# pyprob/pyprob

Hardware: AMD Instinct MI355X
Metric: ic_train_traces_per_sec (higher is better)
Workload: dtype f32; 1 GPU; GaussianUnknownMean IC training, offline traces resident in HBM, LSTM hidden=512, batch=1024 per GPU; traces_in_hbm=1000000, params=1643583, global_batch=1024, parallelism=dp1, optimizer=Adam lr=1e-3*sqrt(world), launch=one Python iteration per step (ICEngine.train_step), eager launches, prewarm_steps=5870, minibatches_resident=976, minibatch_walk=step i trains minibatch (i * 1) mod 976 of the resident dataset

## Files before the change

### include/pyprob_amd.h

```cpp
#ifndef PYPROB_AMD_H
#define PYPROB_AMD_H

#include <stddef.h>
#include <stdint.h>

#ifdef __cplusplus
extern "C" {
#endif

#define PP_ABI_VERSION 15
#define PP_MAX_OBS 8
#define PP_MAX_LSTM_DEPTH 4
#define PP_MAX_OBS_DEPTH 4

#define PP_EINVAL   (-1)
#define PP_ENOSPACE (-2)
#define PP_ENODEV   (-3)
#define PP_EHIP     (-4)

#define PP_HEAD_NORMAL_MIXTURE       0
#define PP_HEAD_TRUNCNORMAL_MIXTURE  1
#define PP_HEAD_CATEGORICAL          2
#define PP_HEAD_BERNOULLI            4
#define PP_HEAD_POISSON_TN_MIXTURE   3
// ... 53 lines not shown

size_t pp_cnn2d5c_workspace_bytes(const pp_net* net, int32_t o, int32_t n_images);
int pp_cnn2d5c_forward(const pp_net* net, int32_t o, const float* params, const float* x, int32_t n_images,
                       float* features_out, void* workspace, size_t workspace_bytes, void* stream);
int pp_cnn2d5c_backward(const pp_net* net, int32_t o, const float* params, const float* d_features, int32_t n_images,
                        float* grads, void* workspace, size_t workspace_bytes, int32_t flags, void* stream);

#define PP_ADDR_TABLE_COLS 8
#define PP_AT_KIND 0
#define PP_AT_SMP_IN 1
#define PP_AT_ADDR_EMB 2
#define PP_AT_DTYPE_EMB 3
#define PP_AT_SMP_W 4
#define PP_AT_SMP_B 5
#define PP_AT_N_OUT 6
#define PP_AT_RESERVED 7

typedef struct pp_batch {
    int32_t n_traces;
    int32_t n_rows;
    int32_t t_max;
    int32_t obs_width;
    const int32_t* n_active;
    const int32_t* row_off;
    const int32_t* grp_off;
    const float*   obs;
    const float*   value;
    const float*   prior;
    const int32_t* addr;
    const int32_t* prev_row;
    const int32_t* grp_rows;
    const int32_t* trace;
    const int32_t* row_off_dev;
    const int32_t* nxt_off;
    const int32_t* nxt_rows;
} pp_batch;

typedef struct pp_pack_info {
    int64_t n_traces, n_rows, t_max, device_words;
    int64_t obs, value, prior, addr, prev_row, grp_rows, trace, row_off_dev, nxt_rows;
    int64_t n_active, row_off, grp_off, nxt_off;
    int64_t order;
    int64_t src_row;
} pp_pack_info;

int64_t pp_pack_words(int32_t n_traces, int64_t n_rows, int32_t t_max, int32_t obs_width, int32_t n_addr);

int pp_pack_ragged(const int32_t* trace_len, const int32_t* addr_ids, const float* values, const float* prior,
                   int32_t prior_width, const float* obs, int32_t n_traces, int32_t obs_width, int32_t n_addr,
                   void* out, int64_t out_words, pp_pack_info* info);

typedef struct pp_shard_columns {
    const int32_t* trace_len;
    const int64_t* row_off;
    const float*   obs;
    const float*   value;
    const float*   prior;
    const int32_t* addr;
    const int32_t* addr_remap;
} pp_shard_columns;

int pp_pack_indexed(const pp_shard_columns* shards, int32_t n_shards, const int64_t* first, const int64_t* ids,
                    int32_t n_ids, int32_t obs_width, int32_t n_addr, void* out, int64_t out_words, pp_pack_info* info);


size_t pp_ic_workspace_bytes(const pp_net* net, int32_t n_traces, int32_t n_rows);

#define PP_LOSS_BACKWARD   1
#define PP_LOSS_ZERO_GRADS 2
#define PP_LOSS_KEEP_LP    4

int pp_ic_loss(const pp_net* net, const pp_batch* batch, const float* params , float* grads ,
               void* workspace , size_t workspace_bytes, float* loss_out ,
               int32_t* status_out , float* lp_out , int32_t flags, void* stream);

#define PP_ADAM_ZERO_GRADS 1
#define PP_ADAM_SCRATCH 1056
#define PP_ADAM_SEEN 1027
int pp_adam_step(float* params, float* grads, float* exp_avg, float* exp_avg_sq, int64_t n_params,
                 const int32_t* chunk_tensor, const float* active, int32_t* tensor_step, int32_t* scratch,
                 int32_t n_tensors, float lr, float beta1, float beta2, float eps, float weight_decay, float grad_scale,
                 int32_t flags, const int32_t* skip, void* stream);

int pp_sgd_step(float* params, float* grads, float* momentum_buf, int64_t n_params, const int32_t* chunk_tensor,
                const float* active, int32_t n_tensors, float lr, float momentum, int32_t nesterov, float weight_decay,
                float grad_scale, int32_t flags, const int32_t* skip, void* stream);

#define PP_LARC_SCRATCH_FLOATS(n_params, n_tensors) (2 * ((n_params) / 1024) + (n_tensors))
int pp_larc_scale(const float* params, float* grads, int64_t n_params, const int32_t* chunk_tensor, const float* active,
                  int32_t n_tensors, float lr, float weight_decay, float grad_scale, float trust_coefficient, float eps,
                  float epsilon, int32_t clip, float* scratch, const int32_t* skip, void* stream);

typedef struct pp_train_buffers {
    float* params; float* grads; float* exp_avg; float* exp_avg_sq;
    const int32_t* chunk_tensor; int32_t* tensor_step; int32_t* adam_scratch;
    void* workspace; size_t workspace_bytes;
    void* staging; void* device_batch; int64_t slot_words;
    float* loss_ring; int32_t* status_ring;
    int32_t n_tensors; int32_t n_slots;
    int32_t dp_world; int32_t dp_n_skip;
    int64_t dp_skip_off[4], dp_skip_cnt[4];
} pp_train_buffers;

typedef struct pp_tensor_roles {
    const int32_t* off;
    const int32_t* addr;
    const int32_t* role;
} pp_tensor_roles;

int64_t pp_train_slot_words(int32_t n_traces, int64_t n_rows, int32_t t_max, int32_t obs_width, int32_t n_addr,
                            int32_t n_tensors);

int pp_train_sync(void);
int pp_train_resident(const pp_net* net, const pp_train_buffers* tb, const pp_batch* const* batches,
                      const float* const* active, int32_t n_steps, const float* lr, float beta1, float beta2, float eps,
                      float weight_decay, int32_t grads_clean, void* stream);

int pp_train_steps(const pp_net* net, const pp_train_buffers* buffers, const pp_tensor_roles* roles,
                   const pp_shard_columns* shards, int32_t n_shards, const int64_t* first, int32_t obs_width,
                   const int64_t* ids, const int64_t* step_off, int32_t n_steps, const float* lr ,
                   float beta1, float beta2, float eps, float weight_decay, int32_t grads_clean,
                   int64_t* addr_iterations, void* stream);


size_t pp_is_workspace_bytes(const pp_net* net, int32_t n);

int pp_is_init(const pp_net* net, const float* params, const float* obs, float* e_out, void* workspace,
               size_t workspace_bytes, void* stream);

int pp_is_step(const pp_net* net, const float* params, int32_t addr_id, int32_t prev_addr_id, int32_t n,
               const float* e_obs_vec, const float* prev_value, const float* prior, int32_t prior_stride,
               float* h, float* c, int32_t state_rows, const float* value_in, float* value_out, float* logq_out,
               uint64_t seed, uint64_t offset, void* workspace, size_t workspace_bytes, void* stream);

int pp_is_step_rows(const pp_net* net, const float* params, int32_t addr_id, int32_t prev_addr_id, int32_t n,
                    const float* e_obs_vec, const float* prev_value, const float* prior, int32_t prior_stride,
                    float* h, float* c, int32_t state_rows, const int64_t* rows, const float* value_in, float* value_out,
                    float* logq_out, uint64_t seed, uint64_t offset, void* workspace, size_t workspace_bytes, void* stream);
int pp_is_step_fused_supported(const pp_net* net, int32_t addr_id, int32_t n);
int pp_is_statement_rows(const pp_net* net, const float* params, int32_t addr_id, int32_t prev_addr_id, int32_t n,
                         const float* e_obs_vec, const float* prev_value_full, const float* prior, int32_t prior_stride,
                         float* h, float* c, int32_t state_rows, const int64_t* rows, float* value_full, float* lw_full,
                         int32_t prior_kind, uint64_t seed, uint64_t offset, void* workspace, size_t workspace_bytes,
                         void* stream);

int pp_logweight_accumulate(int32_t kind, const float* p0, int32_t p0_stride, const float* p1, int32_t p1_stride,
                            const float* x, int32_t x_stride, float scale, float* lw , float* lp_out,
                            int32_t n, void* stream);

int pp_logweight_accumulate_rows(int32_t kind, const float* p0, int32_t p0_stride, const float* p1, int32_t p1_stride,
                                 const float* x, int32_t x_stride, float scale, float* lw ,
                                 const int64_t* rows, int32_t m, void* stream);

int pp_copy_rows(const float* src, int32_t src_stride, float* dst , const int64_t* rows, int32_t m, void* stream);

#define PP_PARTITION_SCRATCH(m) (((m) + 1023) / 1024 + 1)
int pp_partition_rows(const uint8_t* cond, const int64_t* rows, int32_t m, int64_t* rows_true, int64_t* rows_false,
                      int32_t* counts, int32_t* scratch, void* stream);
int pp_partition_rows_polled(const uint8_t* cond, const int64_t* rows, int32_t m, int64_t* rows_true, int64_t* rows_false,
                             int32_t* counts , int32_t seq, int32_t* scratch, void* stream);

typedef struct pp_lw_term {
    int32_t kind, p0_stride, p1_stride, x_stride;
    const float *p0, *p1, *x;
    float scale;
} pp_lw_term;
// ... 184 lines not shown
```

### pyprob_amd/autograd.py

```python
import torch

from . import lib as L
from .ops import ops


def presence(network, bring_home=False):
    eng = network._hip_engine
    index = {n: i for i, n in enumerate(eng.spec.tensors.keys())}
    present = [False] * len(index)
    for name, p in network._hip_named_parameters():
        if p.grad is None:
            continue
        present[index[name]] = True
        if bring_home:
            flat = eng.tensor(name, eng.grads)
            if p.grad.data_ptr() != flat.data_ptr():
                flat.copy_(p.grad)
    return tuple(present)


class HipLoss(torch.autograd.Function):

    @staticmethod
    def forward(ctx, network, packed, names, *params):
        eng = network._hip_engine
        flags = L.PP_LOSS_BACKWARD | (0 if network._hip_grads_clean else L.PP_LOSS_ZERO_GRADS)
        batch_dev, batch_host = packed.op_tensors(eng.device)
        eng._ensure_workspace(packed.n_traces, packed.n_rows)
        loss, status, _ = ops.ic_loss(eng.params, eng.grads, eng.workspace, batch_dev, batch_host, eng.net_handle, flags)
        network._hip_grads_clean = False
        network._hip_status = status
        ctx.network, ctx.names = network, names
        return loss.reshape(())

    @staticmethod
    def backward(ctx, grad_output):
        eng = ctx.network._hip_engine
        eng.grads.mul_(grad_output.reshape(()).to(eng.grads.device))
        return (None, None, None) + tuple(eng.tensor(n, eng.grads) for n in ctx.names)


class _HipOptimizer(torch.optim.Optimizer):

    def __init__(self, network, defaults, larc=False):
        self._network = network
        self._larc = bool(larc)
        super().__init__(list(network.parameters()), defaults)
        self._active_cache = {}
        self._stepped = set()

    def _begin(self):
        net = self._network
        eng = net._hip_engine
        present = presence(net, bring_home=True)
        act = self._active_cache.get(present)
        if act is None:
            act = self._active_cache[present] = torch.tensor(present, dtype=torch.float32).to(eng.device)
            self._stepped.update(i for i, f in enumerate(present) if f)
        eng.active.copy_(act)
        eng._active_key = None
        group = self.param_groups[0]
        wd, scale = float(group['weight_decay']), float(net._hip_grad_scale)
        if self._larc:
            need = L.larc_scratch_floats(eng.params.numel(), eng.active.numel())
            if getattr(self, '_larc_scratch', None) is None or self._larc_scratch.numel() < need:
                self._larc_scratch = torch.empty(need, dtype=torch.float32, device=eng.params.device)
            ops.larc_scale(eng.params, eng.grads, eng.chunk_tensor, eng.active, float(group['lr']), wd, scale, 0.002, 1e-8,
                           1.0 / 16000.0, True, self._larc_scratch, None)
            wd, scale = 0.0, 1.0
        return net, eng, group, wd, scale

    def _end(self, net):
        net._hip_grad_scale = 1.0
        net._hip_grads_clean = True

    def zero_grad(self, set_to_none=True):
        for p in self.param_groups[0]['params']:
            p.grad = None

    def _groups_state(self):
        groups = [dict((k, v) for k, v in self.param_groups[0].items() if k != 'params')]
        groups[0]['params'] = list(range(len(self.param_groups[0]['params'])))
        return groups

    def _load_groups(self, state_dict):
        for k, v in state_dict['param_groups'][0].items():
            if k != 'params':
                self.param_groups[0][k] = v


class HipSGD(_HipOptimizer):

    def __init__(self, network, lr, momentum=0.9, weight_decay=0.0, nesterov=True, larc=False):
        super().__init__(network, dict(lr=lr, momentum=momentum, dampening=0, weight_decay=weight_decay, nesterov=nesterov),
                         larc=larc)

    @torch.no_grad()
    def step(self, closure=None):
        net, eng, group, wd, scale = self._begin()
        ops.sgd_step(eng.params, eng.grads, eng.exp_avg, eng.chunk_tensor, eng.active, float(group['lr']),
                     float(group['momentum']), bool(group['nesterov']), wd, scale, L.PP_ADAM_ZERO_GRADS, None)
        self._end(net)

    def state_dict(self):
        net = self._network
        eng = net._hip_engine
        names = list(eng.spec.tensors.keys())
        state = {}
        if float(self.param_groups[0]['momentum']) != 0.0:
            for i, (name, p) in enumerate(net._hip_named_parameters()):
                if names.index(name) in self._stepped:
# ... 62 lines not shown
```

### pyprob_amd/csrc/cnn2d.hip

```cpp
#include "cnn2d.hpp"

#include <algorithm>

namespace pp {

bool cnn_geom(const pp_net* net, int o, CnnGeom& g) {
    if (!net || o < 0 || o >= net->n_obs || net->obs_kind[o] != PP_OBS_CNN2D5C) return false;
    g.C = net->obs_shape[o][0]; g.H = net->obs_shape[o][1]; g.W = net->obs_shape[o][2];
    if (g.C < 1 || g.C > 4 || g.H < 20 || g.W < 20) return false;
    const int ci[5] = {g.C, 64, 64, 128, 128}, co[5] = {64, 64, 128, 128, 128};
    int h = g.H, w = g.W;
    for (int l = 0; l < 5; ++l) {
        g.cin[l] = ci[l]; g.cout[l] = co[l]; g.hin[l] = h; g.win[l] = w;
        h -= 2; w -= 2;
        if (l == 1) { g.hp1 = h / 2; g.wp1 = w / 2; h = g.hp1; w = g.wp1; }
    }
    g.hp2 = h / 2; g.wp2 = w / 2;
    g.F = 128 * g.hp2 * g.wp2;
    return g.hp2 >= 1 && g.wp2 >= 1;
}

__global__ __launch_bounds__(256) void cnn_weight_images_kernel(const float* __restrict__ W, int Cin, int Cout,
                                                                float* __restrict__ wf, float* __restrict__ wd) {
    const int n = 9 * Cin * Cout;
// ... 416 lines not shown
    hipLaunchKernelGGL(wgrad_reduce_kernel, dim3(cdiv(wn + Cout, 256)), dim3(256), 0, st, w.part, dbp, S, Cin, Cout,
                       grads + net->obs_conv_w[o][l], grads + net->obs_conv_b[o][l]);
    PP_LAUNCH_CHECK("wgrad_reduce");
    prof_end(cls, 2.0 * (double)M * (double)wn, st);
    return 0;
}

int cnn_backward(const pp_net* net, int o, const float* dfeat, int64_t lddf, int B, float* grads, void* ws, size_t ws_bytes,
                 hipStream_t st) {
    CnnGeom g;
    CnnWs w;
    PP_TRY(check_cnn(net, o, g, B, ws, ws_bytes, w, "pp_cnn2d5c_backward"));
    PP_CHECK_ARG(dfeat && grads && lddf >= g.F, "pp_cnn2d5c_backward: null pointer or short rows");
    {
        const int H5 = g.hin[4] - 2, W5 = g.win[4] - 2;
        const int64_t n = (int64_t)B * H5 * W5 * 128;
        prof_begin(PP_PROF_CNN_BWD + 0, st);
        hipLaunchKernelGGL(maxpool_bwd_kernel, dim3(cdiv(n, 256)), dim3(256), 0, st, w.a[4], H5, W5, 128, dfeat, g.hp2, g.wp2, 1,
                           lddf, w.g0, n);
        PP_LAUNCH_CHECK("maxpool_bwd");
        prof_end(PP_PROF_CNN_BWD + 0, 0.0, st);
    }
    PP_TRY(conv_wgrad(net, o, g, 4, w.a[3], w.g0, B, w, grads, st));
    PP_TRY(conv_mfma(PP_PROF_CNN_BWD + 2, w.g0, g.hin[4] - 2, g.win[4] - 2, 128, 128, w.wd[4], nullptr, w.a[3], w.g1, 2, 0, B, st));
    PP_TRY(conv_wgrad(net, o, g, 3, w.a[2], w.g1, B, w, grads, st));
    PP_TRY(conv_mfma(PP_PROF_CNN_BWD + 4, w.g1, g.hin[3] - 2, g.win[3] - 2, 128, 128, w.wd[3], nullptr, w.a[2], w.g0, 2, 0, B, st));
    PP_TRY(conv_wgrad(net, o, g, 2, w.p1, w.g0, B, w, grads, st));
    PP_TRY(conv_mfma(PP_PROF_CNN_BWD + 6, w.g0, g.hin[2] - 2, g.win[2] - 2, 128, 64, w.wd[2], nullptr, nullptr, w.g1, 2, 0, B, st));
    {
        const int H2 = g.hin[1] - 2, W2 = g.win[1] - 2;
        const int64_t n = (int64_t)B * H2 * W2 * 64;
        prof_begin(PP_PROF_CNN_BWD + 7, st);
        hipLaunchKernelGGL(maxpool_bwd_kernel, dim3(cdiv(n, 256)), dim3(256), 0, st, w.a[1], H2, W2, 64, w.g1, g.hp1, g.wp1, 0,
                           (int64_t)0, w.g0, n);
        PP_LAUNCH_CHECK("maxpool_bwd");
        prof_end(PP_PROF_CNN_BWD + 7, 0.0, st);
    }
    PP_TRY(conv_wgrad(net, o, g, 1, w.a[0], w.g0, B, w, grads, st));
    PP_TRY(conv_mfma(PP_PROF_CNN_BWD + 9, w.g0, g.hin[1] - 2, g.win[1] - 2, 64, 64, w.wd[1], nullptr, w.a[0], w.g1, 2, 0, B, st));
    {
        const int64_t M = (int64_t)B * (g.H - 2) * (g.W - 2);
        int64_t chunk;
        const int64_t wn = 9 * (int64_t)g.C * 64;
        const int S = wgrad_splits(M, wn, &chunk);
        float* dbp = w.part + S * wn;
        const dim3 grid(S), block(256);
        prof_begin(PP_PROF_CNN_BWD + 10, st);
        switch (g.C) {
            case 1: hipLaunchKernelGGL(conv1_wgrad_kernel<1>, grid, block, 0, st, w.a0, w.g1, w.part, dbp, g.H, g.W, M, chunk); break;
            case 2: hipLaunchKernelGGL(conv1_wgrad_kernel<2>, grid, block, 0, st, w.a0, w.g1, w.part, dbp, g.H, g.W, M, chunk); break;
            case 3: hipLaunchKernelGGL(conv1_wgrad_kernel<3>, grid, block, 0, st, w.a0, w.g1, w.part, dbp, g.H, g.W, M, chunk); break;
            default: hipLaunchKernelGGL(conv1_wgrad_kernel<4>, grid, block, 0, st, w.a0, w.g1, w.part, dbp, g.H, g.W, M, chunk); break;
        }
        PP_LAUNCH_CHECK("conv1_wgrad");
        hipLaunchKernelGGL(wgrad_reduce_kernel, dim3(cdiv(wn + 64, 256)), dim3(256), 0, st, w.part, dbp, S, g.C, 64,
                           grads + net->obs_conv_w[o][0], grads + net->obs_conv_b[o][0]);
        PP_LAUNCH_CHECK("wgrad_reduce");
        prof_end(PP_PROF_CNN_BWD + 10, 2.0 * (double)M * (double)wn, st);
    }
    return 0;
}

}

extern "C" {

size_t pp_cnn2d5c_workspace_bytes(const pp_net* net, int32_t o, int32_t n_images) {
    return pp::cnn_workspace_bytes(net, o, n_images);
}

int pp_cnn2d5c_forward(const pp_net* net, int32_t o, const float* params, const float* x, int32_t n_images,
                       float* features_out, void* workspace, size_t workspace_bytes, void* stream) {
    pp::CnnGeom g;
    PP_CHECK_ARG(pp::cnn_geom(net, o, g), "pp_cnn2d5c_forward: observable %d is not a CNN2D5C embedding", o);
    return pp::cnn_forward(net, o, params, x, (int64_t)g.C * g.H * g.W, n_images, features_out, g.F, workspace, workspace_bytes,
                           true, pp::as_stream(stream));
}

int pp_cnn2d5c_backward(const pp_net* net, int32_t o, const float* params, const float* d_features, int32_t n_images,
                        float* grads, void* workspace, size_t workspace_bytes, int32_t flags, void* stream) {
    pp::CnnGeom g;
    PP_CHECK_ARG(pp::cnn_geom(net, o, g), "pp_cnn2d5c_backward: observable %d is not a CNN2D5C embedding", o);
    PP_CHECK_ARG(flags == 0, "pp_cnn2d5c_backward: flags must be 0");
    (void)params;
    return pp::cnn_backward(net, o, d_features, g.F, n_images, grads, workspace, workspace_bytes, pp::as_stream(stream));
}

}
```

### pyprob_amd/csrc/common.hpp

```cpp
#pragma once
#include <hip/hip_runtime.h>
#include <stdlib.h>
#include <stdint.h>
#include <stdio.h>

#include "../../include/pyprob_amd.h"

#define PP_LOSS_SLOTS_FLOATS (64 * 32 + 32)
#define PP_TAIL_TEAMS_MAX 16

namespace pp {

constexpr int kWave = 64;

typedef float f32x4 __attribute__((ext_vector_type(4)));
typedef float f32x16 __attribute__((ext_vector_type(16)));

void set_error(const char* fmt, ...);

#define PP_CHECK_ARG(cond, ...)          \
    do {                                 \
        if (!(cond)) {                   \
            pp::set_error(__VA_ARGS__);  \
            return PP_EINVAL;            \
        }                                \
    } while (0)

#define PP_LAUNCH_CHECK(name)                                                   \
    do {                                                                        \
        hipError_t e__ = hipGetLastError();                                     \
        if (e__ != hipSuccess) {                                                \
            pp::set_error("%s: launch failed: %s", name, hipGetErrorString(e__)); \
            return (int)e__;                                                    \
        }                                                                       \
    } while (0)

#define PP_TRY(expr)            \
    do {                        \
        int rc__ = (expr);      \
        if (rc__ != 0) return rc__; \
    } while (0)

struct GemmBlock {
    int m0, m1, n0, n1, k0, k1;
};
struct GemmHole {
    GemmBlock b[2];
};

static inline bool deterministic_mode() {
    static const int on = getenv("PP_DETERMINISTIC") ? atoi(getenv("PP_DETERMINISTIC")) : 0;
    return on != 0;
}

struct GemmExt {
    const float* rb; const int32_t* rb_addr; const int32_t* rb_prev;
    float* cell_c; float* cell_h; int cell_H, cell_rows;
    const float* cell_cprev;
    float* bw_G; const float* bw_C; int bw_H;
    int lean;
    int64_t split_stride; int force_splits;
};
struct AuxJobs;

void prof_begin(int which, hipStream_t st);
void prof_end(int which, double work, hipStream_t st);

int gemm_f32(const pp_gemm_args* a, hipStream_t st, const GemmHole* hole = nullptr, const GemmExt* ext = nullptr);
int gemm_f32_grouped(const pp_gemm_args* args, int count, hipStream_t st, const GemmHole* holes = nullptr,
                     const GemmExt* ext = nullptr, const AuxJobs* aux = nullptr);
int aux_jobs_launch(const AuxJobs& jobs, hipStream_t st);
bool lstm_input_fast_ok(const pp_gemm_args& g, const GemmExt& x);
int lstm_input_fast(const pp_gemm_args& g, const GemmExt& x, hipStream_t st);

static inline hipStream_t as_stream(void* s) { return reinterpret_cast<hipStream_t>(s); }
static inline int cdiv(int64_t a, int64_t b) { return (int)((a + b - 1) / b); }

template <int CTRL>
__device__ __forceinline__ float dpp_mov(float v) {
    return __int_as_float(__builtin_amdgcn_update_dpp(0, __float_as_int(v), CTRL, 0xF, 0xF, false));
}
__device__ __forceinline__ float lane_bcast(float v, int lane) {
    return __int_as_float(__builtin_amdgcn_readlane(__float_as_int(v), lane));
}
__device__ __forceinline__ float wave_sum(float v) {
    v += dpp_mov<0xB1>(v);
    v += dpp_mov<0x4E>(v);
    v += dpp_mov<0x124>(v);
    v += dpp_mov<0x128>(v);
    return (lane_bcast(v, 0) + lane_bcast(v, 16)) + (lane_bcast(v, 32) + lane_bcast(v, 48));
}
__device__ __forceinline__ float wave_max(float v) {
    v = fmaxf(v, dpp_mov<0xB1>(v));
    v = fmaxf(v, dpp_mov<0x4E>(v));
    v = fmaxf(v, dpp_mov<0x124>(v));
    v = fmaxf(v, dpp_mov<0x128>(v));
    return fmaxf(fmaxf(lane_bcast(v, 0), lane_bcast(v, 16)), fmaxf(lane_bcast(v, 32), lane_bcast(v, 48)));
}
__device__ __forceinline__ double wave_sum(double v) {
#pragma unroll
    for (int o = 32; o > 0; o >>= 1) v += __shfl_xor(v, o, 64);
// ... 58 lines not shown
```

### pyprob_amd/csrc/dp.hip

```cpp
#include "common.hpp"

#include <dlfcn.h>
#include <string.h>

#include <rccl/rccl.h>

namespace pp {

struct Rccl {
    void* lib = nullptr;
    ncclResult_t (*GetUniqueId)(ncclUniqueId*) = nullptr;
    ncclResult_t (*CommInitRank)(ncclComm_t*, int, ncclUniqueId, int) = nullptr;
    ncclResult_t (*CommDestroy)(ncclComm_t) = nullptr;
    ncclResult_t (*AllReduce)(const void*, void*, size_t, ncclDataType_t, ncclRedOp_t, ncclComm_t, hipStream_t) = nullptr;
    ncclResult_t (*GroupStart)() = nullptr;
    ncclResult_t (*GroupEnd)() = nullptr;
    const char* (*GetErrorString)(ncclResult_t) = nullptr;
    ncclComm_t comm = nullptr;
    int world = 0, rank = -1;
};
static Rccl g_rccl;

static int rccl_load(const char* path) {
    if (g_rccl.lib) return 0;
// ... 31 lines not shown
    } while (0)

#define PP_NCCL(call, what)                                                                    \
    do {                                                                                       \
        ncclResult_t r__ = (call);                                                             \
        if (r__ != ncclSuccess) {                                                              \
            set_error("pp_dp: %s failed: %s", what, g_rccl.GetErrorString(r__));               \
            return PP_EHIP;                                                                    \
        }                                                                                      \
    } while (0)

int dp_world() { return g_rccl.comm ? g_rccl.world : 0; }

int dp_allreduce_pieces(float* base, const int64_t* off, const int64_t* cnt, int n, hipStream_t st) {
    PP_CHECK_ARG(g_rccl.comm, "pp_dp: no communicator (pp_dp_init)");
    PP_CHECK_ARG(base && off && cnt && n >= 1, "pp_dp_allreduce: bad argument");
    if (n > 1) PP_NCCL(g_rccl.GroupStart(), "ncclGroupStart");
    for (int i = 0; i < n; ++i) {
        if (cnt[i] <= 0) continue;
        PP_NCCL(g_rccl.AllReduce(base + off[i], base + off[i], (size_t)cnt[i], ncclFloat32, ncclSum, g_rccl.comm, st), "ncclAllReduce");
    }
    if (n > 1) PP_NCCL(g_rccl.GroupEnd(), "ncclGroupEnd");
    return 0;
}

struct Overlap {
    int64_t off[2] = {0, 0}, cnt[2] = {0, 0};
    int n = 0;
    hipStream_t side = nullptr;
    hipEvent_t ready = nullptr, done = nullptr;
    hipEvent_t ev[5] = {nullptr, nullptr, nullptr, nullptr, nullptr};
    bool pending = false, stats = false, stats_valid = false;
};
static Overlap g_ov;

bool dp_overlap_hull(int64_t* lo, int64_t* hi) {
    if (!g_rccl.comm || g_ov.n <= 0) return false;
    *lo = g_ov.off[0];
    *hi = g_ov.off[g_ov.n - 1] + g_ov.cnt[g_ov.n - 1];
    return true;
}

static int overlap_objects() {
    if (g_ov.side) return 0;
    PP_HIP(hipStreamCreateWithFlags(&g_ov.side, hipStreamNonBlocking));
    PP_HIP(hipEventCreateWithFlags(&g_ov.ready, hipEventDisableTiming));
    PP_HIP(hipEventCreateWithFlags(&g_ov.done, hipEventDisableTiming));
    for (auto& e : g_ov.ev) PP_HIP(hipEventCreate(&e));
    return 0;
}

int dp_bucket0_issue(float* grads_full, hipStream_t st) {
    if (!g_rccl.comm || g_ov.n <= 0 || g_ov.pending) return 0;
    PP_TRY(overlap_objects());
    PP_HIP(hipEventRecord(g_ov.ready, st));
    PP_HIP(hipStreamWaitEvent(g_ov.side, g_ov.ready, 0));
    if (g_ov.stats) PP_HIP(hipEventRecord(g_ov.ev[0], g_ov.side));
    PP_TRY(dp_allreduce_pieces(grads_full, g_ov.off, g_ov.cnt, g_ov.n, g_ov.side));
    if (g_ov.stats) PP_HIP(hipEventRecord(g_ov.ev[1], g_ov.side));
    PP_HIP(hipEventRecord(g_ov.done, g_ov.side));
    g_ov.pending = true;
    return 0;
}

__global__ void dp_tail_pre_kernel(float* __restrict__ tail, const float* __restrict__ presence, int n_tensors,
                                   const int32_t* __restrict__ status) {
    for (int t = threadIdx.x; t < n_tensors; t += blockDim.x)
        if (presence) tail[t] = presence[t];
    if (threadIdx.x == 0) tail[n_tensors + 1] = status[0] != 0 ? 1.0f : 0.0f;
}
__global__ void dp_tail_post_kernel(const float* __restrict__ tail, int n_tensors, float inv_world, float* __restrict__ loss_out,
                                    int32_t* __restrict__ status_out) {
    if (threadIdx.x == 0) {
        if (loss_out) loss_out[0] = tail[n_tensors] * inv_world;
        if (status_out) status_out[0] = tail[n_tensors + 1] > 0.0f ? 1 : 0;
    }
}

int dp_reduce_grads(float* grads_full, int64_t n_params, int n_tensors, const float* presence, const int32_t* status,
                    const int64_t* skip_off, const int64_t* skip_cnt, int n_skip, float* loss_out, int32_t* status_out,
                    hipStream_t st) {
    PP_CHECK_ARG(g_rccl.comm && grads_full && status && n_params > 0 && n_tensors >= 0 && n_skip >= 0 && n_skip <= 6 && (!g_ov.pending || n_skip <= 4),
                 "pp_dp_reduce_grads: bad argument");
    float* tail = grads_full + n_params;
    hipLaunchKernelGGL(dp_tail_pre_kernel, dim3(1), dim3(256), 0, st, tail, presence, n_tensors, status);
    PP_LAUNCH_CHECK("pp_dp_reduce_grads (tail)");
    int64_t so[8], sc[8];
    int ns = 0;
    {
        int i = 0, j = 0;
        const int nj = g_ov.pending ? g_ov.n : 0;
        while (i < n_skip || j < nj) {
            const bool take_i = j >= nj || (i < n_skip && skip_off[i] <= g_ov.off[j]);
            so[ns] = take_i ? skip_off[i] : g_ov.off[j];
            sc[ns] = take_i ? skip_cnt[i] : g_ov.cnt[j];
            ++ns;
            if (take_i) ++i; else ++j;
        }
    }
    int64_t off[10], cnt[10];
    int n = 0;
    int64_t pos = 0;
    const int64_t total = n_params + n_tensors + 2;
    for (int i = 0; i < ns; ++i) {
        PP_CHECK_ARG(so[i] >= pos && so[i] + sc[i] <= n_params, "pp_dp_reduce_grads: bad skip range (or one that overlaps the overlap range)");
        if (so[i] > pos) { off[n] = pos; cnt[n] = so[i] - pos; ++n; }
        pos = so[i] + sc[i];
    }
    off[n] = pos; cnt[n] = total - pos; ++n;
    const bool stats = g_ov.pending && g_ov.stats;
    if (stats) PP_HIP(hipEventRecord(g_ov.ev[2], st));
    PP_TRY(dp_allreduce_pieces(grads_full, off, cnt, n, st));
    if (stats) PP_HIP(hipEventRecord(g_ov.ev[3], st));
    if (g_ov.pending) {
        PP_HIP(hipStreamWaitEvent(st, g_ov.done, 0));
        if (stats) {
            PP_HIP(hipEventRecord(g_ov.ev[4], st));
            g_ov.stats_valid = true;
        }
        g_ov.pending = false;
    }
    hipLaunchKernelGGL(dp_tail_post_kernel, dim3(1), dim3(64), 0, st, tail, n_tensors, 1.0f / (float)g_rccl.world, loss_out,
                       status_out);
    PP_LAUNCH_CHECK("pp_dp_reduce_grads (tail)");
    return 0;
}

}

extern "C" {

using pp::set_error;

int pp_dp_unique_id(const char* rccl_path, void* id_out) {
    PP_TRY(pp::rccl_load(rccl_path));
    PP_CHECK_ARG(id_out, "pp_dp_unique_id: null pointer");
    ncclUniqueId id;
    if (pp::g_rccl.GetUniqueId(&id) != ncclSuccess) {
        pp::set_error("pp_dp_unique_id: ncclGetUniqueId failed");
        return PP_EHIP;
    }
    memcpy(id_out, &id, sizeof(id));
    return 0;
}

int pp_dp_init(const char* rccl_path, const void* unique_id, int32_t rank, int32_t world) {
    PP_TRY(pp::rccl_load(rccl_path));
    PP_CHECK_ARG(unique_id && world >= 1 && rank >= 0 && rank < world, "pp_dp_init: bad argument");
    if (pp::g_rccl.comm) {
        pp::set_error("pp_dp_init: a communicator already exists (pp_dp_destroy first)");
        return PP_EINVAL;
    }
    ncclUniqueId id;
    memcpy(&id, unique_id, sizeof(id));
    ncclComm_t comm = nullptr;
    ncclResult_t r = pp::g_rccl.CommInitRank(&comm, world, id, rank);
    if (r != ncclSuccess) {
        pp::set_error("pp_dp_init: ncclCommInitRank failed: %s", pp::g_rccl.GetErrorString(r));
        return PP_EHIP;
    }
    pp::g_rccl.comm = comm;
    pp::g_rccl.world = world;
    pp::g_rccl.rank = rank;
    return 0;
}

int pp_dp_world(void) { return pp::dp_world(); }

int pp_dp_destroy(void) {
    if (pp::g_rccl.comm) {
        (void)pp::g_rccl.CommDestroy(pp::g_rccl.comm);
        pp::g_rccl.comm = nullptr;
        pp::g_rccl.world = 0;
        pp::g_rccl.rank = -1;
    }
    pp::g_ov.n = 0;
    pp::g_ov.pending = false;
    pp::g_ov.stats = pp::g_ov.stats_valid = false;
    return 0;
}

int pp_dp_overlap(const int64_t* off, const int64_t* cnt, int32_t n) {
    PP_CHECK_ARG(n >= 0 && n <= 2 && (n == 0 || (off && cnt)), "pp_dp_overlap: at most two ranges");
    if (pp::g_ov.pending) {
        pp::set_error("pp_dp_overlap: an overlapped all-reduce is in flight (call between steps)");
        return PP_EINVAL;
    }
    for (int i = 0; i < n; ++i) {
        PP_CHECK_ARG(off[i] >= 0 && cnt[i] > 0 && (i == 0 || off[i] >= off[i - 1] + cnt[i - 1]), "pp_dp_overlap: ranges must ascend");
        pp::g_ov.off[i] = off[i];
        pp::g_ov.cnt[i] = cnt[i];
    }
    pp::g_ov.n = n;
    return 0;
}

int pp_dp_overlap_stats(int32_t arm, float* us_out) {
    int filled = 0;
    if (us_out && pp::g_ov.stats_valid) {
        PP_HIP(hipEventSynchronize(pp::g_ov.ev[4]));
        PP_HIP(hipEventSynchronize(pp::g_ov.ev[1]));
        float a = 0, b = 0, c = 0;
        PP_HIP(hipEventElapsedTime(&a, pp::g_ov.ev[0], pp::g_ov.ev[1]));
        PP_HIP(hipEventElapsedTime(&b, pp::g_ov.ev[2], pp::g_ov.ev[3]));
        PP_HIP(hipEventElapsedTime(&c, pp::g_ov.ev[3], pp::g_ov.ev[4]));
        us_out[0] = a * 1e3f; us_out[1] = b * 1e3f; us_out[2] = c * 1e3f;
        filled = 1;
    }
    pp::g_ov.stats = arm != 0;
    if (!arm) pp::g_ov.stats_valid = false;
    return filled;
}

int pp_dp_allreduce(float* base, const int64_t* off, const int64_t* cnt, int32_t n, void* stream) {
    return pp::dp_allreduce_pieces(base, off, cnt, n, pp::as_stream(stream));
}

int pp_dp_reduce_grads(float* grads_full, int64_t n_params, int32_t n_tensors, const float* presence, const int32_t* status,
                       const int64_t* skip_off, const int64_t* skip_cnt, int32_t n_skip, float* loss_out,
                       int32_t* status_out, void* stream) {
    return pp::dp_reduce_grads(grads_full, n_params, n_tensors, presence, status, skip_off, skip_cnt, n_skip, loss_out, status_out,
                               pp::as_stream(stream));
}

}
```

### pyprob_amd/csrc/engine.hip

```cpp
#include "common.hpp"
#include "gather.hpp"
#include "aux_jobs.hpp"
#include "panel.hpp"
#include "panel16.hpp"
#include "wgrad_t1.hpp"
#include "cnn2d.hpp"

#include <stdlib.h>
#include <string.h>

#include <algorithm>
#include <vector>

namespace pp {

const char* last_error();
int colsum_multi(const ColsumJob* jobs, int count, hipStream_t st, const float* fin_acc = nullptr,
                 const int32_t* fin_flag = nullptr, int fin_traces = 0, float* fin_loss = nullptr,
                 int32_t* fin_status = nullptr);
int colsum_f32(const float* X, int64_t ldx, const int32_t* idx, int n_rows, int n_cols, float* out, float* out2,
               hipStream_t st);
int embedding_rows(const float* E, int64_t lde, const int32_t* trace, int n_rows, int e_obs, float* Hs, int64_t ldh,
                   float* zero_small, int n_small, hipStream_t st);
int sample_embed_bwd(const pp_net* net, const float* params, const float* value, const int32_t* addr,
                     const int32_t* prev_row, int row_begin, int n_rows, const float* dX, int64_t ldx, float* grads,
                     hipStream_t st);
bool dp_overlap_hull(int64_t* lo, int64_t* hi);
int dp_bucket0_issue(float* grads_full, hipStream_t st);
int lstm_tail_plan(const int32_t* n_active, int T, int H, int* t0_out, int* teams_out);
void lstm_tail_exchange_bytes(int H, size_t* fwd, size_t* bwd);
int lstm_tail_fwd(float* G, float* C, float* Hs, const float* Whh, const int32_t* row_off_dev, int t0, int T, int H, int teams,
                  void* xch_f, void* xch_b, int32_t* flag, hipStream_t st);
int lstm_tail_bwd(float* G, const float* C, float* dH, float* dC, const float* Whh, const int32_t* row_off_dev, int t0, int T,
                  int H, int teams, void* xch_f, void* xch_b, int32_t* flag, float* db, float* db2, const LossFinalize& fin,
                  hipStream_t st);
int obs_grad(const float* dX, int64_t ldx, const int32_t* row_off_dev, int t_max, int n_traces, int e_obs,
             const float* E, int64_t lde, float* dE, int64_t ldde, hipStream_t st);
int lstm_cell_fwd(float* G, const float* c_prev, float* c, float* h, int n, int H, hipStream_t st, int c_prev_shared = 0);
int lstm_cell_bwd(float* G, const float* c_prev, const float* c, const float* dh, float* dc_carry, int n, int n_next,
                  int H, float* db, float* db2, hipStream_t st, const float* fin_acc = nullptr,
                  const int32_t* fin_flag = nullptr, int fin_traces = 0, float* fin_loss = nullptr,
                  int32_t* fin_status = nullptr, const float* dh_parts = nullptr, int n_parts = 0, int64_t part_stride = 0);
int head_logprob(int kind, const float* y, int64_t ldy, const int32_t* rows, const float* value, const float* prior,
                 int n, int n_out, float grad_scale, float* lp_out, float* dy, float* loss_acc, int32_t* nonfinite,
                 hipStream_t st);
bool head_tail_supported(int kind, int hid, int n_out);
struct TailJob {
    const float* A1; const float* W2; const float* b2; const int32_t* rows; float* DY; float* dZ1; int n;
};
int head_tail_multi(int kind, const TailJob* jobs, int count, int64_t lda1, int hid, int n_out, const float* value,
                    const float* prior, float grad_scale, float* lp_out, int64_t lddy, int64_t lddz, float* loss_acc,
                    int32_t* nonfinite, hipStream_t st);
int loss_finalize(const float* acc, const int32_t* flag, int n_traces, float* loss_out, int32_t* status_out,
                  hipStream_t st);
int loss_from_rows(const float* lp, int n_rows, int n_traces, const int32_t* flag, float* loss_out, int32_t* status_out,
                   hipStream_t st);
int sample_embed_bwd_det(const pp_net* net, const float* params, const float* value, const int32_t* prev_row,
                         const int32_t* nxt_rows, const int32_t* nxt_off, const float* dX, int64_t ldx, float* grads,
                         hipStream_t st);
int adam_step(float* params, float* grads, float* m, float* v, int64_t n_params, const int32_t* chunk_tensor,
              const float* active, int32_t* tensor_step, int32_t* arrived, int n_tensors, float lr, float beta1, float beta2,
              float eps, float wd, float gscale, int flags, const int32_t* skip, hipStream_t st);

extern long long* g_timeline;

int obs_embed_dgrad_fused(const pp_net* net, const float* P, int n_traces, float* const* obs_h, const float* cat,
                          const float* f1, const float* dX, int64_t ldx, const int32_t* row_off_dev, int t_max,
                          const float* E, float* dE, float* dF1, float* dCat, float* dHo0, int64_t dh_stride,
                          hipStream_t st, int n_split = 1, int64_t split_stride = 0);

static inline int64_t round4(int64_t x) { return (x + 3) & ~int64_t(3); }

struct Prof {
    int which = -1;
    std::vector<hipEvent_t> ev0, ev1;
    std::vector<double> flops;
    int used = 0;
    int stride = 1, seen = 0;
    bool cur = false;
};
static Prof g_prof;

void prof_begin(int which, hipStream_t st) {
    if (g_prof.which != which) return;
    g_prof.cur = (g_prof.seen++ % g_prof.stride) == 0 && g_prof.used < (int)g_prof.ev0.size();
    if (g_prof.cur) (void)hipEventRecord(g_prof.ev0[g_prof.used], st);
}
void prof_end(int which, double flops, hipStream_t st) {
    if (g_prof.which == which && g_prof.cur) {
        (void)hipEventRecord(g_prof.ev1[g_prof.used], st);
        g_prof.flops[g_prof.used] = flops;
        g_prof.used++;
        g_prof.cur = false;
    }
}

struct Carver {
    char* base;
    size_t off = 0, cap;
    Carver(void* p, size_t c) : base(static_cast<char*>(p)), cap(c) {}
    template <typename T>
    T* take(int64_t count) {
        off = (off + 255) & ~size_t(255);
        T* p = base ? reinterpret_cast<T*>(base + off) : nullptr;
        off += (size_t)std::max<int64_t>(count, 1) * sizeof(T);
        return p;
    }
};

struct Workspace {
    float* obs_h[PP_MAX_OBS];
    float* obs_hl[PP_MAX_OBS][PP_MAX_OBS_DEPTH];
    float* dObsH2;
    float* cat;
    float* f1;
    float* E;
    float* X;
    float* G;
    float* C;
    float* Hs;
    float* Gl[PP_MAX_LSTM_DEPTH];
    float* Cl[PP_MAX_LSTM_DEPTH];
    float* Hl[PP_MAX_LSTM_DEPTH];
    float* dH2;
    float* A1;
    float* Y;
    float* DY;
    float* dZ1;
    float* dH;
    float* dC;
    float* dHp;
    float* dX;
    float* dE;
    float* dF1;
    float* dCat;
    float* dObsH;
    float* loss_acc;
    int32_t* flag;
    void* xch_f;
    void* xch_b;
    float* lp_rows;
    float* AB;
    float* gsum;
    float* WihT;
    float* W1T;
// ... 566 lines not shown
}

static void queue_head_bias_sums(const Step& s, GradQueue& q, const pp_addr& ad, int h0, int m) {
    const Workspace& w = s.w;
    q.cs.push_back(ColsumJob{w.DY + (int64_t)h0 * w.out4, w.out4, nullptr, m, ad.n_out, s.grads + ad.b2, nullptr});
    q.cs.push_back(ColsumJob{w.dZ1 + (int64_t)h0 * w.hid4, w.hid4, nullptr, m, ad.hid, s.grads + ad.b1, nullptr});
}

static int heads_forward(const Step& s, GradQueue& q) {
    const pp_net* net = s.net; const pp_batch* bt = s.bt; const Workspace& w = s.w; const StepPlan& p = s.p;
    const float* P = s.P; hipStream_t st = s.st;
    const int H = p.H;
    const float gscale = -1.0f / (float)p.B;
    {
        std::vector<pp_gemm_args> hq;
        for (int a = 0; a < net->n_addr; ++a) {
            const int g0 = bt->grp_off[a], n = bt->grp_off[a + 1] - g0;
            if (n <= 0) continue;
            const pp_addr& ad = net->addrs[a];
            pp_gemm_args g{};
            g.A = p.heads_in; g.lda = p.heads_ld; g.a_idx = bt->grp_rows + g0;
            g.B = P + ad.w1; g.ldb = H;
            g.C = w.A1 + (int64_t)g0 * w.hid4; g.ldc = w.hid4;
            g.M = n; g.N = ad.hid; g.K = H;
            g.bias = P + ad.b1; g.relu = 1;
            hq.push_back(g);
        }
        PP_TRY(gemm_f32_grouped(hq.data(), (int)hq.size(), st));
    }
    std::vector<char> done(net->n_addr, 0);
    for (int a = 0; a < net->n_addr; ++a) {
        const int g0 = bt->grp_off[a], n = bt->grp_off[a + 1] - g0;
        if (n <= 0 || done[a]) continue;
        const pp_addr& ad = net->addrs[a];
        if (head_tail_supported(ad.kind, ad.hid, ad.n_out)) {
            std::vector<TailJob> tj;
            for (int b = a; b < net->n_addr; ++b) {
                const pp_addr& bd = net->addrs[b];
                const int h0 = bt->grp_off[b], m = bt->grp_off[b + 1] - h0;
                if (m <= 0 || done[b] || bd.kind != ad.kind || bd.hid != ad.hid || bd.n_out != ad.n_out) continue;
                done[b] = 1;
                tj.push_back(TailJob{w.A1 + (int64_t)h0 * w.hid4, P + bd.w2, P + bd.b2, bt->grp_rows + h0,
                                     p.bwd ? w.DY + (int64_t)h0 * w.out4 : nullptr, w.dZ1 + (int64_t)h0 * w.hid4, m});
                if (p.bwd) queue_head_bias_sums(s, q, bd, h0, m);
            }
            PP_TRY(head_tail_multi(ad.kind, tj.data(), (int)tj.size(), w.hid4, ad.hid, ad.n_out, bt->value, bt->prior, gscale,
                                   p.lp_rows, w.out4, w.hid4, p.loss_slots, w.flag, st));
            continue;
        }
        done[a] = 1;
        float* A1 = w.A1 + (int64_t)g0 * w.hid4;
        float* Y = w.Y + (int64_t)g0 * w.out4;
        PP_TRY(linear_fwd(A1, w.hid4, nullptr, P + ad.w2, P + ad.b2, Y, w.out4, n, ad.hid, ad.n_out, false, nullptr, st));
        PP_TRY(head_logprob(ad.kind, Y, w.out4, bt->grp_rows + g0, bt->value, bt->prior, n, ad.n_out, gscale, p.lp_rows,
                            p.bwd ? w.DY + (int64_t)g0 * w.out4 : nullptr, p.loss_slots, w.flag, st));
    }
    return 0;
}

static void queue_head_wgrads(const Step& s, GradQueue& q, int a) {
    const pp_batch* bt = s.bt; const Workspace& w = s.w; const StepPlan& p = s.p;
    const pp_addr& ad = s.net->addrs[a];
    const int g0 = bt->grp_off[a], n = bt->grp_off[a + 1] - g0;
    queue_wgrad(q.wq, w.DY + (int64_t)g0 * w.out4, w.out4, w.A1 + (int64_t)g0 * w.hid4, w.hid4, nullptr, s.grads + ad.w2, n, ad.hid,
                ad.n_out);
    queue_wgrad(q.wq, w.dZ1 + (int64_t)g0 * w.hid4, w.hid4, p.heads_in, p.heads_ld, p.panel ? nullptr : bt->grp_rows + g0,
                s.grads + ad.w1, n, p.H, ad.hid);
}

static int heads_backward(const Step& s, GradQueue& q) {
    const pp_net* net = s.net; const pp_batch* bt = s.bt; const Workspace& w = s.w; const StepPlan& p = s.p;
    const float* P = s.P; float* grads = s.grads; hipStream_t st = s.st;
    const int H = p.H;
    std::vector<pp_gemm_args> dq;
    for (int a = 0; a < net->n_addr; ++a) {
        const int g0 = bt->grp_off[a], n = bt->grp_off[a + 1] - g0;
        if (n <= 0) continue;
        const pp_addr& ad = net->addrs[a];
        const float* A1 = w.A1 + (int64_t)g0 * w.hid4;
        const float* DY = w.DY + (int64_t)g0 * w.out4;
        float* dZ1 = w.dZ1 + (int64_t)g0 * w.hid4;
        queue_head_wgrads(s, q, a);
        if (!head_tail_supported(ad.kind, ad.hid, ad.n_out)) {
            PP_TRY(colsum_f32(DY, w.out4, nullptr, n, ad.n_out, grads + ad.b2, nullptr, st));
            PP_TRY(linear_dgrad(DY, w.out4, P + ad.w2, dZ1, w.hid4, nullptr, A1, w.hid4, n, ad.hid, ad.n_out, false, st,
                                p.det ? nullptr : grads + ad.b1));
            if (p.det) q.cs.push_back(ColsumJob{dZ1, w.hid4, nullptr, n, ad.hid, grads + ad.b1, nullptr});
        }
        pp_gemm_args g{};
        g.A = dZ1; g.lda = w.hid4;
        g.B = P + ad.w1; g.ldb = H; g.b_kmajor = 1;
        g.C = w.dH; g.ldc = H; g.c_idx = bt->grp_rows + g0;
        g.M = n; g.N = H; g.K = ad.hid;
        if (p.fused_bwd) g.colsum = w.gsum + (int64_t)a * 2 * 4 * H;
        dq.push_back(g);
    }
    if (p.fused_bwd) {
        GemmExt x{};
        x.bw_G = w.Gl[0]; x.bw_C = w.Cl[0]; x.bw_H = H; x.lean = p.lean_cell ? 1 : 0;
        return gemm_f32_grouped(dq.data(), (int)dq.size(), st, nullptr, &x);
    }
    return gemm_f32_grouped(dq.data(), (int)dq.size(), st);
}

static void queue_lstm_wgrads(const Step& s, GradQueue& q, int l) {
    const pp_net* net = s.net; const pp_batch* bt = s.bt; const Workspace& w = s.w; const StepPlan& p = s.p;
    const int B = p.B, R = p.R, H = p.H;
    const LstmLayer ly = lstm_layer(net, l);
    GemmHole wh{};
    if (l == 0 && p.compact) {
        wh.b[1] = GemmBlock{H, 2 * H, 0, p.nx, 0, B};
        wh.b[0] = GemmBlock{0, 4 * H, p.c1, p.nx, 0, B};
        queue_wgrad(q.wq, w.Gl[0], 4 * H, w.X, w.i4, nullptr, s.grads + net->w_ih, R, p.nx, 4 * H, &q.holes, wh);
        q.wq.back().ldc = p.I;
    } else {
        const float* in = l == 0 ? w.X : w.Hl[l - 1];
        const int64_t in_ld = l == 0 ? w.i4 : H;
        const int in_w = l == 0 ? p.I : H;
        wh.b[1] = GemmBlock{H, 2 * H, 0, in_w, 0, B};
        if (l == 0) wh.b[0] = GemmBlock{0, 4 * H, p.c1, p.c4, 0, B};
        queue_wgrad(q.wq, w.Gl[l], 4 * H, in, in_ld, nullptr, s.grads + ly.w_ih, R, in_w, 4 * H, &q.holes, wh);
    }
    if (p.T > 1) {
        const int r1 = bt->row_off[1];
        queue_wgrad(q.wq, w.Gl[l] + (int64_t)r1 * 4 * H, 4 * H, w.Hl[l], H, bt->prev_row + r1, s.grads + ly.w_hh, R - r1, H, 4 * H);
    }
}

static int lstm_backward_steps(const Step& s, int l, float* dH_cur) {
    const pp_batch* bt = s.bt; const Workspace& w = s.w; const StepPlan& p = s.p;
    const int B = p.B, T = p.T, H = p.H;
    const LstmLayer ly = lstm_layer(s.net, l);
    const float* Whh = s.P + ly.w_hh;
    float* db_ih = p.det ? nullptr : s.grads + ly.b_ih;
    float* db_hh = p.det ? nullptr : s.grads + ly.b_hh;
    LossFinalize fin = p.fin;
    if (l != p.L - 1) fin.acc = nullptr;
    int dh_parts = 0;
    for (int t = T - 1; t >= 0; --t) {
        if (p.tail_teams && t >= p.tail_t0) {
            PP_TRY(lstm_tail_bwd(w.Gl[l], w.Cl[l], dH_cur, w.dC, Whh, bt->row_off_dev, p.tail_t0, T, H, p.tail_teams, w.xch_f,
                                 w.xch_b, w.flag, db_ih, db_hh, fin, s.st));
            t = p.tail_t0;
            continue;
        }
        const int n = bt->n_active[t], r0 = bt->row_off[t];
        const int n_next = (t + 1 < T) ? bt->n_active[t + 1] : 0;
        float* Gt = w.Gl[l] + (int64_t)r0 * 4 * H;
        const float* c_prev = t > 0 ? w.Cl[l] + (int64_t)bt->row_off[t - 1] * H : nullptr;
        PP_TRY(lstm_cell_bwd(Gt, c_prev, w.Cl[l] + (int64_t)r0 * H, dH_cur + (int64_t)r0 * H, w.dC, n, n_next, H, db_ih, db_hh, s.st,
                             t == T - 1 ? fin.acc : nullptr, w.flag, B, fin.loss_out, fin.status_out, w.dHp, dh_parts,
                             (int64_t)B * H));
        dh_parts = 0;
        if (t == 0) break;
        const int tiles = cdiv(n, 64) * cdiv(H, 64), nslab = 4 * H / 32;
        const int splits = std::max(1, std::min({DH_SPLITS, cdiv(256, tiles), nslab / 2}));
        if (step_env().dh_partials && !p.det && splits > 1 && H % 4 == 0) {
            pp_gemm_args g{};
            g.A = Gt; g.lda = 4 * H;
            g.B = Whh; g.ldb = H; g.b_kmajor = 1;
            g.C = w.dHp; g.ldc = H;
            g.M = n; g.N = H; g.K = 4 * H;
            GemmExt x{};
            x.split_stride = (int64_t)B * H;
            x.force_splits = splits;
            PP_TRY(gemm_f32(&g, s.st, nullptr, &x));
            dh_parts = splits;
        } else {
            PP_TRY(linear_dgrad(Gt, 4 * H, Whh, dH_cur + (int64_t)bt->row_off[t - 1] * H, H, nullptr, nullptr, 0, n, H, 4 * H, true,
                                s.st));
        }
    }
    return 0;
}

static int lstm_backward(const Step& s, GradQueue& q) {
    const Workspace& w = s.w; const StepPlan& p = s.p;
    const int B = p.B, R = p.R, H = p.H;
    float* dH_cur = w.dH;
    float* dH_other = w.dH2;
    for (int l = p.L - 1; l >= 0; --l) {
        const LstmLayer ly = lstm_layer(s.net, l);
        if (!p.fused_bwd) PP_TRY(lstm_backward_steps(s, l, dH_cur));
        if (p.det)
            q.cs.push_back(ColsumJob{w.Gl[l], 4 * H, nullptr, R, 4 * H, s.grads + ly.b_ih, s.grads + ly.b_hh});
        queue_lstm_wgrads(s, q, l);
        if (l > 0) {
            GemmHole dh{};
            dh.b[0] = GemmBlock{0, B, 0, H, H, 2 * H};
            PP_TRY(linear_dgrad(w.Gl[l], 4 * H, s.P + ly.w_ih, dH_other, H, nullptr, nullptr, 0, R, H, 4 * H, false, s.st, nullptr,
                                &dh));
            std::swap(dH_cur, dH_other);
        }
    }
    return 0;
}

static int input_backward(const Step& s, GradQueue& q) {
    const pp_net* net = s.net; const pp_batch* bt = s.bt; const Workspace& w = s.w; const StepPlan& p = s.p;
    const float* P = s.P; float* grads = s.grads; hipStream_t st = s.st;
    const int B = p.B, R = p.R, T = p.T, H = p.H;
    if (p.compact) {
        const GemmHole dx_unused{{{0, B, p.c1, p.nx, 0, 4 * H}, {0, B, 0, p.nx, H, 2 * H}}};
        pp_gemm_args g{};
        g.A = w.G; g.lda = 4 * H;
        g.B = P + net->w_ih; g.ldb = p.I; g.b_kmajor = 1;
        g.C = w.dX; g.ldc = w.i4;
        g.M = R; g.N = p.nx; g.K = 4 * H;
        if (p.dx_partials) {
            GemmExt x{};
            x.split_stride = (int64_t)R * w.i4;
            x.force_splits = p.dx_splits;
            PP_TRY(gemm_f32(&g, st, &dx_unused, &x));
        } else {
            g.accumulate = 1;
            g.split_k = 1;
            PP_TRY(gemm_f32(&g, st, &dx_unused));
        }
        if (!p.fused_bwd)
            for (int a = 0; a < net->n_addr; ++a) {
                const int g0 = bt->grp_off[a], n = bt->grp_off[a + 1] - g0;
                if (n > 0) q.cs.push_back(ColsumJob{w.G, 4 * H, bt->grp_rows + g0, n, 4 * H, w.gsum + (int64_t)a * 2 * 4 * H, nullptr});
                const int q0 = bt->nxt_off[a], m = bt->nxt_off[a + 1] - q0;
                if (m > 0)
                    q.cs.push_back(ColsumJob{w.G, 4 * H, bt->nxt_rows + q0, m, 4 * H, w.gsum + ((int64_t)a * 2 + 1) * 4 * H, nullptr});
            }
    } else {
        const GemmHole dx_unused{{{0, B, p.c1, p.c4, 0, 4 * H}, {0, B, 0, p.I, H, 2 * H}}};
        PP_TRY(linear_dgrad(w.G, 4 * H, P + net->w_ih, w.dX, w.i4, nullptr, nullptr, 0, R, p.I, 4 * H, true, st, nullptr,
                            &dx_unused));
        for (int a = 0; a < net->n_addr; ++a) {
            const pp_addr& ad = net->addrs[a];
            const int g0 = bt->grp_off[a], n = bt->grp_off[a + 1] - g0;
            if (n > 0) {
                q.cs.push_back(ColsumJob{w.dX + p.c4, w.i4, bt->grp_rows + g0, n, net->dtype_dim, grads + ad.dtype_emb, nullptr});
                q.cs.push_back(ColsumJob{w.dX + p.c5, w.i4, bt->grp_rows + g0, n, net->addr_dim, grads + ad.addr_emb, nullptr});
            }
            const int q0 = bt->nxt_off[a], m = bt->nxt_off[a + 1] - q0;
            if (m > 0) {
                q.cs.push_back(ColsumJob{w.dX + p.c2, w.i4, bt->nxt_rows + q0, m, net->dtype_dim, grads + ad.dtype_emb, nullptr});
                q.cs.push_back(ColsumJob{w.dX + p.c3, w.i4, bt->nxt_rows + q0, m, net->addr_dim, grads + ad.addr_emb, nullptr});
            }
        }
    }
    if (T > 1 && p.det)
        PP_TRY(sample_embed_bwd_det(net, P, bt->value, bt->prev_row, bt->nxt_rows, bt->nxt_off, w.dX, w.i4, grads, st));
    else if (T > 1)
        PP_TRY(sample_embed_bwd(net, P, bt->value, bt->addr, bt->prev_row, bt->row_off[1], R, w.dX, w.i4, grads, st));
    return 0;
}

static int flush_wgrads(const Step& s, GradQueue& q, const AuxJobs* aux = nullptr) {
    std::vector<pp_gemm_args>& wq = q.wq;
    std::vector<GemmHole>& wholes = q.holes;
    wholes.resize(wq.size(), GemmHole{});
    int64_t lo = 0, hi = 0;
    if (dp_overlap_hull(&lo, &hi) && wq.size() > 1) {
        std::vector<pp_gemm_args> qa, qb;
        std::vector<GemmHole> ha, hb;
        for (size_t i = 0; i < wq.size(); ++i) {
            const bool in = wq[i].C >= s.grads + lo && wq[i].C < s.grads + hi;
            (in ? qa : qb).push_back(wq[i]);
            (in ? ha : hb).push_back(wholes[i]);
        }
        if (!qa.empty() && !qb.empty()) {
            PP_TRY(launch_wgrads(qa, s.st, &ha, true, aux, true));
            PP_TRY(dp_bucket0_issue(s.grads, s.st));
            PP_TRY(launch_wgrads(qb, s.st, &hb, false, nullptr, true));
            wq.clear();
            wholes.clear();
            return 0;
        }
    }
    PP_TRY(launch_wgrads(wq, s.st, &wholes, true, aux, true));
    wq.clear();
    wholes.clear();
    return 0;
}

static bool colsums_ride(const std::vector<ColsumJob>& cs, AuxJobs& aux) {
    int n_live = 0;
    for (const auto& j : cs) n_live += (j.n_rows > 0 && j.n_cols > 0) ? 1 : 0;
    if (n_live > AUX_MAX_COLSUM) return false;
    for (const auto& j : cs)
        if (j.n_rows > 0 && j.n_cols > 0) aux.cs[aux.n_colsum++] = j;
    return true;
}

static int reduce_and_flush(const Step& s, GradQueue& q) {
    const pp_net* net = s.net; const StepPlan& p = s.p;
    const bool ride = step_env().aux_colsum;
    AuxJobs aux{};
    if (!p.compact) {
        if (p.ff && !p.det && ride && !q.wq.empty() && colsums_ride(q.cs, aux)) {
            aux.fin = p.fin;
            aux_layout(aux, false);
            return flush_wgrads(s, q, &aux);
        }
        if (p.ff)
            PP_TRY(colsum_multi(q.cs.data(), (int)q.cs.size(), s.st, p.fin_acc, s.w.flag, p.B, p.fin.loss_out, p.fin.status_out));
        else
            PP_TRY(colsum_multi(q.cs.data(), (int)q.cs.size(), s.st));
        return flush_wgrads(s, q);
    }
    if (!(p.fused_bwd && ride && colsums_ride(q.cs, aux))) PP_TRY(colsum_multi(q.cs.data(), (int)q.cs.size(), s.st));
    aux_derived(s, aux);
    if (p.fused_bwd) {
        aux.db_ih = s.grads + net->b_ih; aux.db_hh = s.grads + net->b_hh;
        aux.fin = p.fin;
    }
    aux_layout(aux, true);
    return flush_wgrads(s, q, &aux);
}

static const float* obs_grad_rows(const Step& s, int64_t* ld) {
    *ld = s.p.ff ? s.p.H : s.w.i4;
    return s.p.ff ? s.w.dH : s.w.dX;
}

static int obs_dgrad_fused(const Step& s) {
    const Workspace& w = s.w; const StepPlan& p = s.p;
    int64_t ldxs;
    const float* dXs = obs_grad_rows(s, &ldxs);
    return obs_embed_dgrad_fused(s.net, s.P, p.B, w.obs_h, w.cat, w.f1, dXs, ldxs, s.bt->row_off_dev, p.T, w.E, w.dE, w.dF1, w.dCat,
                                 w.dObsH, (int64_t)p.B * w.maxohid4, s.st, p.dx_splits, (int64_t)p.R * w.i4);
}
static void queue_obs_grads_fused(const Step& s, GradQueue& q) {
    const pp_net* net = s.net; const pp_batch* bt = s.bt; const Workspace& w = s.w;
    float* grads = s.grads;
    const int B = s.p.B, e = net->e_obs;
    const int64_t dhs = (int64_t)B * w.maxohid4;
    queue_wgrad(q.wq, w.dE, w.e4, w.f1, w.e4, nullptr, grads + net->fin_w1, B, e, e);
    queue_wgrad(q.wq, w.dF1, w.e4, w.cat, w.e4, nullptr, grads + net->fin_w0, B, e, e);
    q.cs.push_back(ColsumJob{w.dE, w.e4, nullptr, B, e, grads + net->fin_b1, nullptr});
    q.cs.push_back(ColsumJob{w.dF1, w.e4, nullptr, B, e, grads + net->fin_b0, nullptr});
    int ci = 0, co = 0;
    for (int o = 0; o < net->n_obs; ++o) {
        const int in = net->obs_in[o], hid = net->obs_hid[o], out = net->obs_out[o];
        float* dHo = w.dObsH + (int64_t)o * dhs;
        queue_wgrad(q.wq, w.dCat + co, w.e4, w.obs_h[o], w.ohid4[o], nullptr, grads + net->obs_w1[o], B, hid, out);
        for (int k = 0; k < in; ++k)
            q.cs.push_back(ColsumJob{dHo, w.ohid4[o], nullptr, B, hid, grads + net->obs_w0[o] + k, nullptr, bt->obs + ci + k,
                                     bt->obs_width, in});
        q.cs.push_back(ColsumJob{w.dCat + co, w.e4, nullptr, B, out, grads + net->obs_b1[o], nullptr});
        q.cs.push_back(ColsumJob{dHo, w.ohid4[o], nullptr, B, hid, grads + net->obs_b0[o], nullptr});
        ci += in;
        co += out;
    }
}

static int obs_backward_generic(const Step& s, GradQueue& q) {
    const pp_net* net = s.net; const pp_batch* bt = s.bt; const Workspace& w = s.w; const StepPlan& p = s.p;
    const float* P = s.P; float* grads = s.grads; hipStream_t st = s.st;
    const int B = p.B, e = net->e_obs;
    int64_t ldxs;
    const float* dXs = obs_grad_rows(s, &ldxs);
    PP_TRY(obs_grad(dXs, ldxs, bt->row_off_dev, p.T, B, e, w.E, w.e4, w.dE, w.e4, st));
    PP_TRY(reduce_and_flush(s, q));
    PP_TRY(linear_wgrad(w.dE, w.e4, w.f1, w.e4, nullptr, grads + net->fin_w1, grads + net->fin_b1, nullptr, B, e, e, st));
    PP_TRY(linear_dgrad(w.dE, w.e4, P + net->fin_w1, w.dF1, w.e4, nullptr, w.f1, w.e4, B, e, e, false, st,
                        p.det ? nullptr : grads + net->fin_b0));
    if (p.det) PP_TRY(colsum_f32(w.dF1, w.e4, nullptr, B, e, grads + net->fin_b0, nullptr, st));
    PP_TRY(linear_wgrad(w.dF1, w.e4, w.cat, w.e4, nullptr, grads + net->fin_w0, nullptr, nullptr, B, e, e, st));
    PP_TRY(linear_dgrad(w.dF1, w.e4, P + net->fin_w0, w.dCat, w.e4, nullptr, w.cat, w.e4, B, e, e, false, st));
    int ci = 0, co = 0;
    for (int o = 0; o < net->n_obs; ++o) {
        const bool cnn = net->obs_kind[o] == PP_OBS_CNN2D5C;
        const float* dz = w.dCat + co;
        int64_t lddz = w.e4;
        float* scratch[2] = {w.dObsH, w.dObsH2};
        for (int l = obs_layers(net, o) - 1; l >= 0; --l) {
            const ObsLin ly = obs_lin(net, o, l);
            const float* x = l == 0 ? (cnn ? w.cnn_feat[o] : bt->obs + ci) : w.obs_hl[o][l - 1];
            const int64_t ldx = l == 0 ? (cnn ? w.f4[o] : bt->obs_width) : w.ohid4[o];
            PP_TRY(linear_wgrad(dz, lddz, x, ldx, nullptr, grads + ly.w, grads + ly.b, nullptr, B, ly.in, ly.out, st));
            if (l > 0) {
                float* dprev = scratch[l & 1];
                PP_TRY(linear_dgrad(dz, lddz, P + ly.w, dprev, w.ohid4[o], nullptr, x, ldx, B, ly.in, ly.out, false, st));
                dz = dprev;
                lddz = w.ohid4[o];
            } else if (cnn) {
                PP_TRY(linear_dgrad(dz, lddz, P + ly.w, w.cnn_dfeat[o], w.f4[o], nullptr, nullptr, 0, B, ly.in, ly.out, false, st));
                PP_TRY(cnn_backward(net, o, w.cnn_dfeat[o], w.f4[o], B, grads, w.cnn_ws[o], w.cnn_ws_bytes[o], st));
            }
        }
        ci += net->obs_in[o];
        co += net->obs_out[o];
    }
    return 0;
}

int ic_loss(const pp_net* net, const pp_batch* bt, const float* P, float* grads, void* ws,
            size_t ws_bytes, float* loss_out, int32_t* status_out, float* lp_out, int flags, hipStream_t st) {
    PP_TRY(check_net(net));
    PP_CHECK_ARG(bt && P && ws && loss_out, "pp_ic_loss: null pointer");
    PP_CHECK_ARG(bt->n_traces > 0 && bt->n_rows >= bt->n_traces && bt->t_max >= 1, "pp_ic_loss: empty batch");
    PP_CHECK_ARG(bt->n_active && bt->row_off && bt->grp_off && bt->obs && bt->value && bt->prior && bt->addr &&
                     bt->prev_row && bt->grp_rows && bt->trace && bt->row_off_dev && bt->nxt_off && bt->nxt_rows,
                 "pp_ic_loss: incomplete pp_batch");
    {
        int obs_in = 0;
        for (int o = 0; o < net->n_obs; ++o) obs_in += net->obs_in[o];
        PP_CHECK_ARG(bt->obs_width == obs_in, "pp_ic_loss: batch obs_width %d != the network's observable width %d",
                     bt->obs_width, obs_in);
    }
    const bool bwd = flags & PP_LOSS_BACKWARD;
    PP_CHECK_ARG(!bwd || grads, "pp_ic_loss: PP_LOSS_BACKWARD needs a gradient buffer");
    Workspace w;
    carve(net, bt->n_traces, bt->n_rows, ws, ws_bytes, w);
    if (w.bytes > ws_bytes) {
        set_error("pp_ic_loss: workspace too small (%zu < %zu bytes)", ws_bytes, w.bytes);
        return PP_ENOSPACE;
    }
    if (bwd && (flags & PP_LOSS_ZERO_GRADS)) (void)hipMemsetAsync(grads, 0, (size_t)net->n_params * sizeof(float), st);
    const StepPlan p = plan_step(net, bt, flags, lp_out, loss_out, status_out, w);
    const Step s{net, bt, P, grads, w, p, st, lp_out, flags};
    GradQueue q;
    PP_TRY(first_launch(s));
    if (p.panel) {
        PP_TRY(panel_launch(s));
        const pp_addr& ad = net->addrs[p.only_addr];
        queue_head_bias_sums(s, q, ad, 0, p.R);
        queue_head_wgrads(s, q, p.only_addr);
        queue_lstm_wgrads(s, q, 0);
        if (!p.obs_tail) PP_TRY(obs_dgrad_fused(s));
        queue_obs_grads_fused(s, q);
        return reduce_and_flush(s, q);
    }
    PP_TRY(lstm_forward(s));
    PP_TRY(heads_forward(s, q));
    if (p.det) PP_TRY(loss_from_rows(p.lp_rows, p.R, p.B, w.flag, loss_out, status_out, st));
    if (!bwd) {
        if (!p.det) PP_TRY(loss_finalize(w.loss_acc, w.flag, p.B, loss_out, status_out, st));
        return 0;
    }
    PP_TRY(heads_backward(s, q));
    PP_TRY(lstm_backward(s, q));
    if (!p.ff) PP_TRY(input_backward(s, q));
    if (!p.fused_obs) return obs_backward_generic(s, q);
    PP_TRY(obs_dgrad_fused(s));
    queue_obs_grads_fused(s, q);
    return reduce_and_flush(s, q);
}

}

extern "C" {

int pp_abi_version(void) { return PP_ABI_VERSION; }
const char* pp_last_error(void) { return pp::last_error(); }

int pp_device_count(void) {
    int n = 0;
    if (hipGetDeviceCount(&n) != hipSuccess) return 0;
    int ok = 0;
    for (int i = 0; i < n; ++i) {
        hipDeviceProp_t prop;
        if (hipGetDeviceProperties(&prop, i) == hipSuccess && strncmp(prop.gcnArchName, "gfx950", 6) == 0) ok++;
    }
    return ok;
}

size_t pp_ic_workspace_bytes(const pp_net* net, int32_t n_traces, int32_t n_rows) {
    if (!net || pp::check_net(net) != 0) return 0;
    pp::Workspace w;
    pp::carve(net, n_traces, n_rows, nullptr, 0, w);
    return w.bytes;
}

int pp_ic_loss(const pp_net* net, const pp_batch* batch, const float* params, float* grads, void* workspace,
               size_t workspace_bytes, float* loss_out, int32_t* status_out, float* lp_out, int32_t flags, void* stream) {
    return pp::ic_loss(net, batch, params, grads, workspace, workspace_bytes, loss_out, status_out, lp_out, flags,
                       pp::as_stream(stream));
}

int pp_adam_step(float* params, float* grads, float* exp_avg, float* exp_avg_sq, int64_t n_params,
                 const int32_t* chunk_tensor, const float* active, int32_t* tensor_step, int32_t* arrived, int32_t n_tensors,
                 float lr, float beta1, float beta2, float eps, float weight_decay, float grad_scale, int32_t flags,
                 const int32_t* skip, void* stream) {
    pp::prof_begin(3, pp::as_stream(stream));
    const int rc = pp::adam_step(params, grads, exp_avg, exp_avg_sq, n_params, chunk_tensor, active, tensor_step, arrived,
                                 n_tensors, lr, beta1, beta2, eps, weight_decay, grad_scale, flags, skip, pp::as_stream(stream));
    pp::prof_end(3, ((flags & PP_ADAM_ZERO_GRADS) ? 32.0 : 28.0) * (double)n_params, pp::as_stream(stream));
    return rc;
}

int pp_colsum_f32(const float* X, int64_t ldx, const int32_t* row_idx, int32_t n_rows, int32_t n_cols, float* out,
                  float* out2, void* stream) {
    return pp::colsum_f32(X, ldx, row_idx, n_rows, n_cols, out, out2, pp::as_stream(stream));
}

int pp_lstm_input_gather(const pp_net* net, const float* params, const float* E, const int32_t* trace_of_row,
                         const float* value, const int32_t* addr, const int32_t* prev_row, int32_t n_rows, float* X,
                         int64_t ldx, void* stream) {
    if (!net) return PP_EINVAL;
    return pp::lstm_input_gather(net, params, E, pp::round4(net->e_obs), trace_of_row, value, addr, prev_row, -1, -1, n_rows,
                                 X, ldx, pp::as_stream(stream));
}

int pp_lstm_cell_fwd(float* G, const float* c_prev, float* c, float* h, int32_t n, int32_t H, void* stream) {
    return pp::lstm_cell_fwd(G, c_prev, c, h, n, H, pp::as_stream(stream));
}

int pp_lstm_cell_bwd(float* G, const float* c_prev, const float* c, const float* dh, float* dc_carry, int32_t n,
                     int32_t n_next, int32_t H, void* stream) {
    return pp::lstm_cell_bwd(G, c_prev, c, dh, dc_carry, n, n_next, H, nullptr, nullptr, pp::as_stream(stream));
}

int pp_head_logprob(int32_t kind, const float* y, int64_t ldy, const int32_t* rows, const float* value, const float* prior,
                    int32_t n, int32_t n_out, float grad_scale, float* lp_out, float* dy, float* loss_acc,
                    int32_t* nonfinite, void* stream) {
    return pp::head_logprob(kind, y, ldy, rows, value, prior, n, n_out, grad_scale, lp_out, dy, loss_acc, nonfinite,
                            pp::as_stream(stream));
}

__global__ void clock_probe_kernel(int iters, long long* out, float* sink) {
    float x = (float)threadIdx.x;
    const long long c0 = clock64();
    const long long w0 = wall_clock64();
    for (int i = 0; i < iters; ++i) x = x * 1.0000001f + 0.5f;
    const long long c1 = clock64();
    const long long w1 = wall_clock64();
    if (threadIdx.x == 0) {
        out[0] = c1 - c0;
        out[1] = w1 - w0;
    }
    if (x == 123.456f) sink[0] = x;
}

int pp_debug_clock_probe(int32_t iters, long long* out , float* sink , void* stream) {
    hipLaunchKernelGGL(clock_probe_kernel, dim3(1), dim3(64), 0, pp::as_stream(stream), iters, out, sink);
    PP_LAUNCH_CHECK("pp_debug_clock_probe");
    return 0;
}

int pp_debug_timeline(long long* buf ) {
    pp::g_timeline = buf;
    return 0;
}

int pp_prof_arm(int32_t which, int32_t max_samples) {
    for (auto e : pp::g_prof.ev0) (void)hipEventDestroy(e);
    for (auto e : pp::g_prof.ev1) (void)hipEventDestroy(e);
    pp::g_prof.ev0.clear();
    pp::g_prof.ev1.clear();
    pp::g_prof.flops.clear();
    pp::g_prof.used = 0;
    pp::g_prof.seen = 0;
    pp::g_prof.cur = false;
    pp::g_prof.which = -1;
    if (max_samples <= 0) return 0;
    pp::g_prof.ev0.resize(max_samples);
    pp::g_prof.ev1.resize(max_samples);
    pp::g_prof.flops.assign(max_samples, 0.0);
    for (int i = 0; i < max_samples; ++i) {
        if (hipEventCreate(&pp::g_prof.ev0[i]) != hipSuccess || hipEventCreate(&pp::g_prof.ev1[i]) != hipSuccess) {
            pp::set_error("pp_prof_arm: hipEventCreate failed");
            return PP_ENODEV;
        }
    }
    pp::g_prof.which = which;
    return 0;
}

int pp_prof_stride(int32_t stride) {
    pp::g_prof.stride = stride > 0 ? stride : 1;
    return 0;
}

int pp_prof_collect(float* ms_out, int32_t cap, int32_t* n_out, double* flops_out) {
    int n = std::min<int>(pp::g_prof.used, cap);
// ... 14 lines not shown
```

### pyprob_amd/csrc/gemm_f32.hip

```cpp
#include "common.hpp"
#include "aux_jobs.hpp"

#include <algorithm>

namespace pp {

extern long long* g_timeline;
#define GEMM_STAMP(k) do { __builtin_amdgcn_sched_barrier(0); if (p.dbg && threadIdx.x == 0 && bx == 1 && by == 1 && bz == 0) p.dbg[10 + (k)] = clock64(); __builtin_amdgcn_sched_barrier(0); } while (0)

constexpr int BK = 32;
constexpr int KPAD = 4;

struct GemmParams {
    const float* A; int64_t lda; const int32_t* a_idx;
    const float* B; int64_t ldb; const int32_t* b_idx;
    float* C; int64_t ldc; const int32_t* c_idx;
    int M, N, K;
    const float* bias; const float* bias2;
    const float* mask; int64_t ldmask;
    float* colsum;
    int relu, accumulate;
    int vec;
    int vec_c;
    int dbg_plain;
// ... 1573 lines not shown
                        a->K, (long long)a->lda, (long long)a->ldb, (int)((uintptr_t)a->A & 15), (int)((uintptr_t)a->B & 15));
            as = as && async_ok(a);
            tiles += (int64_t)cdiv(a->M, 64) * cdiv(a->N, 64);
            static const int effw = 1;
            work += effw ? effective_work(a, holes ? &holes[k] : nullptr)
                         : (int64_t)cdiv(a->M, 64) * cdiv(a->N, 64) * cdiv(a->K, BK);
            work32 += (int64_t)cdiv(a->M, DT) * cdiv(a->N, DT) * cdiv(a->K, BK);
            ++c;
        }
        const bool direct = (ext && ext->bw_G) ? true : use_direct(tiles, work);
        const int target = as ? target_async : target_staged;
        static const int spb_max = 24;
        const int spb = direct ? (int)std::max<int64_t>(8, (work32 + target_direct - 1) / target_direct)
                               : (int)std::min<int64_t>(spb_max, std::max<int64_t>(2, (work + target - 1) / target));
        const int tile = direct ? DT : 64;
        int64_t active_blocks = 0;
        int xcd_cursor = 0;
        int j = i;
        for (; j < count && g.count < GROUP_MAX; ++j) {
            const pp_gemm_args* a = &args[j];
            PP_CHECK_ARG(a->A && a->B && a->C && a->M >= 0 && a->N >= 0 && a->K >= 0, "pp_gemm_f32_grouped: bad problem");
            if (a->a_kmajor != akm || a->b_kmajor != bkm) break;
            if (a->M == 0 || a->N == 0) continue;
            const int q = g.count++;
            fill_params(a, g.p[q]);
            set_hole(g.p[q], holes ? &holes[j] : nullptr);
            g.p[q].vec = vec_ok(a) ? 1 : 0;
            int splits = direct ? (split_allowed(a) ? std::max(1, std::min(cdiv(cdiv(a->K, BK), spb), 32)) : 1)
                                : pick_splits_by_work(a, spb);
            static const int small_div = 1;
            if (!direct && as && small_div > 1 && split_allowed(a) && (int64_t)cdiv(a->M, 64) * cdiv(a->N, 64) <= 2)
                splits = std::max(splits, pick_splits_by_work(a, std::max(2, spb / small_div)));
            if (as && !direct && split_allowed(a) && !async_split_ok(a, splits))
                splits = std::min(cdiv(cdiv(a->K, BK), AS_KSLABS), 32);
            if (splits > 1 && !a->accumulate) PP_TRY(zero_for_split(a, st));
            as = as && async_split_ok(a, splits);
            g.gx[q] = cdiv(a->N, tile); g.gy[q] = cdiv(a->M, tile); g.gz[q] = splits;
            {
                int act = g.gx[q] * g.gy[q];
                if (tile == 64) (void)effective_work(a, holes ? &holes[j] : nullptr, &act);
                active_blocks += (int64_t)act * splits;
            }
            g.pmode[q] = pick_pmode(a->M, a->N, g.gx[q], g.gy[q]);
            static const int rotate = 1;
            g.rot[q] = (g.pmode[q] == 0 && rotate) ? (xcd_cursor & 7) : 0;
            if (g.pmode[q] == 0) xcd_cursor += g.gx[q] * g.gy[q];
            g.first[q + 1] = g.first[q] + group_blocks(g.gx[q], g.gy[q], splits, g.pmode[q]);
        }
        if (g_wgtrace && ((g_wgtrace_mode == 1 && akm && bkm) || (g_wgtrace_mode == 2 && !akm && bkm)) &&
            g.first[g.count] + (aux_pending ? aux->n_blocks : 0) <= g_wgtrace_cap)
            g.trace = g_wgtrace;
        bool rode = false;
        if (g.count > 0 && aux_pending && aux_fused_ok && akm && bkm && (direct || as)) {
            const int rc = direct ? launch_direct_grouped_aux(g, *aux, st)
                                  : launch_async_grouped_aux(g, *aux, eight_waves(active_blocks), st);
            if (rc == 0) {
                rode = true;
                aux_pending = false;
            } else {
                (void)hipGetLastError();
                aux_fused_ok = false;
            }
        }
        if (rode) { i = j; continue; }
        if (g.count > 0 && direct) PP_TRY(launch_direct_grouped(g, akm, bkm, st));
        else if (g.count > 0 && as) PP_TRY(launch_async_grouped(g, akm, bkm, st, active_blocks));
        else
        if (g.count > 0) PP_TRY(launch_grouped<4>(g, akm, bkm, st));
        i = j;
    }
    if (aux_pending) PP_TRY(aux_jobs_launch(*aux, st));
    return 0;
}

}

extern "C" int pp_debug_wgtrace(long long* buf, int32_t cap, int32_t mode) {
    pp::g_wgtrace = buf;
    pp::g_wgtrace_cap = cap;
    pp::g_wgtrace_mode = mode;
    return 0;
}

extern "C" int pp_gemm_f32(const pp_gemm_args* args, void* stream) { return pp::gemm_f32(args, pp::as_stream(stream), nullptr, nullptr); }
extern "C" int pp_gemm_f32_grouped(const pp_gemm_args* args, int32_t count, void* stream) {
    return pp::gemm_f32_grouped(args, count, pp::as_stream(stream), nullptr, nullptr, nullptr);
}
```

### pyprob_amd/csrc/is_kernels.hip

```cpp
#include "common.hpp"
#include "gather.hpp"
#include "is_draw.hpp"
#include "is_step_fused.hpp"
#include "obs_embed.hpp"
#include "cnn2d.hpp"

#include <math.h>
#include <string.h>

#include <algorithm>

namespace pp {

int lstm_cell_fwd(float* G, const float* c_prev, float* c, float* h, int n, int H, hipStream_t st, int c_prev_shared = 0);
bool obs_fused_supported(const pp_net* net);

static inline int64_t round4(int64_t x) { return (x + 3) & ~int64_t(3); }

template <int KIND>
__global__ __launch_bounds__(256) void is_mixture_shared_kernel(const float* __restrict__ y, const float* __restrict__ prior,
                                                                int n, int K, const float* __restrict__ value_in,
                                                                float* __restrict__ value_out,
                                                                float* __restrict__ logq_out, uint64_t seed,
                                                                uint64_t offset) {
// ... 1415 lines not shown
    PP_LAUNCH_CHECK("pp_is_fused");
    return 0;
}

int pp_logweight_accumulate(int32_t kind, const float* p0, int32_t p0_stride, const float* p1, int32_t p1_stride,
                            const float* x, int32_t x_stride, float scale, float* lw, float* lp_out, int32_t n,
                            void* stream) {
    if (!(p0 && x) || !pp::lw_kind_ok(kind, p1, p1_stride) || kind == 2) {
        pp::set_error("pp_logweight_accumulate: bad argument");
        return PP_EINVAL;
    }
    if (n <= 0) return 0;
    hipLaunchKernelGGL(pp::logweight_kernel, dim3(pp::cdiv(n, 256)), dim3(256), 0, pp::as_stream(stream), kind, p0,
                       p0_stride, p1, p1_stride, x, x_stride, scale, lw, lp_out, n);
    PP_LAUNCH_CHECK("pp_logweight_accumulate");
    return 0;
}

int pp_logweight_accumulate_rows(int32_t kind, const float* p0, int32_t p0_stride, const float* p1, int32_t p1_stride,
                                 const float* x, int32_t x_stride, float scale, float* lw, const int64_t* rows, int32_t m,
                                 void* stream) {
    if (!(p0 && x && lw && rows) || !pp::lw_kind_ok(kind, p1, p1_stride) || kind == 2) {
        pp::set_error("pp_logweight_accumulate_rows: bad argument");
        return PP_EINVAL;
    }
    if (m <= 0) return 0;
    hipLaunchKernelGGL(pp::logweight_rows_kernel, dim3(pp::cdiv(m, 256)), dim3(256), 0, pp::as_stream(stream), kind, p0, p0_stride,
                       p1, p1_stride, x, x_stride, scale, lw, rows, m);
    PP_LAUNCH_CHECK("pp_logweight_accumulate_rows");
    return 0;
}

int pp_copy_rows(const float* src, int32_t src_stride, float* dst, const int64_t* rows, int32_t m, void* stream) {
    if (!(src && dst && rows) || (src_stride != 0 && src_stride != 1)) {
        pp::set_error("pp_copy_rows: bad argument");
        return PP_EINVAL;
    }
    if (m <= 0) return 0;
    hipLaunchKernelGGL(pp::rows_copy_kernel, dim3(pp::cdiv(m, 256)), dim3(256), 0, pp::as_stream(stream), src, src_stride, dst, rows, m);
    PP_LAUNCH_CHECK("pp_copy_rows");
    return 0;
}

static int partition_rows(const uint8_t* cond, const int64_t* rows, int32_t m, int64_t* rows_true, int64_t* rows_false,
                          int32_t* counts, int32_t* scratch, int seq, void* stream) {
    if (!(cond && rows_true && rows_false && counts && scratch) || m < 0) {
        pp::set_error("pp_partition_rows: bad argument (scratch of PP_PARTITION_SCRATCH(m) int32 is required)");
        return PP_EINVAL;
    }
    hipStream_t st = pp::as_stream(stream);
    if (m == 0) {
        if (seq != 0) {
            pp::set_error("pp_partition_rows_polled: m = 0 needs no launch (the caller knows the counts)");
            return PP_EINVAL;
        }
        (void)hipMemsetAsync(counts, 0, 2 * sizeof(int32_t), st);
        return 0;
    }
    const int blocks = pp::cdiv(m, pp::PART_TILE);
    hipLaunchKernelGGL(pp::partition_count_kernel, dim3(blocks), dim3(256), 0, st, cond, rows, m, scratch);
    hipLaunchKernelGGL(pp::partition_scatter_kernel, dim3(blocks), dim3(256), 0, st, cond, rows, m, scratch, rows_true, rows_false,
                       counts, seq);
    PP_LAUNCH_CHECK("pp_partition_rows");
    return 0;
}

int pp_partition_rows(const uint8_t* cond, const int64_t* rows, int32_t m, int64_t* rows_true, int64_t* rows_false,
                      int32_t* counts, int32_t* scratch, void* stream) {
    return partition_rows(cond, rows, m, rows_true, rows_false, counts, scratch, 0, stream);
}

int pp_partition_rows_polled(const uint8_t* cond, const int64_t* rows, int32_t m, int64_t* rows_true, int64_t* rows_false,
                             int32_t* counts, int32_t seq, int32_t* scratch, void* stream) {
    if (seq == 0) {
        pp::set_error("pp_partition_rows_polled: seq must be non-zero");
        return PP_EINVAL;
    }
    return partition_rows(cond, rows, m, rows_true, rows_false, counts, scratch, seq, stream);
}

int pp_axpy(float scale, const float* term, float* lw, int32_t n, void* stream) {
    if (!(term && lw)) return PP_EINVAL;
    if (n <= 0) return 0;
    hipLaunchKernelGGL(pp::axpy_kernel, dim3(pp::cdiv(n, 256)), dim3(256), 0, pp::as_stream(stream), scale, term, lw, n);
    PP_LAUNCH_CHECK("pp_axpy");
    return 0;
}

int pp_is_stats(const float* lw, const float* x, int32_t n, double* out, double* scratch, void* stream) {
    if (!(lw && out && scratch) || n <= 0) {
        pp::set_error("pp_is_stats: bad argument (scratch of PP_IS_STATS_SCRATCH doubles is required)");
        return PP_EINVAL;
    }
    const int tile = 256 * pp::STAT_PER_THREAD;
    const int blocks = std::min(pp::STAT_BLOCKS, pp::cdiv(n, tile));
    hipLaunchKernelGGL(pp::is_stats_partial_kernel, dim3(blocks), dim3(256), 0, pp::as_stream(stream), lw, x, n, scratch);
    hipLaunchKernelGGL(pp::is_stats_combine_kernel, dim3(1), dim3(256), 0, pp::as_stream(stream), scratch, blocks, out);
    PP_LAUNCH_CHECK("pp_is_stats");
    return 0;
}

int pp_logweight_terms(const pp_lw_term* terms, int32_t count, float* lw, int32_t n, int32_t overwrite, void* stream) {
    if (!(terms && lw) || count < 1 || count > 4) {
        pp::set_error("pp_logweight_terms: 1..4 terms");
        return PP_EINVAL;
    }
    if (n <= 0) return 0;
    pp::LwTerms t;
    t.count = count;
    for (int q = 0; q < count; ++q) {
        const pp_lw_term& s = terms[q];
        if (!s.x || (s.kind != 2 && !(s.p0 && pp::lw_kind_ok(s.kind, s.p1, s.p1_stride)))) {
            pp::set_error("pp_logweight_terms: bad term %d", q);
            return PP_EINVAL;
        }
        t.t[q] = pp::LwTerm{s.kind, s.p0_stride, s.p1_stride, s.x_stride, s.p0, s.p1, s.x, s.scale};
    }
    hipLaunchKernelGGL(pp::logweight_multi_kernel, dim3(pp::cdiv(n, 256)), dim3(256), 0, pp::as_stream(stream), t, lw, n,
                       overwrite);
    PP_LAUNCH_CHECK("pp_logweight_terms");
    return 0;
}

}
```

### pyprob_amd/csrc/kernels.hip

```cpp
#include "common.hpp"
#include "gather.hpp"
#include "head_math.hpp"
#include "aux_jobs.hpp"

#include <math.h>
#include <stdarg.h>
#include <stdlib.h>

#include <algorithm>
#include <vector>

namespace pp {

static thread_local char g_err[512] = "";
void set_error(const char* fmt, ...) {
    va_list ap;
    va_start(ap, fmt);
    vsnprintf(g_err, sizeof(g_err), fmt, ap);
    va_end(ap);
}
const char* last_error() { return g_err; }

constexpr int COLSUM_ROWS = 64;
constexpr int COLSUM_MAX_JOBS = 48;

int loss_finalize(const float* acc, const int32_t* flag, int n_traces, float* loss_out, int32_t* status_out, hipStream_t st);

struct ColsumGroups {
    ColsumJob j[COLSUM_MAX_JOBS];
    int first[COLSUM_MAX_JOBS + 1];
};

__global__ __launch_bounds__(256) void colsum_det_kernel(const ColsumGroups g) {
    __shared__ float part[4][64];
    const int tid = threadIdx.x, cl = tid & 63, rl = tid >> 6;
    const int col = blockIdx.x * 64 + cl;
    const int j0 = g.first[blockIdx.y], j1 = g.first[blockIdx.y + 1];
    float total = 0.0f;
    for (int q = j0; q < j1; ++q) {
        const ColsumJob& jb = g.j[q];
        float acc = 0.0f;
        if (col < jb.n_cols) {
            for (int i = rl; i < jb.n_rows; i += 4) {
                const int64_t r = jb.idx ? (int64_t)jb.idx[i] : (int64_t)i;
                float v = jb.X[r * jb.ldx + col];
                if (jb.wgt) v *= jb.wgt[(int64_t)i * jb.ldw];
                acc += v;
            }
        }
        part[rl][cl] = acc;
        __syncthreads();
        if (rl == 0) total += (part[0][cl] + part[1][cl]) + (part[2][cl] + part[3][cl]);
        __syncthreads();
    }
    const ColsumJob& j = g.j[j0];
    if (rl == 0 && col < j.n_cols) {
        float* dst = j.out + (int64_t)col * (j.out_stride ? j.out_stride : 1);
        *dst += total;
        if (j.out2) j.out2[col] += total;
    }
}

static int colsum_multi_det(const ColsumJob* jobs, int count, hipStream_t st) {
    std::vector<char> done(count, 0);
    int left = 0;
    for (int i = 0; i < count; ++i) {
        if (jobs[i].n_rows <= 0 || jobs[i].n_cols <= 0) done[i] = 1; else ++left;
    }
    while (left > 0) {
        ColsumGroups pack;
        int n = 0, groups = 0, max_cols = 0;
        pack.first[0] = 0;
        for (int i = 0; i < count && n < COLSUM_MAX_JOBS; ++i) {
            if (done[i]) continue;
            bool clash = false;
            for (int q = 0; q < n; ++q) clash = clash || pack.j[q].out == jobs[i].out;
            if (clash) continue;
            const int g0 = n;
            for (int k = i; k < count && n < COLSUM_MAX_JOBS; ++k) {
                if (done[k] || jobs[k].out != jobs[i].out) continue;
                PP_CHECK_ARG(jobs[k].X && jobs[k].n_cols == jobs[i].n_cols && jobs[k].out2 == jobs[i].out2 &&
                                 jobs[k].out_stride == jobs[i].out_stride, "pp_colsum_f32: inconsistent jobs for one destination");
                pack.j[n++] = jobs[k];
                done[k] = 1;
                --left;
            }
            if (n > g0) {
                pack.first[++groups] = n;
                max_cols = std::max(max_cols, jobs[i].n_cols);
            }
        }
        if (groups == 0) break;
// ... 855 lines not shown
        TailJobs pack;
        int nj = 0, max_n = 0;
        for (; i < count && nj < TAIL_MAX_JOBS; ++i) {
            if (jobs[i].n <= 0) continue;
            PP_CHECK_ARG(jobs[i].A1 && jobs[i].W2 && jobs[i].b2 && (!jobs[i].DY || jobs[i].dZ1), "head_tail: bad job");
            pack.j[nj++] = jobs[i];
            max_n = std::max(max_n, jobs[i].n);
        }
        if (nj == 0) continue;
        const int rpw = std::max((max_n + 4 * 256 - 1) / (4 * 256), 1);
        dim3 grid(cdiv(max_n, 4 * rpw), nj);
        if (kind == PP_HEAD_NORMAL_MIXTURE)
            PP_TRY(head_tail_launch<0>(ne, grid, lds, st, pack, lda1, hid, n_out / 3, value, prior, rpw, grad_scale, lp_out, lddy,
                                       lddz, loss_acc, nonfinite));
        else if (kind == PP_HEAD_TRUNCNORMAL_MIXTURE)
            PP_TRY(head_tail_launch<1>(ne, grid, lds, st, pack, lda1, hid, n_out / 3, value, prior, rpw, grad_scale, lp_out, lddy,
                                       lddz, loss_acc, nonfinite));
        else
            PP_TRY(head_tail_launch<2>(ne, grid, lds, st, pack, lda1, hid, n_out / 3, value, prior, rpw, grad_scale, lp_out, lddy,
                                       lddz, loss_acc, nonfinite));
        PP_LAUNCH_CHECK("head_tail");
    }
    return 0;
}

__global__ void loss_finalize_kernel(const float* __restrict__ acc, const int32_t* __restrict__ flag, float inv_b,
                                     float* __restrict__ loss_out, int32_t* __restrict__ status_out) {
    float tot = 0.0f;
    for (int k = 0; k < 64; ++k) tot += acc[32 * k];
    const float l = tot * inv_b;
    loss_out[0] = l;
    if (status_out) status_out[0] = (flag[0] != 0 || !isfinite(l)) ? 1 : 0;
}

__global__ __launch_bounds__(256) void loss_rows_kernel(const float* __restrict__ lp, int n_rows, float inv_b,
                                                        const int32_t* __restrict__ flag, float* __restrict__ loss_out,
                                                        int32_t* __restrict__ status_out) {
    __shared__ double part[256];
    __shared__ int bad[256];
    double acc = 0.0;
    int b = 0;
    for (int r = threadIdx.x; r < n_rows; r += 256) {
        float l = lp[r];
        if (l == -INFINITY) l = kLogEps;
        if (!isfinite(l)) b = 1;
        acc -= (double)l;
    }
    part[threadIdx.x] = acc;
    bad[threadIdx.x] = b;
    __syncthreads();
    for (int s = 128; s > 0; s >>= 1) {
        if (threadIdx.x < s) {
            part[threadIdx.x] += part[threadIdx.x + s];
            bad[threadIdx.x] |= bad[threadIdx.x + s];
        }
        __syncthreads();
    }
    if (threadIdx.x == 0) {
        const float l = (float)(part[0] * (double)inv_b);
        loss_out[0] = l;
        if (status_out) status_out[0] = (bad[0] || (flag && flag[0] != 0) || !isfinite(l)) ? 1 : 0;
    }
}

int loss_from_rows(const float* lp, int n_rows, int n_traces, const int32_t* flag, float* loss_out, int32_t* status_out,
                   hipStream_t st) {
    hipLaunchKernelGGL(loss_rows_kernel, dim3(1), dim3(256), 0, st, lp, n_rows, 1.0f / (float)n_traces, flag, loss_out,
                       status_out);
    PP_LAUNCH_CHECK("loss_from_rows");
    return 0;
}

int loss_finalize(const float* acc, const int32_t* flag, int n_traces, float* loss_out, int32_t* status_out,
                  hipStream_t st) {
    hipLaunchKernelGGL(loss_finalize_kernel, dim3(1), dim3(1), 0, st, acc, flag, 1.0f / (float)n_traces, loss_out,
                       status_out);
    PP_LAUNCH_CHECK("loss_finalize");
    return 0;
}

constexpr int ADAM_TOP = 1024, ADAM_FIRST = 1025, ADAM_CHUNKS = 1026;
constexpr int ADAM_SEEN = 1027;

__global__ __launch_bounds__(256) void adam_kernel(float* __restrict__ P, float* __restrict__ Gr, float* __restrict__ M,
                                                   float* __restrict__ V, const int32_t* __restrict__ chunk_tensor,
                                                   int n_chunks, const float* __restrict__ active,
                                                   int32_t* __restrict__ tensor_step, int32_t* __restrict__ scratch, float lr,
                                                   float beta1, float beta2, float eps, float wd, float gscale,
                                                   int zero_grads, const int32_t* __restrict__ skip, int wt) {
    __shared__ float s_corr[2];
    const uint32_t buf_bytes = (uint32_t)n_chunks * 4096u, wo = ((uint32_t)blockIdx.x * 1024u + threadIdx.x * 4u) * 4u;
    const f32x4 zero4 = f32x4{0.f, 0.f, 0.f, 0.f};
    const int b = blockIdx.x;
    const bool skipped = skip && skip[0] != 0;
    const int t = chunk_tensor[b];
    if (t < 0 || !(active[t] > 0.0f)) return;
    if (skipped) {
        if (zero_grads) {
            if (wt) store16_wt(Gr, buf_bytes, wo, zero4);
            else *reinterpret_cast<f32x4*>(Gr + (int64_t)b * 1024 + threadIdx.x * 4) = zero4;
        }
        return;
    }
    int32_t* const sc = scratch + (int64_t)t * PP_ADAM_SCRATCH;
    const int64_t o = (int64_t)b * 1024 + threadIdx.x * 4;
    const f32x4 g0 = *reinterpret_cast<const f32x4*>(Gr + o);
    __shared__ int s_seen;
    if (threadIdx.x == 0) s_seen = __atomic_load_n(sc + ADAM_SEEN, __ATOMIC_RELAXED);
    __syncthreads();
    const bool seen = s_seen != 0;
    bool idle = false;
    if (!seen && wd == 0.0f) {
        const bool zero = g0[0] == 0.0f && g0[1] == 0.0f && g0[2] == 0.0f && g0[3] == 0.0f;
        idle = __syncthreads_and(zero ? 1 : 0) != 0;
        if (!idle && threadIdx.x == 0) __atomic_store_n(sc + ADAM_SEEN, 1, __ATOMIC_RELAXED);
    } else if (!seen && threadIdx.x == 0) {
        __atomic_store_n(sc + ADAM_SEEN, 1, __ATOMIC_RELAXED);
    }
    f32x4 p = f32x4{0.f, 0.f, 0.f, 0.f}, m = p, v = p;
    if (!idle) {
        p = *reinterpret_cast<f32x4*>(P + o);
        m = *reinterpret_cast<f32x4*>(M + o);
        v = *reinterpret_cast<f32x4*>(V + o);
    }
    int step_old = 0, first = 0, chunks = 0;
    if (threadIdx.x == 0) {
        first = __atomic_load_n(sc + ADAM_FIRST, __ATOMIC_RELAXED) - 1;
        chunks = __atomic_load_n(sc + ADAM_CHUNKS, __ATOMIC_RELAXED);
        if (first < 0) {
            int lo = 0, hi = b;
            while (lo < hi) {
                const int mid = (lo + hi) >> 1;
                if (chunk_tensor[mid] < t) lo = mid + 1; else hi = mid;
            }
            int lo2 = b, hi2 = n_chunks;
            while (lo2 < hi2) {
                const int mid = (lo2 + hi2) >> 1;
                if (chunk_tensor[mid] <= t) lo2 = mid + 1; else hi2 = mid;
            }
            first = lo;
            chunks = lo2 - lo;
        }
        step_old = __atomic_load_n(tensor_step + t, __ATOMIC_RELAXED);
        const int step = step_old + 1;
        double p1 = 1.0, p2 = 1.0, q1 = (double)beta1, q2 = (double)beta2;
        for (int e = step; e > 0; e >>= 1) {
            if (e & 1) { p1 *= q1; p2 *= q2; }
            q1 *= q1;
            q2 *= q2;
        }
        const double bc1 = 1.0 - p1, bc2 = 1.0 - p2;
        s_corr[0] = (float)((double)lr / bc1);
        s_corr[1] = (float)(1.0 / sqrt(bc2));
    }
    __syncthreads();
    const float step_size = s_corr[0], inv_sqrt_bc2 = s_corr[1];
    const int k = (b - first) & 31;
    const int quota = (chunks - k + 31) >> 5;
    int ticket = -1;
    if (threadIdx.x == 0) ticket = atomicAdd(sc + 32 * k, 1);
    if (!idle) {
#pragma unroll
        for (int e = 0; e < 4; ++e) {
            float g = g0[e] * gscale;
            if (wd != 0.0f) g += wd * p[e];
            m[e] = beta1 * m[e] + (1.0f - beta1) * g;
            v[e] = beta2 * v[e] + (1.0f - beta2) * g * g;
            const float denom = sqrtf(v[e]) * inv_sqrt_bc2 + eps;
            p[e] -= step_size * (m[e] / denom);
        }
        if (wt) {
            store16_wt(P, buf_bytes, wo, p);
            store16_wt(M, buf_bytes, wo, m);
            store16_wt(V, buf_bytes, wo, v);
            if (zero_grads) store16_wt(Gr, buf_bytes, wo, zero4);
        } else {
            *reinterpret_cast<f32x4*>(P + o) = p;
            *reinterpret_cast<f32x4*>(M + o) = m;
            *reinterpret_cast<f32x4*>(V + o) = v;
            if (zero_grads) *reinterpret_cast<f32x4*>(Gr + o) = zero4;
        }
    }
    if (threadIdx.x == 0 && ticket == quota - 1) {
        __atomic_store_n(sc + 32 * k, 0, __ATOMIC_RELAXED);
        if (atomicAdd(sc + ADAM_TOP, 1) == min(chunks, 32) - 1) {
            __atomic_store_n(sc + ADAM_TOP, 0, __ATOMIC_RELAXED);
            __atomic_store_n(sc + ADAM_FIRST, first + 1, __ATOMIC_RELAXED);
            __atomic_store_n(sc + ADAM_CHUNKS, chunks, __ATOMIC_RELAXED);
            __atomic_store_n(tensor_step + t, step_old + 1, __ATOMIC_RELAXED);
        }
    }
}

int adam_step(float* params, float* grads, float* m, float* v, int64_t n_params, const int32_t* chunk_tensor,
              const float* active, int32_t* tensor_step, int32_t* scratch, int n_tensors, float lr, float beta1, float beta2,
              float eps, float wd, float gscale, int flags, const int32_t* skip, hipStream_t st) {
    PP_CHECK_ARG(params && grads && m && v && chunk_tensor && active && tensor_step && scratch, "pp_adam_step: null pointer");
    PP_CHECK_ARG(n_params % 1024 == 0, "pp_adam_step: n_params must be a multiple of 1024 (padded tensors)");
    if (n_tensors <= 0 || n_params == 0) return 0;
    const int n_chunks = (int)(n_params / 1024);
    const int wt = store_wt_mode() && n_params < ((int64_t)1 << 30) ? 1 : 0;
    hipLaunchKernelGGL(adam_kernel, dim3((unsigned)n_chunks), dim3(256), 0, st, params, grads, m, v, chunk_tensor, n_chunks,
                       active, tensor_step, scratch, lr, beta1, beta2, eps, wd, gscale, (flags & PP_ADAM_ZERO_GRADS) ? 1 : 0, skip, wt);
    PP_LAUNCH_CHECK("pp_adam_step");
    return 0;
}

}
```

### pyprob_amd/csrc/optim.hip

```cpp
#include "common.hpp"

namespace pp {

__global__ __launch_bounds__(256) void sgd_kernel(float* __restrict__ P, float* __restrict__ Gr, float* __restrict__ Mb,
                                                  const int32_t* __restrict__ chunk_tensor, const float* __restrict__ active,
                                                  float lr, float momentum, int nesterov, float wd, float gscale,
                                                  int zero_grads, const int32_t* __restrict__ skip) {
    const int b = blockIdx.x;
    const int t = chunk_tensor[b];
    if (t < 0 || !(active[t] > 0.0f)) return;
    const int64_t o = (int64_t)b * 1024 + threadIdx.x * 4;
    const f32x4 zero = f32x4{0.f, 0.f, 0.f, 0.f};
    if (skip && skip[0] != 0) {
        if (zero_grads) *reinterpret_cast<f32x4*>(Gr + o) = zero;
        return;
    }
    const f32x4 g0 = *reinterpret_cast<const f32x4*>(Gr + o);
    f32x4 p = *reinterpret_cast<const f32x4*>(P + o);
    f32x4 m = zero;
    const bool with_momentum = momentum != 0.0f;
    if (with_momentum) m = *reinterpret_cast<const f32x4*>(Mb + o);
#pragma unroll
    for (int e = 0; e < 4; ++e) {
        float g = g0[e] * gscale;
// ... 64 lines not shown
            const int mid = (lo + hi) >> 1;
            if (chunk_tensor[mid] < t) lo = mid + 1; else hi = mid;
        }
        int lo2 = lo, hi2 = n_chunks;
        while (lo2 < hi2) {
            const int mid = (lo2 + hi2) >> 1;
            if (chunk_tensor[mid] <= t) lo2 = mid + 1; else hi2 = mid;
        }
        s_run[0] = lo;
        s_run[1] = lo2;
    }
    __syncthreads();
    double sp = 0.0, sg = 0.0;
    for (int c = s_run[0] + (int)threadIdx.x; c < s_run[1]; c += 256) {
        sp += (double)partial[2 * (int64_t)c];
        sg += (double)partial[2 * (int64_t)c + 1];
    }
    sp = wave_sum(sp);
    sg = wave_sum(sg);
    const int w = threadIdx.x >> 6;
    if ((threadIdx.x & 63) == 0) {
        s_red[w] = sp;
        s_red[4 + w] = sg;
    }
    __syncthreads();
    if (threadIdx.x == 0) {
        const double pn = sqrt((s_red[0] + s_red[1]) + (s_red[2] + s_red[3]));
        const double gn = sqrt((s_red[4] + s_red[5]) + (s_red[6] + s_red[7])) * (double)gscale;
        double local = (double)epsilon;
        if (pn != 0.0 && gn != 0.0) local = (double)trust * pn / (gn + pn * (double)wd + (double)eps);
        const double adaptive = clip ? fmin(local / (double)lr, 1.0) : local;
        ratio[t] = (float)adaptive;
    }
}

__global__ __launch_bounds__(256) void larc_apply_kernel(const float* __restrict__ P, float* __restrict__ Gr,
                                                         const int32_t* __restrict__ chunk_tensor,
                                                         const float* __restrict__ active, const float* __restrict__ ratio,
                                                         float wd, float gscale, const int32_t* __restrict__ skip) {
    const int b = blockIdx.x;
    const int t = chunk_tensor[b];
    if (t < 0 || !(active[t] > 0.0f) || (skip && skip[0] != 0)) return;
    const int64_t o = (int64_t)b * 1024 + threadIdx.x * 4;
    f32x4 g = *reinterpret_cast<const f32x4*>(Gr + o);
    const float r = ratio[t];
    if (wd != 0.0f) {
        const f32x4 p = *reinterpret_cast<const f32x4*>(P + o);
#pragma unroll
        for (int e = 0; e < 4; ++e) g[e] = (g[e] * gscale + wd * p[e]) * r;
    } else {
#pragma unroll
        for (int e = 0; e < 4; ++e) g[e] = (g[e] * gscale) * r;
    }
    *reinterpret_cast<f32x4*>(Gr + o) = g;
}

int larc_scale(const float* params, float* grads, int64_t n_params, const int32_t* chunk_tensor, const float* active,
               int n_tensors, float lr, float wd, float gscale, float trust, float eps, float epsilon, int clip, float* scratch,
               const int32_t* skip, hipStream_t st) {
    PP_CHECK_ARG(params && grads && chunk_tensor && active && scratch, "pp_larc_scale: null pointer");
    PP_CHECK_ARG(n_params % 1024 == 0, "pp_larc_scale: n_params must be a multiple of 1024 (padded tensors)");
    PP_CHECK_ARG(lr > 0.0f || !clip, "pp_larc_scale: the clipping variant divides by the learning rate");
    if (n_tensors <= 0 || n_params == 0) return 0;
    const int n_chunks = (int)(n_params / 1024);
    float* partial = scratch;
    float* ratio = scratch + 2 * (int64_t)n_chunks;
    hipLaunchKernelGGL(larc_partial_kernel, dim3((unsigned)n_chunks), dim3(256), 0, st, params, grads, chunk_tensor, active, partial,
                       skip);
    hipLaunchKernelGGL(larc_ratio_kernel, dim3((unsigned)n_tensors), dim3(256), 0, st, chunk_tensor, n_chunks, active, partial, ratio,
                       lr, wd, gscale, trust, eps, epsilon, clip ? 1 : 0, skip);
    hipLaunchKernelGGL(larc_apply_kernel, dim3((unsigned)n_chunks), dim3(256), 0, st, params, grads, chunk_tensor, active, ratio, wd,
                       gscale, skip);
    PP_LAUNCH_CHECK("pp_larc_scale");
    return 0;
}

}

extern "C" {

int pp_sgd_step(float* params, float* grads, float* momentum_buf, int64_t n_params, const int32_t* chunk_tensor,
                const float* active, int32_t n_tensors, float lr, float momentum, int32_t nesterov, float weight_decay,
                float grad_scale, int32_t flags, const int32_t* skip, void* stream) {
    pp::prof_begin(3, pp::as_stream(stream));
    const int rc = pp::sgd_step(params, grads, momentum_buf, n_params, chunk_tensor, active, n_tensors, lr, momentum, nesterov,
                                weight_decay, grad_scale, flags, skip, pp::as_stream(stream));
    const double words = (momentum != 0.0f ? 5.0 : 3.0) + ((flags & PP_ADAM_ZERO_GRADS) ? 1.0 : 0.0);
    pp::prof_end(3, 4.0 * words * (double)n_params, pp::as_stream(stream));
    return rc;
}

int pp_larc_scale(const float* params, float* grads, int64_t n_params, const int32_t* chunk_tensor, const float* active,
                  int32_t n_tensors, float lr, float weight_decay, float grad_scale, float trust_coefficient, float eps,
                  float epsilon, int32_t clip, float* scratch, const int32_t* skip, void* stream) {
    return pp::larc_scale(params, grads, n_params, chunk_tensor, active, n_tensors, lr, weight_decay, grad_scale,
                          trust_coefficient, eps, epsilon, clip, scratch, skip, pp::as_stream(stream));
}

}
```

### pyprob_amd/csrc/train_loop.hip

```cpp
#include "common.hpp"

#include <algorithm>
#include <vector>

namespace pp {
void set_error(const char* fmt, ...);
int ic_loss(const pp_net* net, const pp_batch* bt, const float* P, float* grads, void* ws, size_t ws_bytes, float* loss_out,
            int32_t* status_out, float* lp_out, int flags, hipStream_t st);
int adam_step(float* params, float* grads, float* m, float* v, int64_t n_params, const int32_t* chunk_tensor,
              const float* active, int32_t* tensor_step, int32_t* arrived, int n_tensors, float lr, float beta1, float beta2,
              float eps, float wd, float gscale, int flags, const int32_t* skip, hipStream_t st);
int dp_world();
int dp_reduce_grads(float* grads_full, int64_t n_params, int n_tensors, const float* presence, const int32_t* status,
                    const int64_t* skip_off, const int64_t* skip_cnt, int n_skip, float* loss_out, int32_t* status_out,
                    hipStream_t st);
}

static hipEvent_t g_half_event[2];
static bool g_have_event[2] = {false, false};

extern "C" {

int64_t pp_train_slot_words(int32_t n_traces, int64_t n_rows, int32_t t_max, int32_t obs_width, int32_t n_addr,
                            int32_t n_tensors) {
    return ((pp_pack_words(n_traces, n_rows, t_max, obs_width, n_addr) + n_tensors + 63) / 64) * 64;
}

int pp_train_steps(const pp_net* net, const pp_train_buffers* tb, const pp_tensor_roles* roles,
                   const pp_shard_columns* shards, int32_t n_shards, const int64_t* first, int32_t obs_width,
                   const int64_t* ids, const int64_t* step_off, int32_t n_steps, const float* lr, float beta1, float beta2,
                   float eps, float weight_decay, int32_t grads_clean, int64_t* addr_iterations, void* stream) {
    if (!(net && tb && roles && shards && first && ids && step_off && lr) || n_steps < 0) {
        pp::set_error("pp_train_steps: null pointer");
        return PP_EINVAL;
    }
    if (!(tb->params && tb->grads && tb->exp_avg && tb->exp_avg_sq && tb->chunk_tensor && tb->tensor_step && tb->adam_scratch &&
          tb->workspace && tb->staging && tb->device_batch && tb->loss_ring && tb->status_ring) ||
        tb->n_slots < 1 || tb->n_slots > 64 || tb->slot_words <= 0 || tb->n_tensors <= 0) {
        pp::set_error("pp_train_steps: incomplete pp_train_buffers");
        return PP_EINVAL;
    }
    hipStream_t st = pp::as_stream(stream);
    const int n_addr = net->n_addr, n_tensors = tb->n_tensors;
    const bool dp = tb->dp_world >= 1;
    if (dp && (pp::dp_world() != tb->dp_world || tb->dp_n_skip < 0 || tb->dp_n_skip > 4)) {
        pp::set_error("pp_train_steps: dp_world %d but the communicator has %d ranks (pp_dp_init)", tb->dp_world, pp::dp_world());
        return PP_EINVAL;
    }
    float* const dp_tail = tb->grads + net->n_params;
    const int G = std::max(1, tb->n_slots / 2);
    hipEvent_t* ev = g_half_event;
    bool* have_ev = g_have_event;
    struct Packed { pp_pack_info info; int64_t words; };
    std::vector<Packed> pk(G);
    int rc = 0;
    for (int i = 0, gi = 0; i < n_steps && rc == 0; ++gi) {
        const int half = tb->n_slots >= 2 ? (gi & 1) : 0;
        const int gs = std::min({G, 1 << std::min(gi, 16), n_steps - i});
        if (!have_ev[half]) {
            if (hipEventCreateWithFlags(&ev[half], hipEventDisableTiming) != hipSuccess) {
                pp::set_error("pp_train_steps: hipEventCreate failed");
                rc = PP_EHIP;
                break;
            }
            have_ev[half] = true;
        } else {
            (void)hipEventSynchronize(ev[half]);
        }
        float* host0 = static_cast<float*>(tb->staging) + (int64_t)half * G * tb->slot_words;
        float* dev0 = static_cast<float*>(tb->device_batch) + (int64_t)half * G * tb->slot_words;
        for (int k = 0; k < gs && rc == 0; ++k) {
            float* host = host0 + (int64_t)k * tb->slot_words;
            const int32_t* hosti = reinterpret_cast<const int32_t*>(host);
            const int64_t n = step_off[i + k + 1] - step_off[i + k];
            if (n <= 0 || n > INT32_MAX) {
                pp::set_error("pp_train_steps: step %d has %lld traces", i + k, (long long)n);
                rc = PP_EINVAL;
                break;
            }
            pp_pack_info& info = pk[k].info;
            rc = pp_pack_indexed(shards, n_shards, first, ids + step_off[i + k], (int32_t)n, obs_width, n_addr, host,
                                 tb->slot_words - n_tensors, &info);
            if (rc != 0) break;
            pk[k].words = info.src_row + info.n_rows;
            const int32_t* goff = hosti + info.grp_off;
            const int32_t* noff = hosti + info.nxt_off;
            float* act = host + pk[k].words;
            for (int t = 0; t < n_tensors; ++t) {
                const int role = roles->role[t];
                bool on = role & 4;
                for (int q = roles->off[t]; q < roles->off[t + 1] && !on; ++q) {
                    const int a = roles->addr[q];
                    on = ((role & 1) && goff[a + 1] > goff[a]) || ((role & 2) && noff[a + 1] > noff[a]);
                }
                act[t] = on ? 1.0f : 0.0f;
            }
            if (addr_iterations)
                for (int a = 0; a < n_addr; ++a) addr_iterations[a] += goff[a + 1] > goff[a];
        }
        if (rc != 0) break;
        const size_t bytes = ((size_t)(gs - 1) * tb->slot_words + pk[gs - 1].words + n_tensors) * 4;
        if (hipMemcpyAsync(dev0, host0, bytes, hipMemcpyHostToDevice, st) != hipSuccess ||
            hipEventRecord(ev[half], st) != hipSuccess) {
            pp::set_error("pp_train_steps: upload failed: %s", hipGetErrorString(hipGetLastError()));
            rc = PP_EHIP;
            break;
        }
        for (int k = 0; k < gs && rc == 0; ++k, ++i) {
            const pp_pack_info& info = pk[k].info;
            const int32_t* hosti = reinterpret_cast<const int32_t*>(host0 + (int64_t)k * tb->slot_words);
            float* dev = dev0 + (int64_t)k * tb->slot_words;
            const int32_t* devi = reinterpret_cast<const int32_t*>(dev);
            pp_batch bt{};
            bt.n_traces = (int32_t)info.n_traces; bt.n_rows = (int32_t)info.n_rows; bt.t_max = (int32_t)info.t_max;
            bt.obs_width = obs_width;
            bt.n_active = hosti + info.n_active; bt.row_off = hosti + info.row_off;
            bt.grp_off = hosti + info.grp_off; bt.nxt_off = hosti + info.nxt_off;
            bt.obs = dev + info.obs; bt.value = dev + info.value; bt.prior = dev + info.prior;
            bt.addr = devi + info.addr; bt.prev_row = devi + info.prev_row; bt.grp_rows = devi + info.grp_rows;
            bt.trace = devi + info.trace; bt.row_off_dev = devi + info.row_off_dev; bt.nxt_rows = devi + info.nxt_rows;
            const int flags = PP_LOSS_BACKWARD | ((i == 0 && !grads_clean) ? PP_LOSS_ZERO_GRADS : 0);
            rc = pp::ic_loss(net, &bt, tb->params, tb->grads, tb->workspace, tb->workspace_bytes,
                             dp ? dp_tail + n_tensors : tb->loss_ring + i, tb->status_ring + i, nullptr, flags, st);
            if (rc != 0) break;
            if (dp) {
                rc = pp::dp_reduce_grads(tb->grads, net->n_params, n_tensors, dev + pk[k].words, tb->status_ring + i,
                                         tb->dp_skip_off, tb->dp_skip_cnt, tb->dp_n_skip, tb->loss_ring + i, tb->status_ring + i,
                                         st);
                if (rc != 0) break;
            }
            rc = pp::adam_step(tb->params, tb->grads, tb->exp_avg, tb->exp_avg_sq, net->n_params, tb->chunk_tensor,
                               dp ? dp_tail : dev + pk[k].words, tb->tensor_step, tb->adam_scratch, n_tensors, lr[i], beta1, beta2,
                               eps, weight_decay, dp ? 1.0f / (float)tb->dp_world : 1.0f, PP_ADAM_ZERO_GRADS,
                               tb->status_ring + i, st);
        }
    }
    return rc;
}

int pp_train_resident(const pp_net* net, const pp_train_buffers* tb, const pp_batch* const* batches, const float* const* active,
                      int32_t n_steps, const float* lr, float beta1, float beta2, float eps, float weight_decay,
                      int32_t grads_clean, void* stream) {
    if (!(net && tb && batches && active && lr) || n_steps < 0) {
        pp::set_error("pp_train_resident: null pointer");
        return PP_EINVAL;
    }
    if (!(tb->params && tb->grads && tb->exp_avg && tb->exp_avg_sq && tb->chunk_tensor && tb->tensor_step && tb->adam_scratch &&
          tb->workspace && tb->loss_ring && tb->status_ring) || tb->n_tensors <= 0) {
        pp::set_error("pp_train_resident: incomplete pp_train_buffers");
        return PP_EINVAL;
    }
    hipStream_t st = pp::as_stream(stream);
    const int n_tensors = tb->n_tensors;
    const bool dp = tb->dp_world >= 1;
    if (dp && (pp::dp_world() != tb->dp_world || tb->dp_n_skip < 0 || tb->dp_n_skip > 4)) {
        pp::set_error("pp_train_resident: dp_world %d but the communicator has %d ranks (pp_dp_init)", tb->dp_world, pp::dp_world());
        return PP_EINVAL;
    }
    float* const dp_tail = tb->grads + net->n_params;
    for (int i = 0; i < n_steps; ++i) {
        if (!batches[i] || !active[i]) {
            pp::set_error("pp_train_resident: step %d has no batch / presence map", i);
            return PP_EINVAL;
        }
        const int flags = PP_LOSS_BACKWARD | ((i == 0 && !grads_clean) ? PP_LOSS_ZERO_GRADS : 0);
        int rc = pp::ic_loss(net, batches[i], tb->params, tb->grads, tb->workspace, tb->workspace_bytes,
                             dp ? dp_tail + n_tensors : tb->loss_ring + i, tb->status_ring + i, nullptr, flags, st);
        if (rc != 0) return rc;
        if (dp) {
            rc = pp::dp_reduce_grads(tb->grads, net->n_params, n_tensors, active[i], tb->status_ring + i, tb->dp_skip_off,
                                     tb->dp_skip_cnt, tb->dp_n_skip, tb->loss_ring + i, tb->status_ring + i, st);
            if (rc != 0) return rc;
        }
        rc = pp::adam_step(tb->params, tb->grads, tb->exp_avg, tb->exp_avg_sq, net->n_params, tb->chunk_tensor,
                           dp ? dp_tail : active[i], tb->tensor_step, tb->adam_scratch, n_tensors, lr[i], beta1, beta2, eps,
                           weight_decay, dp ? 1.0f / (float)tb->dp_world : 1.0f, PP_ADAM_ZERO_GRADS, tb->status_ring + i, st);
        if (rc != 0) return rc;
    }
    return 0;
}

int pp_train_sync(void) {
    for (int h = 0; h < 2; ++h)
        if (g_have_event[h] && hipEventSynchronize(g_half_event[h]) != hipSuccess) {
            pp::set_error("pp_train_sync: %s", hipGetErrorString(hipGetLastError()));
            return PP_EHIP;
        }
    return 0;
}

}
```

### pyprob_amd/engine.py

```python
import ctypes as C

import numpy as np
import torch

from . import lib as L
from .spec import NetSpec


import os
_ADAM_CLEARS = os.environ.get('PP_ADAM_ZERO', '1') != '0'
import itertools
_engine_tokens = itertools.count(1)


class ICEngine:
    def __init__(self, spec: NetSpec, device='cuda:0', seed=None):
        self.lib = L.load()
        self.token = next(_engine_tokens)
        if not torch.cuda.is_available():
            raise L.HipLibraryError('pyprob_amd needs a ROCm device (torch.cuda.is_available() is False); there is '
                                    'no CPU fallback.')
        self.spec = spec
        self.device = torch.device(device)
        self.rng = np.random.default_rng(seed)
        self.params = torch.zeros(0, dtype=torch.float32, device=self.device)
        self.workspace = None
        self.ws_bytes = 0
        self.ws_shape = (0, 0)
        self.status_buf = torch.zeros(4, dtype=torch.int32, device=self.device)
        self.world_size = 1
        self.force_allreduce = False
        self.optimizer = dict(kind='adam', larc=False, momentum=0.9)
        self._resize(initialise=list(spec.tensors.keys()))

    def _resize(self, initialise):
        spec = self.spec
        n = spec.n_params
        new = torch.zeros(n + 1024, dtype=torch.float32, device=self.device)[:n]
        old_n = self.params.numel()
        if old_n:
            new[:old_n].copy_(self.params)
        host = {}
        for name in initialise:
            host[name] = spec.init_tensor(name, self.rng)
        self.params = new
        for name, arr in host.items():
            self.set_tensor(name, arr)
        self.grads_full = torch.zeros(n + spec.n_tensors + 2, dtype=torch.float32, device=self.device)
        self.grads = self.grads_full[:n]
        self.active = self.grads_full[n:n + spec.n_tensors]
        self.loss_buf = self.grads_full[n + spec.n_tensors:n + spec.n_tensors + 1]
        self.status_tail = self.grads_full[n + spec.n_tensors + 1:]
        self.dp_skip = []
        self.dp_overlap = getattr(self, 'dp_overlap', [])
        self.native_dp = getattr(self, 'native_dp', False)
        self.exp_avg = torch.zeros(n, dtype=torch.float32, device=self.device)
        self.exp_avg_sq = torch.zeros(n, dtype=torch.float32, device=self.device)
        self.tensor_step = torch.zeros(spec.n_tensors, dtype=torch.int32, device=self.device)
        self.arrived = torch.zeros(L.PP_ADAM_SCRATCH * spec.n_tensors, dtype=torch.int32, device=self.device)
        self._grads_clean = False
        self.chunk_tensor = torch.from_numpy(spec.chunk_tensor_map()).to(self.device)
        self.addr_table = torch.from_numpy(spec.address_table()).to(self.device)
        self.net = spec.c_struct(self.addr_table.data_ptr())
        from . import ops
        ops.unregister_net(getattr(self, 'net_handle', None))
        self.net_handle = ops.register_net(self.net, spec)
        self._active_cache = {}
        self._active_key = None
        self.ws_shape = (0, 0)

    def add_addresses(self, items):
        created = []
        for address, dist_name, ncat in items:
            created += self.spec.add_address(address, dist_name, ncat)
        if created:
            self._resize(initialise=created)
        return bool(created)

    def _ensure_workspace(self, n_traces, n_rows):
        if n_traces <= self.ws_shape[0] and n_rows <= self.ws_shape[1]:
            return
        bt, br = max(n_traces, self.ws_shape[0]), max(n_rows, self.ws_shape[1])
        need = self.lib.pp_ic_workspace_bytes(C.byref(self.net), bt, br)
        if need == 0:
            raise RuntimeError('pp_ic_workspace_bytes failed: %s' % self.lib.pp_last_error().decode())
        self.workspace = torch.zeros(need, dtype=torch.uint8, device=self.device)
        self.ws_bytes = need
        self.ws_shape = (bt, br)

    def tensor(self, name, buf=None):
        off, shape = self.spec.tensors[name]
        buf = self.params if buf is None else buf
        return buf[off:off + int(np.prod(shape))].view(shape)

    def set_tensor(self, name, array):
        t = torch.as_tensor(np.asarray(array, np.float32)).to(self.device)
        self.tensor(name).copy_(t.view(self.spec.tensors[name][1]))

    def state_dict(self):
        return {name: self.tensor(name).detach().cpu().clone() for name in self.spec.tensors}

    def load_state_dict(self, sd):
        for name in self.spec.tensors:
            self.set_tensor(name, sd[name].detach().cpu().numpy() if hasattr(sd[name], 'detach') else sd[name])

    def grad_dict(self):
        return {name: self.tensor(name, self.grads).detach().cpu().numpy().copy() for name in self.spec.tensors}

    def loss(self, batch, backward=False, keep_lp=False, zero_grads=True, loss_out=None, status_out=None):
        if batch.c is None:
            batch.to(self.device)
        self._ensure_workspace(batch.n_traces, batch.n_rows)
        flags = 0
        if backward:
            flags |= L.PP_LOSS_BACKWARD
            if zero_grads and not self._grads_clean:
                flags |= L.PP_LOSS_ZERO_GRADS
            self._grads_clean = False
        lp = None
        if keep_lp:
            flags |= L.PP_LOSS_KEEP_LP
            lp = torch.empty(batch.n_rows, dtype=torch.float32, device=self.device)
        if getattr(self, '_use_ops', False):
            from .ops import ops
            bdev, bhost = batch.op_tensors(self.device)
            l_, s_, lp_ = ops.ic_loss(self.params, self.grads, self.workspace, bdev, bhost, self.net_handle, flags)
            (self.loss_buf if loss_out is None else loss_out)[:1].copy_(l_)
            (self.status_buf if status_out is None else status_out)[:1].copy_(s_)
            if keep_lp:
                lp.copy_(lp_)
        else:
            rc = self.lib.pp_ic_loss(C.byref(self.net), C.byref(batch.c), self.params.data_ptr(),
                                     self.grads.data_ptr() if backward else None, self.workspace.data_ptr(), self.ws_bytes,
                                     (self.loss_buf if loss_out is None else loss_out).data_ptr(),
                                     (self.status_buf if status_out is None else status_out).data_ptr(), L.ptr(lp), flags,
                                     L.stream_ptr())
            L.check(rc, 'pp_ic_loss')
        if backward:
            self._set_active(batch)
        return (self.loss_buf[:1], lp) if keep_lp else self.loss_buf[:1]

    def _set_active(self, batch):
        key = batch.presence_key
        if key == self._active_key and self.world_size == 1 and not self.force_allreduce:
            return
        act = self._active_cache.get(key)
        if act is None:
            act = torch.from_numpy(self.spec.active_mask(batch.cur_counts, batch.prev_counts)).to(self.device)
            self._active_cache[key] = act
        if self.world_size == 1 and not self.force_allreduce:
            self._presence = act
        else:
            self.active.copy_(act)
            self._presence = self.active
        self._active_key = key

    def presence(self):
        return self._presence if self._active_key is not None else self.active

    def adam_step(self, lr, beta1=0.9, beta2=0.999, eps=1e-8, weight_decay=0.0, zero_grads=False, skip=None, grad_scale=None):
        gs = 1.0 / self.world_size if grad_scale is None else grad_scale
        if getattr(self, '_use_ops', False):
            from .ops import ops
            ops.adam_step(self.params, self.grads, self.exp_avg, self.exp_avg_sq, self.chunk_tensor, self.presence(),
                          self.tensor_step, self.arrived, lr, beta1, beta2, eps, weight_decay, gs,
                          L.PP_ADAM_ZERO_GRADS if zero_grads else 0, skip)
        else:
            rc = self.lib.pp_adam_step(self.params.data_ptr(), self.grads.data_ptr(), self.exp_avg.data_ptr(),
                                       self.exp_avg_sq.data_ptr(), self.spec.n_params, self.chunk_tensor.data_ptr(),
                                       self.presence().data_ptr(), self.tensor_step.data_ptr(), self.arrived.data_ptr(),
                                       self.spec.n_tensors, lr, beta1, beta2, eps, weight_decay, gs,
                                       L.PP_ADAM_ZERO_GRADS if zero_grads else 0, L.ptr(skip), L.stream_ptr())
            L.check(rc, 'pp_adam_step')
        self._grads_clean = bool(zero_grads)

    def set_optimizer(self, kind='adam', larc=False, momentum=0.9):
        kind = str(kind).lower()
        if kind not in ('adam', 'sgd'):
            raise ValueError('unknown optimizer {!r} (adam | sgd)'.format(kind))
        self.optimizer = dict(kind=kind, larc=bool(larc), momentum=float(momentum))
        self.reset_optimizer()

    def sgd_step(self, lr, momentum=0.9, nesterov=True, weight_decay=0.0, zero_grads=False, skip=None, grad_scale=None):
        gs = 1.0 / self.world_size if grad_scale is None else grad_scale
        flags = L.PP_ADAM_ZERO_GRADS if zero_grads else 0
        if getattr(self, '_use_ops', False):
            from .ops import ops
            ops.sgd_step(self.params, self.grads, self.exp_avg, self.chunk_tensor, self.presence(), float(lr), float(momentum),
                         bool(nesterov), float(weight_decay), float(gs), flags, skip)
        else:
            rc = self.lib.pp_sgd_step(self.params.data_ptr(), self.grads.data_ptr(), self.exp_avg.data_ptr(), self.spec.n_params,
                                      self.chunk_tensor.data_ptr(), self.presence().data_ptr(), self.spec.n_tensors, lr, momentum,
                                      int(bool(nesterov)), weight_decay, gs, flags, L.ptr(skip), L.stream_ptr())
            L.check(rc, 'pp_sgd_step')
        self._grads_clean = bool(zero_grads)

    def larc_scale(self, lr, weight_decay=0.0, skip=None, trust_coefficient=0.002, clip=True, eps=1e-8, epsilon=1.0 / 16000.0):
        need = L.larc_scratch_floats(self.spec.n_params, self.spec.n_tensors)
        if getattr(self, '_larc_scratch', None) is None or self._larc_scratch.numel() < need:
            self._larc_scratch = torch.empty(need, dtype=torch.float32, device=self.device)
        if getattr(self, '_use_ops', False):
            from .ops import ops
            ops.larc_scale(self.params, self.grads, self.chunk_tensor, self.presence(), float(lr), float(weight_decay),
                           1.0 / self.world_size, float(trust_coefficient), float(eps), float(epsilon), bool(clip),
                           self._larc_scratch, skip)
        else:
            rc = self.lib.pp_larc_scale(self.params.data_ptr(), self.grads.data_ptr(), self.spec.n_params,
                                        self.chunk_tensor.data_ptr(), self.presence().data_ptr(), self.spec.n_tensors, lr, weight_decay,
                                        1.0 / self.world_size, trust_coefficient, eps, epsilon, int(bool(clip)),
                                        self._larc_scratch.data_ptr(), L.ptr(skip), L.stream_ptr())
            L.check(rc, 'pp_larc_scale')

    def optimizer_step(self, lr, weight_decay=0.0, zero_grads=False, skip=None):
        opt = self.optimizer
        scale = None
        if opt['larc']:
            self.larc_scale(lr, weight_decay, skip=skip)
            weight_decay, scale = 0.0, 1.0
        if opt['kind'] == 'sgd':
            self.sgd_step(lr, opt['momentum'], True, weight_decay, zero_grads, skip, grad_scale=scale)
        elif scale is None:
            self.adam_step(lr, weight_decay=weight_decay, zero_grads=zero_grads, skip=skip)
        else:
            self.adam_step(lr, weight_decay=0.0, zero_grads=zero_grads, skip=skip, grad_scale=1.0)

    def _adam_only(self, what):
        if self.optimizer['kind'] != 'adam' or self.optimizer['larc']:
            raise RuntimeError('{} runs Optimizer.ADAM; other optimizers step through train_step'.format(what))

    def train_step(self, batch, lr, weight_decay=0.0):
        loss = self.loss(batch, backward=True)
        if self.world_size > 1 or self.force_allreduce:
            self.allreduce_grads()
            self.optimizer_step(lr, weight_decay=weight_decay, zero_grads=_ADAM_CLEARS, skip=self.reduced_status())
        else:
            self.optimizer_step(lr, weight_decay=weight_decay, zero_grads=_ADAM_CLEARS, skip=self.status_buf)
        return loss

    def train_run(self, dataset, id_lists, lrs, weight_decay=0.0, beta1=0.9, beta2=0.999, eps=1e-8):
        self._adam_only('train_run (pp_train_steps)')
        dp = self.world_size != 1 or self.force_allreduce
        if dp and not (self.native_dp and self.lib.pp_dp_world() == self.world_size):
            raise RuntimeError('train_run under data parallelism needs the native RCCL communicator '
                               '(pyprob_amd.parallel.init_native_comm); without it the steps go through train_step')
        n_steps = len(id_lists)
        spec = self.spec
        shards, n_shards, first = dataset.native_columns(spec)
        sizes = np.fromiter((len(x) for x in id_lists), np.int64, n_steps)
        step_off = np.concatenate([[0], np.cumsum(sizes)]).astype(np.int64)
        ids = np.ascontiguousarray(np.concatenate([np.asarray(x, np.int64).reshape(-1) for x in id_lists]))
        if ids.size == 0 or np.any(sizes <= 0):
            raise ValueError('empty batch')
        if np.any(ids < 0) or np.any(ids >= len(dataset.trace_len)):
            raise IndexError('trace index out of range')
        lens = dataset.trace_len[ids].astype(np.int64)
        b_max, t_max = int(sizes.max()), int(lens.max())
        r_max = int(np.add.reduceat(lens, step_off[:-1]).max())
        self._ensure_workspace(b_max, r_max)
        key = (id(spec), spec.n_tensors)
        if getattr(self, '_roles_key', None) != key:
            off, addr, role = spec.tensor_roles()
            self._roles_arrays = (off, addr, role)
            self._roles = L.pp_tensor_roles(off.ctypes.data, addr.ctypes.data, role.ctypes.data)
            self._roles_key = key
        n_slots = 16
        slot_words = int(self.lib.pp_train_slot_words(b_max, r_max, t_max, dataset.obs_width, len(spec.addresses),
                                                      spec.n_tensors))
        if getattr(self, '_slot_words', 0) < slot_words:
            L.check(self.lib.pp_train_sync(), 'pp_train_sync')
            torch.cuda.synchronize(self.device)
            self._staging = torch.empty(n_slots * slot_words, dtype=torch.float32).pin_memory()
            self._device_batch = torch.empty(n_slots * slot_words, dtype=torch.float32, device=self.device)
            self._slot_words = slot_words
        if getattr(self, '_ring_n', 0) < n_steps:
            self._ring_n = max(n_steps, 64)
            self._loss_ring = torch.zeros(self._ring_n, dtype=torch.float32, device=self.device)
            self._status_ring = torch.zeros(self._ring_n, dtype=torch.int32, device=self.device)
        tb = L.pp_train_buffers(self.params.data_ptr(), self.grads.data_ptr(), self.exp_avg.data_ptr(),
                                self.exp_avg_sq.data_ptr(), self.chunk_tensor.data_ptr(), self.tensor_step.data_ptr(),
                                self.arrived.data_ptr(), self.workspace.data_ptr(), self.ws_bytes,
                                self._staging.data_ptr(), self._device_batch.data_ptr(), self._slot_words,
                                self._loss_ring.data_ptr(), self._status_ring.data_ptr(), spec.n_tensors, n_slots)
        if dp:
            tb.dp_world, tb.dp_n_skip = self.world_size, len(self.dp_skip)
            for k, (off, cnt) in enumerate(self.dp_skip):
                tb.dp_skip_off[k], tb.dp_skip_cnt[k] = off, cnt
        lr = np.ascontiguousarray(lrs, np.float32).reshape(-1)
        if len(lr) != n_steps:
            raise ValueError('one learning rate per step')
        iters = np.zeros(max(len(spec.addresses), 1), np.int64)
        rc = self.lib.pp_train_steps(C.byref(self.net), C.byref(tb), C.byref(self._roles), shards, n_shards,
                                     first.ctypes.data, dataset.obs_width, ids.ctypes.data, step_off.ctypes.data, n_steps,
                                     lr.ctypes.data, beta1, beta2, eps, weight_decay, 1 if self._grads_clean else 0,
                                     iters.ctypes.data, L.stream_ptr())
        if rc != 0:
            msg = self.lib.pp_last_error().decode()
            self._grads_clean = False
            if 'address' in msg:
                raise KeyError('Address unknown by inference network ({})'.format(msg))
            raise RuntimeError('pp_train_steps failed (rc=%d): %s' % (rc, msg))
        self._grads_clean = True
        self._active_key = None
        for a, k in enumerate(iters[:len(spec.addresses)]):
            spec.addresses[a].total_train_iterations += int(k)
        return self._loss_ring[:n_steps], self._status_ring[:n_steps]

    def train_resident(self, batches, lrs, weight_decay=0.0, beta1=0.9, beta2=0.999, eps=1e-8):
        n_steps = len(batches)
        self._adam_only('train_resident (pp_train_resident)')
        dp = self.world_size != 1 or self.force_allreduce
        if dp and not (self.native_dp and self.lib.pp_dp_world() == self.world_size):
            raise RuntimeError('train_resident under data parallelism needs the native RCCL communicator')
        b_max = max(b.n_traces for b in batches)
        r_max = max(b.n_rows for b in batches)
        self._ensure_workspace(b_max, r_max)
        if getattr(self, '_ring_n', 0) < n_steps:
            self._ring_n = max(n_steps, 64)
            self._loss_ring = torch.zeros(self._ring_n, dtype=torch.float32, device=self.device)
            self._status_ring = torch.zeros(self._ring_n, dtype=torch.int32, device=self.device)
# ... 9 lines not shown
            acts.append(act)
        bptr = (C.c_void_p * n_steps)(*[C.addressof(b.c) for b in batches])
        aptr = (C.c_void_p * n_steps)(*[a.data_ptr() for a in acts])
        lr = np.ascontiguousarray(lrs, np.float32).reshape(-1)
        if len(lr) != n_steps:
            raise ValueError('one learning rate per step')
        tb = L.pp_train_buffers(self.params.data_ptr(), self.grads.data_ptr(), self.exp_avg.data_ptr(),
                                self.exp_avg_sq.data_ptr(), self.chunk_tensor.data_ptr(), self.tensor_step.data_ptr(),
                                self.arrived.data_ptr(), self.workspace.data_ptr(), self.ws_bytes, None, None, 0,
                                self._loss_ring.data_ptr(), self._status_ring.data_ptr(), self.spec.n_tensors, 0)
        if dp:
            tb.dp_world, tb.dp_n_skip = self.world_size, len(self.dp_skip)
            for k, (off, cnt) in enumerate(self.dp_skip):
                tb.dp_skip_off[k], tb.dp_skip_cnt[k] = off, cnt
        rc = self.lib.pp_train_resident(C.byref(self.net), C.byref(tb), bptr, aptr, n_steps, lr.ctypes.data, beta1, beta2, eps,
                                        weight_decay, 1 if self._grads_clean else 0, L.stream_ptr())
        L.check(rc, 'pp_train_resident')
        self._grads_clean = True
        self._active_key = None
        return self._loss_ring[:n_steps], self._status_ring[:n_steps]

    def read_back(self, losses, statuses):
        n = losses.numel()
        pool = getattr(self, '_readback_pool', None)
        if pool is None:
            pool = self._readback_pool = []
        k = getattr(self, '_readback_next', 0)
        self._readback_next = k + 1
        if len(pool) < 4:
            pool.append(None)
        slot = k % len(pool)
        if pool[slot] is None or pool[slot][0].numel() < n:
            pool[slot] = (torch.empty(max(n, 64), dtype=torch.float32).pin_memory(),
                          torch.empty(max(n, 64), dtype=torch.int32).pin_memory(), torch.cuda.Event())
        h_loss, h_status, event = pool[slot]
        h_loss[:n].copy_(losses, non_blocking=True)
        h_status[:n].copy_(statuses, non_blocking=True)
        event.record()

        def wait():
            event.synchronize()
            return h_loss[:n].numpy().copy(), h_status[:n].numpy().copy()
        return wait

    def capture_train_step(self, batch, lr, weight_decay=0.0):
        self._ensure_workspace(batch.n_traces, batch.n_rows)
        self.loss(batch, backward=True)
        self.adam_step(lr, weight_decay=weight_decay)
        torch.cuda.synchronize()
        g1 = torch.cuda.CUDAGraph()
        if self.world_size == 1:
            with torch.cuda.graph(g1):
                self.loss(batch, backward=True)
                self.adam_step(lr, weight_decay=weight_decay)
            self._graphs = (g1, None)
        else:
            g2 = torch.cuda.CUDAGraph()
            with torch.cuda.graph(g1):
                self.loss(batch, backward=True)
            with torch.cuda.graph(g2):
                self.adam_step(lr, weight_decay=weight_decay)
            self._graphs = (g1, g2)
        return self._graphs

    def replay_train_step(self):
        g1, g2 = self._graphs
        g1.replay()
        if g2 is not None:
            self.allreduce_grads()
            g2.replay()
        return self.loss_buf[:1]

    def allreduce_grads(self):
        if self.native_dp and self.lib.pp_dp_world() == self.world_size and not self.grads_full.is_cpu:
            n = self.grads.numel()
            k = len(self.dp_skip)
            off = (C.c_int64 * max(k, 1))(*[o for o, _ in self.dp_skip])
            cnt = (C.c_int64 * max(k, 1))(*[c for _, c in self.dp_skip])
            L.check(self.lib.pp_dp_reduce_grads(self.grads_full.data_ptr(), n, self.spec.n_tensors, None,
                                                self.status_buf.data_ptr(), off, cnt, k, None, None, L.stream_ptr()),
                    'pp_dp_reduce_grads')
            return
        from .parallel import allreduce_flat_
        self.status_tail.copy_(self.status_buf[:1])
        if self.dp_overlap:
            import torch.distributed as dist
            from .parallel import allreduce_pieces_
            early = [dist.all_reduce(self.grads_full[o:o + c], async_op=True) for o, c in self.dp_overlap]
            pieces, pos = [], 0
            for off, cnt in sorted(list(self.dp_skip) + list(self.dp_overlap)):
                if off > pos:
                    pieces.append((pos, off))
                pos = off + cnt
            pieces.append((pos, self.grads_full.numel()))
            allreduce_pieces_([self.grads_full[a:b] for a, b in pieces if b > a])
            for work in early:
                work.wait()
            return
        if not self.dp_skip:
            allreduce_flat_(self.grads_full)
            return
        pieces, pos = [], 0
        for off, cnt in self.dp_skip:
            if off > pos:
                pieces.append((pos, off))
            pos = off + cnt
        pieces.append((pos, self.grads_full.numel()))
        from .parallel import allreduce_pieces_
        allreduce_pieces_([self.grads_full[a:b] for a, b in pieces])

    def reduced_status(self):
        return self.status_tail.view(torch.int32)

    def skip_recurrent_weights(self, enable=True):
        self.dp_skip = []
        if enable and not self.spec.feedforward:
            off, shape = self.spec.tensors['_layers_lstm.weight_hh_l0']
            n = int(np.prod(shape))
            self.dp_skip = [(off, ((n + 1023) // 1024) * 1024)]

    def enable_dp_overlap(self, enable=True):
        self.dp_overlap = []
        if enable and not self.spec.feedforward and os.environ.get('PP_DP_OVERLAP', '0') == '1':
            names = ['_layers_lstm.weight_ih_l0', '_layers_lstm.weight_hh_l0', '_layers_lstm.bias_ih_l0', '_layers_lstm.bias_hh_l0']
            pieces = []
            for n in names:
                off, shape = self.spec.tensors[n]
                cnt = ((int(np.prod(shape)) + 1023) // 1024) * 1024
                if any(o <= off and off + cnt <= o + c for o, c in self.dp_skip):
                    continue
                if pieces and pieces[-1][0] + pieces[-1][1] == off:
                    pieces[-1] = (pieces[-1][0], pieces[-1][1] + cnt)
                else:
                    pieces.append((off, cnt))
            self.dp_overlap = pieces[:2] if len(pieces) <= 2 else []
        if self.native_dp and not self.grads_full.is_cpu and self.lib.pp_dp_world() >= 1:
            k = len(self.dp_overlap)
            off = (C.c_int64 * max(k, 1))(*[o for o, _ in self.dp_overlap])
            cnt = (C.c_int64 * max(k, 1))(*[c for _, c in self.dp_overlap])
            L.check(self.lib.pp_dp_overlap(off, cnt, k), 'pp_dp_overlap')
        return list(self.dp_overlap)

    def agree_skip_recurrent(self, single_statement):
        flag = 1 if single_statement else 0
        if self.world_size > 1:
            import torch.distributed as dist
            if dist.is_available() and dist.is_initialized():
                dev = self.device if dist.get_backend() == 'nccl' else 'cpu'
                t = torch.tensor([flag], dtype=torch.int32, device=dev)
                dist.all_reduce(t, op=dist.ReduceOp.MIN)
                flag = int(t.item())
        self.skip_recurrent_weights(bool(flag))
        if self.world_size > 1 or self.force_allreduce:
            self.enable_dp_overlap(True)
        return bool(flag)

    def broadcast_params(self):
        import torch.distributed as dist
        dist.broadcast(self.params, 0)

    def reset_optimizer(self):
        self.exp_avg.zero_()
        self.exp_avg_sq.zero_()
        self.tensor_step.zero_()
        self.arrived.view(-1, L.PP_ADAM_SCRATCH)[:, L.PP_ADAM_SEEN] = 0

    def moments_written(self):
        self.arrived.view(-1, L.PP_ADAM_SCRATCH)[:, L.PP_ADAM_SEEN] = 1
```

### pyprob_amd/lib.py

```python
import ctypes as C
import os

HERE = os.path.dirname(os.path.abspath(__file__))
LIB_PATH = os.path.join(HERE, 'libpyprob_amd.so')

PP_ABI_VERSION = 15
PP_MAX_OBS = 8
PP_MAX_LSTM_DEPTH = 4
PP_MAX_OBS_DEPTH = 4
PP_MAX_MIXTURE_COMPONENTS = 16
PP_ADDR_TABLE_COLS = 8
PP_HEAD_NORMAL_MIXTURE, PP_HEAD_TRUNCNORMAL_MIXTURE, PP_HEAD_CATEGORICAL, PP_HEAD_POISSON_TN_MIXTURE = 0, 1, 2, 3
PP_HEAD_BERNOULLI = 4
PP_OBS_FEEDFORWARD, PP_OBS_CNN2D5C = 0, 1
PP_PROF_CNN_FWD, PP_PROF_CNN_BWD = 32, 48
PP_LOSS_BACKWARD, PP_LOSS_ZERO_GRADS, PP_LOSS_KEEP_LP = 1, 2, 4
PP_ADAM_ZERO_GRADS = 1
PP_ADAM_SCRATCH = 1056
PP_ADAM_SEEN = 1027


def larc_scratch_floats(n_params, n_tensors):
    return 2 * (int(n_params) // 1024) + int(n_tensors)

# ... 47 lines not shown


class pp_lw_term(C.Structure):
    _fields_ = [('kind', i32), ('p0_stride', i32), ('p1_stride', i32), ('x_stride', i32),
                ('p0', vp), ('p1', vp), ('x', vp), ('scale', C.c_float)]


PP_DIST_MAX_TERMS = 8
PP_DIST_MAX_ROUNDS = 64


class pp_dist(C.Structure):
    _fields_ = [('kind', i32), ('p_stride', i32 * 4), ('p', vp * 4)]


class pp_dist_term(C.Structure):
    _fields_ = [('d', pp_dist), ('x', vp), ('x_stride', i32), ('scale', C.c_float)]


PP_MIX_MAX_COMPONENTS = 16
PP_OBS_PER_GROUP_X = 16


class pp_mixture(C.Structure):
    _fields_ = [('count', i32), ('probs_stride', i32), ('probs', vp), ('comp', pp_dist * PP_MIX_MAX_COMPONENTS)]


class pp_obs_operand(C.Structure):
    _fields_ = [('p', vp), ('row_stride', i64), ('elem_stride', i32), ('_pad', i32)]


class pp_gemm_args(C.Structure):
    _fields_ = [('A', vp), ('lda', i64), ('a_idx', vp),
                ('B', vp), ('ldb', i64), ('b_idx', vp),
                ('C', vp), ('ldc', i64), ('c_idx', vp),
                ('M', i32), ('N', i32), ('K', i32), ('a_kmajor', i32), ('b_kmajor', i32),
                ('bias', vp), ('bias2', vp), ('mask', vp), ('ldmask', i64), ('relu', i32), ('accumulate', i32),
                ('colsum', vp), ('split_k', i32), ('_pad', i32)]


class pp_pack_info(C.Structure):
    _fields_ = [(n, i64) for n in ('n_traces', 'n_rows', 't_max', 'device_words', 'obs', 'value', 'prior', 'addr', 'prev_row',
                                   'grp_rows', 'trace', 'row_off_dev', 'nxt_rows', 'n_active', 'row_off', 'grp_off',
                                   'nxt_off', 'order', 'src_row')]


class pp_shard_columns(C.Structure):
    _fields_ = [(n, vp) for n in ('trace_len', 'row_off', 'obs', 'value', 'prior', 'addr', 'addr_remap')]


class pp_train_buffers(C.Structure):
    _fields_ = [('params', vp), ('grads', vp), ('exp_avg', vp), ('exp_avg_sq', vp),
                ('chunk_tensor', vp), ('tensor_step', vp), ('adam_scratch', vp),
                ('workspace', vp), ('workspace_bytes', C.c_size_t),
                ('staging', vp), ('device_batch', vp), ('slot_words', i64),
                ('loss_ring', vp), ('status_ring', vp), ('n_tensors', i32), ('n_slots', i32),
                ('dp_world', i32), ('dp_n_skip', i32), ('dp_skip_off', i64 * 4), ('dp_skip_cnt', i64 * 4)]


class pp_tensor_roles(C.Structure):
    _fields_ = [('off', vp), ('addr', vp), ('role', vp)]


PROTOTYPES = {
    'pp_train_slot_words': (i64, [i32, i64, i32, i32, i32, i32]),
    'pp_train_sync': (C.c_int, []),
    'pp_train_resident': (C.c_int, [C.POINTER(pp_net), C.POINTER(pp_train_buffers), vp, vp, i32, vp, C.c_float, C.c_float,
                                    C.c_float, C.c_float, i32, vp]),
    'pp_train_steps': (C.c_int, [C.POINTER(pp_net), C.POINTER(pp_train_buffers), C.POINTER(pp_tensor_roles), vp, i32, vp, i32,
                                 vp, vp, i32, vp, C.c_float, C.c_float, C.c_float, C.c_float, i32, vp, vp]),
    'pp_pack_indexed': (C.c_int, [vp, i32, vp, vp, i32, i32, i32, vp, i64, vp]),
    'pp_pack_words': (i64, [i32, i64, i32, i32, i32]),
    'pp_pack_ragged': (C.c_int, [vp, vp, vp, vp, i32, vp, i32, i32, i32, vp, i64, vp]),
    'pp_cnn2d5c_workspace_bytes': (C.c_size_t, [C.POINTER(pp_net), i32, i32]),
    'pp_cnn2d5c_forward': (C.c_int, [C.POINTER(pp_net), i32, vp, vp, i32, vp, vp, C.c_size_t, vp]),
    'pp_cnn2d5c_backward': (C.c_int, [C.POINTER(pp_net), i32, vp, vp, i32, vp, vp, C.c_size_t, i32, vp]),
    'pp_abi_version': (C.c_int, []),
    'pp_last_error': (C.c_char_p, []),
    'pp_device_count': (C.c_int, []),
    'pp_ic_workspace_bytes': (C.c_size_t, [C.POINTER(pp_net), i32, i32]),
    'pp_ic_loss': (C.c_int, [C.POINTER(pp_net), C.POINTER(pp_batch), vp, vp, vp, C.c_size_t, vp, vp, vp, i32, vp]),
    'pp_adam_step': (C.c_int, [vp, vp, vp, vp, i64, vp, vp, vp, vp, i32, C.c_float, C.c_float, C.c_float, C.c_float,
                               C.c_float, C.c_float, i32, vp, vp]),
    'pp_sgd_step': (C.c_int, [vp, vp, vp, i64, vp, vp, i32, C.c_float, C.c_float, i32, C.c_float, C.c_float, i32, vp, vp]),
    'pp_larc_scale': (C.c_int, [vp, vp, i64, vp, vp, i32, C.c_float, C.c_float, C.c_float, C.c_float, C.c_float, C.c_float,
                                i32, vp, vp, vp]),
    'pp_is_workspace_bytes': (C.c_size_t, [C.POINTER(pp_net), i32]),
    'pp_is_init': (C.c_int, [C.POINTER(pp_net), vp, vp, vp, vp, C.c_size_t, vp]),
    'pp_is_step': (C.c_int, [C.POINTER(pp_net), vp, i32, i32, i32, vp, vp, vp, i32, vp, vp, i32, vp, vp, vp, C.c_uint64,
                             C.c_uint64, vp, C.c_size_t, vp]),
    'pp_is_step_rows': (C.c_int, [C.POINTER(pp_net), vp, i32, i32, i32, vp, vp, vp, i32, vp, vp, i32, vp, vp, vp, vp, C.c_uint64,
                                  C.c_uint64, vp, C.c_size_t, vp]),
    'pp_is_step_fused_supported': (C.c_int, [C.POINTER(pp_net), i32, i32]),
    'pp_is_statement_rows': (C.c_int, [C.POINTER(pp_net), vp, i32, i32, i32, vp, vp, vp, i32, vp, vp, i32, vp, vp, vp, i32,
                                       C.c_uint64, C.c_uint64, vp, C.c_size_t, vp]),
    'pp_prior_draw': (C.c_int, [i32, vp, i32, vp, i32, i32, C.c_uint64, C.c_uint64, C.c_uint32, vp, vp]),
    'pp_obs_draw': (C.c_int, [i32, vp, C.c_int64, i32, vp, C.c_int64, i32, i32, i32, C.c_uint64, C.c_uint64, C.c_uint32, vp, vp]),
    'pp_is_first_statement_supported': (C.c_int, [C.POINTER(pp_net), i32]),
    'pp_is_first_statement': (C.c_int, [C.POINTER(pp_net), vp, vp, i32, vp, vp, vp, vp, C.c_size_t, vp]),
    'pp_is_step_net': (C.c_int, [C.POINTER(pp_net), vp, i32, i32, i32, vp, vp, vp, vp, i32, vp, C.c_size_t, vp]),
    'pp_is_fused': (C.c_int, [C.POINTER(pp_net), i32, i32, vp, C.POINTER(pp_lw_term), C.POINTER(C.c_int32), i32, vp, vp, i32,
                              C.c_uint64, C.c_uint64, vp, vp, vp, C.c_size_t, vp]),
    'pp_is_batch_workspace_bytes': (C.c_size_t, [C.POINTER(pp_net), i32]),
    'pp_is_batch_first': (C.c_int, [C.POINTER(pp_net), vp, vp, i32, i32, vp, i64, vp, vp, vp, C.c_size_t, vp]),
    'pp_is_fused_groups': (C.c_int, [C.POINTER(pp_net), i32, i32, i32, vp, i64, vp, C.POINTER(pp_lw_term), C.POINTER(C.c_int32), i32,
                                     vp, vp, i32, C.c_uint64, C.c_uint64, vp, vp, C.c_size_t, vp]),
    'pp_is_batch_bias': (C.c_int, [C.POINTER(pp_net), vp, i32, i32, i32, i32, i32, vp, vp, vp, C.c_size_t, vp]),
    'pp_is_statement_groups': (C.c_int, [C.POINTER(pp_net), vp, i32, i32, i32, i32, vp, vp, vp, vp, i32, vp, vp, vp, vp, i32,
                                         C.c_uint64, C.c_uint64, vp, i64, vp, C.c_size_t, vp]),
    'pp_is_cdf_workspace_bytes': (C.c_size_t, [i32, i32]),
    'pp_is_cdf_groups': (C.c_int, [vp, i32, i32, vp, vp, vp, C.c_size_t, vp]),
    'pp_is_resample_groups': (C.c_int, [vp, vp, i32, i32, i32, i32, i32, C.c_uint64, C.c_uint64, vp, vp, vp]),
    'pp_is_moments_workspace_bytes': (C.c_size_t, [i32, i32, i32]),
    'pp_is_moments_groups': (C.c_int, [vp, vp, i32, i32, i32, vp, vp, vp, C.c_size_t, vp]),
    'pp_is_hist_shift': (i32, [i32]),
    'pp_is_hist_workspace_bytes': (C.c_size_t, [i32, i32, i32, i32]),
    'pp_is_hist_groups': (C.c_int, [vp, vp, vp, i32, i32, vp, i32, i64, vp, i32, i64, vp, vp, vp, C.c_size_t, vp]),
    'pp_is_extent_workspace_bytes': (C.c_size_t, [i32, i32]),
    'pp_is_extent_groups': (C.c_int, [vp, vp, i32, i32, vp, vp, C.c_size_t, vp]),
    'pp_logweight_accumulate': (C.c_int, [i32, vp, i32, vp, i32, vp, i32, C.c_float, vp, vp, i32, vp]),
    'pp_logweight_accumulate_rows': (C.c_int, [i32, vp, i32, vp, i32, vp, i32, C.c_float, vp, vp, i32, vp]),
    'pp_copy_rows': (C.c_int, [vp, i32, vp, vp, i32, vp]),
    'pp_partition_rows': (C.c_int, [vp, vp, i32, vp, vp, vp, vp, vp]),
    'pp_partition_rows_polled': (C.c_int, [vp, vp, i32, vp, vp, vp, i32, vp, vp]),
    'pp_logweight_terms': (C.c_int, [C.POINTER(pp_lw_term), i32, vp, i32, i32, vp]),
    'pp_axpy': (C.c_int, [C.c_float, vp, vp, i32, vp]),
    'pp_is_stats': (C.c_int, [vp, vp, i32, vp, vp, vp]),
    'pp_dist_logweight': (C.c_int, [C.POINTER(pp_dist_term), i32, vp, vp, vp, i32, i32, vp]),
    'pp_dist_draw': (C.c_int, [C.POINTER(pp_dist), vp, i32, i32, C.c_uint64, C.c_uint64, C.c_uint32, vp, vp]),
    'pp_mix_logweight': (C.c_int, [C.POINTER(pp_mixture), vp, i32, C.c_float, vp, vp, vp, i32, i32, vp]),
    'pp_obs_logweight': (C.c_int, [i32, C.POINTER(pp_obs_operand), pp_obs_operand, i32, C.c_float, vp, vp, vp, i32, i32, vp]),
    'pp_obs_logweight_groups': (C.c_int, [i32, C.POINTER(pp_obs_operand), pp_obs_operand, i32, i32, C.c_float, vp, vp, i32, i32, vp]),
    'pp_mix_draw': (C.c_int, [C.POINTER(pp_mixture), vp, i32, i32, C.c_uint64, C.c_uint64, C.c_uint32, vp, vp]),
    'pp_gemm_f32': (C.c_int, [C.POINTER(pp_gemm_args), vp]),
    'pp_gemm_f32_grouped': (C.c_int, [C.POINTER(pp_gemm_args), i32, vp]),
    'pp_colsum_f32': (C.c_int, [vp, i64, vp, i32, i32, vp, vp, vp]),
    'pp_lstm_input_gather': (C.c_int, [C.POINTER(pp_net), vp, vp, vp, vp, vp, vp, i32, vp, i64, vp]),
    'pp_lstm_cell_fwd': (C.c_int, [vp, vp, vp, vp, i32, i32, vp]),
    'pp_lstm_cell_bwd': (C.c_int, [vp, vp, vp, vp, vp, i32, i32, i32, vp]),
    'pp_head_logprob': (C.c_int, [i32, vp, i64, vp, vp, vp, i32, i32, C.c_float, vp, vp, vp, vp, vp]),
    'pp_debug_clock_probe': (C.c_int, [i32, vp, vp, vp]),
    'pp_dp_unique_id': (C.c_int, [C.c_char_p, vp]),
    'pp_dp_init': (C.c_int, [C.c_char_p, vp, i32, i32]),
    'pp_dp_world': (C.c_int, []),
    'pp_dp_destroy': (C.c_int, []),
    'pp_dp_allreduce': (C.c_int, [vp, vp, vp, i32, vp]),
    'pp_dp_reduce_grads': (C.c_int, [vp, i64, i32, vp, vp, vp, vp, i32, vp, vp, vp]),
    'pp_dp_overlap': (C.c_int, [vp, vp, i32]),
    'pp_dp_overlap_stats': (C.c_int, [i32, vp]),
    'pp_debug_timeline': (C.c_int, [vp]),
    'pp_debug_wgtrace': (C.c_int, [vp, C.c_int32, C.c_int32]),
    'pp_debug_wgrad_plan': (C.c_int, [vp, vp, i32, vp, i32, vp]),
    'pp_debug_wgrad_run': (C.c_int, [vp, vp, i32, i32, vp, vp, i32]),
    'pp_prof_arm': (C.c_int, [i32, i32]),
    'pp_prof_stride': (C.c_int, [i32]),
    'pp_prof_collect': (C.c_int, [vp, i32, vp, vp]),
}

_lib = None


class HipLibraryError(RuntimeError):
    pass


def load():
# ... 43 lines not shown
```

Baseline: 16.99 million traces/s.

## Restrict Adam step to tensors whose gradients were actually written

Adds host-side tracking of which parameter tensors had gradients written since the last clean state, and builds a cached run/gap plan so the Adam kernel processes only the contiguous runs of touched tensors. Untouched tensors (zero grads, with no weight decay) can then be skipped instead of streamed through the full optimizer. Every gradient-writing entry point now marks the tensors it touches, which adds host bookkeeping per launch and risks wrong updates if a writer is missed. Because Adam momentum still moves parameters even when gradients are zero, the skipped tensors need separate handling, for example the gap bookkeeping.

Result: faster. 17.23 million traces/s, median of 6 (+1.4%).

```diff
diff --git a/include/pyprob_amd.h b/include/pyprob_amd.h
--- a/include/pyprob_amd.h
+++ b/include/pyprob_amd.h
@@ -159,6 +159,21 @@
                  int32_t n_tensors, float lr, float beta1, float beta2, float eps, float weight_decay, float grad_scale,
                  int32_t flags, const int32_t* skip, void* stream);
 
+int pp_adam_step_live(float* params, float* grads, float* exp_avg, float* exp_avg_sq, int64_t n_params,
+                      const int32_t* chunk_tensor, const float* active, int32_t* tensor_step, int32_t* scratch,
+                      int32_t n_tensors, float lr, float beta1, float beta2, float eps, float weight_decay, float grad_scale,
+                      int32_t flags, const int32_t* skip, void* stream);
+int pp_adam_live_bind(const float* grads , const float* exp_avg , const float* exp_avg_sq , int64_t n_params,
+                      const int32_t* tensor_first , int32_t n_tensors, int32_t clean);
+int pp_adam_live_unbind(const float* grads);
+int pp_adam_live_mark_touched(const void* buffer);
+int pp_adam_live_mark_range(const float* grads, int64_t offset, int64_t count);
+int pp_adam_live_info(const float* grads, int64_t* out , uint8_t* touched_out );
+int pp_adam_live_plan(const int32_t* tensor_first , int32_t n_tensors, const uint8_t* live ,
+                      int32_t* out );
+int pp_adam_live_table(const float* grads, const float* exp_avg, const float* exp_avg_sq, int64_t n_params, int32_t n_tensors,
+                       float weight_decay, int32_t* out );
+
 int pp_sgd_step(float* params, float* grads, float* momentum_buf, int64_t n_params, const int32_t* chunk_tensor,
                 const float* active, int32_t n_tensors, float lr, float momentum, int32_t nesterov, float weight_decay,
                 float grad_scale, int32_t flags, const int32_t* skip, void* stream);
diff --git a/pyprob_amd/autograd.py b/pyprob_amd/autograd.py
--- a/pyprob_amd/autograd.py
+++ b/pyprob_amd/autograd.py
@@ -27,6 +27,7 @@
         flags = L.PP_LOSS_BACKWARD | (0 if network._hip_grads_clean else L.PP_LOSS_ZERO_GRADS)
         batch_dev, batch_host = packed.op_tensors(eng.device)
         eng._ensure_workspace(packed.n_traces, packed.n_rows)
+        eng.mark_touched()
         loss, status, _ = ops.ic_loss(eng.params, eng.grads, eng.workspace, batch_dev, batch_host, eng.net_handle, flags)
         network._hip_grads_clean = False
         network._hip_status = status
diff --git a/pyprob_amd/csrc/adam_live.hpp b/pyprob_amd/csrc/adam_live.hpp
--- /dev/null
+++ b/pyprob_amd/csrc/adam_live.hpp
@@ -0,0 +1,94 @@
+#pragma once
+#include <cstdint>
+#include <vector>
+
+namespace pp {
+
+constexpr int ADAM_LIVE_MAX_RUNS = 4;
+
+struct AdamLiveTable {
+    int n_runs;
+    int live_blocks;
+    int run_blk[ADAM_LIVE_MAX_RUNS];
+    int run_chunk[ADAM_LIVE_MAX_RUNS];
+    int n_gaps;
+    int gap_t0[ADAM_LIVE_MAX_RUNS + 1], gap_t1[ADAM_LIVE_MAX_RUNS + 1];
+};
+
+inline bool adam_live_plan(const int32_t* first, int n_tensors, const uint8_t* live, AdamLiveTable& tab) {
+    tab = AdamLiveTable{};
+    int blk = 0;
+    for (int t = 0; t < n_tensors;) {
+        int e = t;
+        while (e < n_tensors && (live[e] != 0) == (live[t] != 0)) ++e;
+        if (live[t]) {
+            if (first[e] > first[t]) {
+                if (tab.n_runs == ADAM_LIVE_MAX_RUNS) return false;
+                tab.run_blk[tab.n_runs] = blk;
+                tab.run_chunk[tab.n_runs] = first[t];
+                ++tab.n_runs;
+                blk += first[e] - first[t];
+            }
+        } else {
+            if (tab.n_gaps == ADAM_LIVE_MAX_RUNS + 1) return false;
+            tab.gap_t0[tab.n_gaps] = t;
+            tab.gap_t1[tab.n_gaps] = e;
+            ++tab.n_gaps;
+        }
+        t = e;
+    }
+    tab.live_blocks = blk;
+    return true;
+}
+
+struct GradTrack {
+    const float* grads = nullptr;
+    const float* m = nullptr;
+    const float* v = nullptr;
+    int64_t n_params = 0;
+    int n_tensors = 0;
+    std::vector<int32_t> first;
+    std::vector<uint8_t> touched;
+    uint64_t version = 1;
+    uint64_t plan_version = 0;
+    int plan_key = -1;
+    bool plan_ok = false;
+    AdamLiveTable plan{};
+    uint64_t builds = 0;
+
+    int tensor_of_chunk(int64_t c) const {
+        int lo = 0, hi = n_tensors;
+        while (hi - lo > 1) {
+            const int mid = (lo + hi) >> 1;
+            if (first[mid] <= c) lo = mid; else hi = mid;
+        }
+        return lo;
+    }
+    void touch_tensor(int t) {
+        if (!touched[t]) {
+            touched[t] = 1;
+            ++version;
+        }
+    }
+    void touch_all() {
+        for (int t = 0; t < n_tensors; ++t) touch_tensor(t);
+    }
+    void touch_offset(int64_t off) {
+        if (off >= 0 && off < n_params && n_tensors > 0) touch_tensor(tensor_of_chunk(off >> 10));
+    }
+    bool table(bool wd_on, const AdamLiveTable** out) {
+        const int key = wd_on ? 1 : 0;
+        if (plan_version != version || plan_key != key) {
+            std::vector<uint8_t> live(touched);
+            if (wd_on) live.assign(live.size(), 1);
+            plan_ok = adam_live_plan(first.data(), n_tensors, live.data(), plan);
+            plan_version = version;
+            plan_key = key;
+            ++builds;
+        }
+        *out = &plan;
+        return plan_ok;
+    }
+};
+
+}
diff --git a/pyprob_amd/csrc/cnn2d.hip b/pyprob_amd/csrc/cnn2d.hip
--- a/pyprob_amd/csrc/cnn2d.hip
+++ b/pyprob_amd/csrc/cnn2d.hip
@@ -522,6 +522,7 @@
     pp::CnnGeom g;
     PP_CHECK_ARG(pp::cnn_geom(net, o, g), "pp_cnn2d5c_backward: observable %d is not a CNN2D5C embedding", o);
     PP_CHECK_ARG(flags == 0, "pp_cnn2d5c_backward: flags must be 0");
+    pp::grads_touch_all(grads);
     (void)params;
     return pp::cnn_backward(net, o, d_features, g.F, n_images, grads, workspace, workspace_bytes, pp::as_stream(stream));
 }
diff --git a/pyprob_amd/csrc/common.hpp b/pyprob_amd/csrc/common.hpp
--- a/pyprob_amd/csrc/common.hpp
+++ b/pyprob_amd/csrc/common.hpp
@@ -17,6 +17,10 @@
 typedef float f32x16 __attribute__((ext_vector_type(16)));
 
 void set_error(const char* fmt, ...);
+
+void grads_touch(const float* ptr);
+void grads_touch_range(const float* grads, int64_t off, int64_t cnt);
+void grads_touch_all(const void* ptr);
 
 #define PP_CHECK_ARG(cond, ...)          \
     do {                                 \
diff --git a/pyprob_amd/csrc/dp.hip b/pyprob_amd/csrc/dp.hip
--- a/pyprob_amd/csrc/dp.hip
+++ b/pyprob_amd/csrc/dp.hip
@@ -137,6 +137,14 @@
                     hipStream_t st) {
     PP_CHECK_ARG(g_rccl.comm && grads_full && status && n_params > 0 && n_tensors >= 0 && n_skip >= 0 && n_skip <= 6 && (!g_ov.pending || n_skip <= 4),
                  "pp_dp_reduce_grads: bad argument");
+    {
+        int64_t pos = 0;
+        for (int i = 0; i < n_skip; ++i) {
+            grads_touch_range(grads_full, pos, skip_off[i] - pos);
+            pos = skip_off[i] + skip_cnt[i];
+        }
+        grads_touch_range(grads_full, pos, n_params - pos);
+    }
     float* tail = grads_full + n_params;
     hipLaunchKernelGGL(dp_tail_pre_kernel, dim3(1), dim3(256), 0, st, tail, presence, n_tensors, status);
     PP_LAUNCH_CHECK("pp_dp_reduce_grads (tail)");
@@ -268,6 +276,7 @@
 }
 
 int pp_dp_allreduce(float* base, const int64_t* off, const int64_t* cnt, int32_t n, void* stream) {
+    for (int i = 0; base && off && cnt && i < n; ++i) pp::grads_touch_range(base, off[i], cnt[i]);
     return pp::dp_allreduce_pieces(base, off, cnt, n, pp::as_stream(stream));
 }
 
diff --git a/pyprob_amd/csrc/engine.hip b/pyprob_amd/csrc/engine.hip
--- a/pyprob_amd/csrc/engine.hip
+++ b/pyprob_amd/csrc/engine.hip
@@ -5,6 +5,7 @@
 #include "panel16.hpp"
 #include "wgrad_t1.hpp"
 #include "cnn2d.hpp"
+#include "adam_live.hpp"
 
 #include <stdlib.h>
 #include <string.h>
@@ -61,6 +62,15 @@
 int adam_step(float* params, float* grads, float* m, float* v, int64_t n_params, const int32_t* chunk_tensor,
               const float* active, int32_t* tensor_step, int32_t* arrived, int n_tensors, float lr, float beta1, float beta2,
               float eps, float wd, float gscale, int flags, const int32_t* skip, hipStream_t st);
+int adam_step_live(float* params, float* grads, float* m, float* v, int64_t n_params, const int32_t* chunk_tensor,
+                   const float* active, int32_t* tensor_step, int32_t* arrived, int n_tensors, float lr, float beta1, float beta2,
+                   float eps, float wd, float gscale, int flags, const int32_t* skip, hipStream_t st);
+int adam_live_bind(const float* grads, const float* m, const float* v, int64_t n_params, const int32_t* first, int n_tensors,
+                   bool clean);
+void adam_live_unbind(const float* grads);
+bool adam_live_table(const float* grads, const float* m, const float* v, int64_t n_params, int n_tensors, bool wd_on,
+                     AdamLiveTable& tab);
+int adam_live_info(const float* grads, int64_t* out, uint8_t* touched_out);
 
 extern long long* g_timeline;
 
@@ -793,6 +803,8 @@
         float* dZ1 = w.dZ1 + (int64_t)g0 * w.hid4;
         queue_head_wgrads(s, q, a);
         if (!head_tail_supported(ad.kind, ad.hid, ad.n_out)) {
+            grads_touch(grads + ad.b2);
+            grads_touch(grads + ad.b1);
             PP_TRY(colsum_f32(DY, w.out4, nullptr, n, ad.n_out, grads + ad.b2, nullptr, st));
             PP_TRY(linear_dgrad(DY, w.out4, P + ad.w2, dZ1, w.hid4, nullptr, A1, w.hid4, n, ad.hid, ad.n_out, false, st,
                                 p.det ? nullptr : grads + ad.b1));
@@ -845,6 +857,8 @@
     const float* Whh = s.P + ly.w_hh;
     float* db_ih = p.det ? nullptr : s.grads + ly.b_ih;
     float* db_hh = p.det ? nullptr : s.grads + ly.b_hh;
+    if (db_ih) grads_touch(db_ih);
+    if (db_hh) grads_touch(db_hh);
     LossFinalize fin = p.fin;
     if (l != p.L - 1) fin.acc = nullptr;
     int dh_parts = 0;
@@ -954,6 +968,7 @@
             }
         }
     }
+    if (T > 1) grads_touch_all(grads);
     if (T > 1 && p.det)
         PP_TRY(sample_embed_bwd_det(net, P, bt->value, bt->prev_row, bt->nxt_rows, bt->nxt_off, w.dX, w.i4, grads, st));
     else if (T > 1)
@@ -1002,6 +1017,22 @@
     const pp_net* net = s.net; const StepPlan& p = s.p;
     const bool ride = step_env().aux_colsum;
     AuxJobs aux{};
+    for (const auto& g : q.wq) grads_touch(g.C);
+    for (const auto& j : q.cs) {
+        grads_touch(j.out);
+        if (j.out2) grads_touch(j.out2);
+    }
+    if (p.compact) {
+        grads_touch(s.grads + net->w_ih);
+        for (int a = 0; a < net->n_addr; ++a) {
+            grads_touch(s.grads + net->addrs[a].addr_emb);
+            grads_touch(s.grads + net->addrs[a].dtype_emb);
+        }
+        if (p.fused_bwd) {
+            grads_touch(s.grads + net->b_ih);
+            grads_touch(s.grads + net->b_hh);
+        }
+    }
     if (!p.compact) {
         if (p.ff && !p.det && ride && !q.wq.empty() && colsums_ride(q.cs, aux)) {
             aux.fin = p.fin;
@@ -1066,6 +1097,7 @@
     const int B = p.B, e = net->e_obs;
     int64_t ldxs;
     const float* dXs = obs_grad_rows(s, &ldxs);
+    grads_touch_all(grads);
     PP_TRY(obs_grad(dXs, ldxs, bt->row_off_dev, p.T, B, e, w.E, w.e4, w.dE, w.e4, st));
     PP_TRY(reduce_and_flush(s, q));
     PP_TRY(linear_wgrad(w.dE, w.e4, w.f1, w.e4, nullptr, grads + net->fin_w1, grads + net->fin_b1, nullptr, B, e, e, st));
@@ -1189,6 +1221,7 @@
                  const int32_t* chunk_tensor, const float* active, int32_t* tensor_step, int32_t* arrived, int32_t n_tensors,
                  float lr, float beta1, float beta2, float eps, float weight_decay, float grad_scale, int32_t flags,
                  const int32_t* skip, void* stream) {
+    pp::grads_touch_all(grads);
     pp::prof_begin(3, pp::as_stream(stream));
     const int rc = pp::adam_step(params, grads, exp_avg, exp_avg_sq, n_params, chunk_tensor, active, tensor_step, arrived,
                                  n_tensors, lr, beta1, beta2, eps, weight_decay, grad_scale, flags, skip, pp::as_stream(stream));
@@ -1196,8 +1229,71 @@
     return rc;
 }
 
+int pp_adam_step_live(float* params, float* grads, float* exp_avg, float* exp_avg_sq, int64_t n_params,
+                      const int32_t* chunk_tensor, const float* active, int32_t* tensor_step, int32_t* arrived, int32_t n_tensors,
+                      float lr, float beta1, float beta2, float eps, float weight_decay, float grad_scale, int32_t flags,
+                      const int32_t* skip, void* stream) {
+    pp::prof_begin(3, pp::as_stream(stream));
+    const int rc = pp::adam_step_live(params, grads, exp_avg, exp_avg_sq, n_params, chunk_tensor, active, tensor_step, arrived,
+                                      n_tensors, lr, beta1, beta2, eps, weight_decay, grad_scale, flags, skip,
+                                      pp::as_stream(stream));
+    pp::prof_end(3, ((flags & PP_ADAM_ZERO_GRADS) ? 32.0 : 28.0) * (double)n_params, pp::as_stream(stream));
+    return rc;
+}
+
+int pp_adam_live_bind(const float* grads, const float* exp_avg, const float* exp_avg_sq, int64_t n_params,
+                      const int32_t* tensor_first, int32_t n_tensors, int32_t clean) {
+    return pp::adam_live_bind(grads, exp_avg, exp_avg_sq, n_params, tensor_first, n_tensors, clean != 0);
+}
+
+int pp_adam_live_unbind(const float* grads) {
+    pp::adam_live_unbind(grads);
+    return 0;
+}
+
+int pp_adam_live_mark_touched(const void* buffer) {
+    pp::grads_touch_all(buffer);
+    return 0;
+}
+
+int pp_adam_live_mark_range(const float* grads, int64_t offset, int64_t count) {
+    pp::grads_touch_range(grads, offset, count);
+    return 0;
+}
+
+int pp_adam_live_info(const float* grads, int64_t* out, uint8_t* touched_out) {
+    if (!out) return PP_EINVAL;
+    return pp::adam_live_info(grads, out, touched_out);
+}
+
+static void adam_table_words(const pp::AdamLiveTable& tab, int32_t* out) {
+    int k = 0;
+    out[k++] = tab.n_runs; out[k++] = tab.live_blocks; out[k++] = tab.n_gaps;
+    for (int r = 0; r < pp::ADAM_LIVE_MAX_RUNS; ++r) { out[k++] = tab.run_blk[r]; out[k++] = tab.run_chunk[r]; }
+    for (int g = 0; g <= pp::ADAM_LIVE_MAX_RUNS; ++g) { out[k++] = tab.gap_t0[g]; out[k++] = tab.gap_t1[g]; }
+}
+
+int pp_adam_live_plan(const int32_t* tensor_first, int32_t n_tensors, const uint8_t* live, int32_t* out) {
+    if (!(tensor_first && live && out) || n_tensors <= 0) return PP_EINVAL;
+    pp::AdamLiveTable tab;
+    if (!pp::adam_live_plan(tensor_first, n_tensors, live, tab)) return 1;
+    adam_table_words(tab, out);
+    return 0;
+}
+
+int pp_adam_live_table(const float* grads, const float* exp_avg, const float* exp_avg_sq, int64_t n_params, int32_t n_tensors,
+                       float weight_decay, int32_t* out) {
+    if (!out) return PP_EINVAL;
+    pp::AdamLiveTable tab;
+    if (!pp::adam_live_table(grads, exp_avg, exp_avg_sq, n_params, n_tensors, weight_decay != 0.0f, tab)) return 1;
+    adam_table_words(tab, out);
+    return 0;
+}
+
 int pp_colsum_f32(const float* X, int64_t ldx, const int32_t* row_idx, int32_t n_rows, int32_t n_cols, float* out,
                   float* out2, void* stream) {
+    pp::grads_touch_all(out);
+    pp::grads_touch_all(out2);
     return pp::colsum_f32(X, ldx, row_idx, n_rows, n_cols, out, out2, pp::as_stream(stream));
 }
 
diff --git a/pyprob_amd/csrc/gemm_f32.hip b/pyprob_amd/csrc/gemm_f32.hip
--- a/pyprob_amd/csrc/gemm_f32.hip
+++ b/pyprob_amd/csrc/gemm_f32.hip
@@ -1679,7 +1679,11 @@
     return 0;
 }
 
-extern "C" int pp_gemm_f32(const pp_gemm_args* args, void* stream) { return pp::gemm_f32(args, pp::as_stream(stream), nullptr, nullptr); }
+extern "C" int pp_gemm_f32(const pp_gemm_args* args, void* stream) {
+    if (args) pp::grads_touch_all(args->C);
+    return pp::gemm_f32(args, pp::as_stream(stream), nullptr, nullptr);
+}
 extern "C" int pp_gemm_f32_grouped(const pp_gemm_args* args, int32_t count, void* stream) {
+    for (int i = 0; args && i < count; ++i) pp::grads_touch_all(args[i].C);
     return pp::gemm_f32_grouped(args, count, pp::as_stream(stream), nullptr, nullptr, nullptr);
 }
diff --git a/pyprob_amd/csrc/is_kernels.hip b/pyprob_amd/csrc/is_kernels.hip
--- a/pyprob_amd/csrc/is_kernels.hip
+++ b/pyprob_amd/csrc/is_kernels.hip
@@ -1521,6 +1521,7 @@
 int pp_axpy(float scale, const float* term, float* lw, int32_t n, void* stream) {
     if (!(term && lw)) return PP_EINVAL;
     if (n <= 0) return 0;
+    pp::grads_touch_all(lw);
     hipLaunchKernelGGL(pp::axpy_kernel, dim3(pp::cdiv(n, 256)), dim3(256), 0, pp::as_stream(stream), scale, term, lw, n);
     PP_LAUNCH_CHECK("pp_axpy");
     return 0;
diff --git a/pyprob_amd/csrc/kernels.hip b/pyprob_amd/csrc/kernels.hip
--- a/pyprob_amd/csrc/kernels.hip
+++ b/pyprob_amd/csrc/kernels.hip
@@ -2,12 +2,14 @@
 #include "gather.hpp"
 #include "head_math.hpp"
 #include "aux_jobs.hpp"
+#include "adam_live.hpp"
 
 #include <math.h>
 #include <stdarg.h>
 #include <stdlib.h>
 
 #include <algorithm>
+#include <mutex>
 #include <vector>
 
 namespace pp {
@@ -1029,18 +1031,83 @@
 constexpr int ADAM_TOP = 1024, ADAM_FIRST = 1025, ADAM_CHUNKS = 1026;
 constexpr int ADAM_SEEN = 1027;
 
+#define ADAM_STAMP(k, lane0) do { if (tr && threadIdx.x == (lane0)) { __builtin_amdgcn_sched_barrier(0); tr[k] = wall_clock64(); __builtin_amdgcn_sched_barrier(0); } } while (0)
+#define ADAM_STAMP_ARRIVED(k, lane0) do { if (tr) { asm volatile("s_waitcnt vmcnt(0) lgkmcnt(0)" ::: "memory"); ADAM_STAMP(k, lane0); } } while (0)
+
+__device__ __forceinline__ void adam_corrections(int step, float lr, float beta1, float beta2, float* corr) {
+    double p1 = 1.0, p2 = 1.0, q1 = (double)beta1, q2 = (double)beta2;
+    for (int e = step; e > 0; e >>= 1) {
+        if (e & 1) { p1 *= q1; p2 *= q2; }
+        q1 *= q1;
+        q2 *= q2;
+    }
+    const double bc1 = 1.0 - p1, bc2 = 1.0 - p2;
+    corr[0] = (float)((double)lr / bc1);
+    corr[1] = (float)(1.0 / sqrt(bc2));
+}
+
+__device__ __forceinline__ void adam_update_store(float* __restrict__ P, float* __restrict__ Gr, float* __restrict__ M,
+                                                  float* __restrict__ V, int64_t o, uint32_t buf_bytes, uint32_t wo, f32x4 g0,
+                                                  f32x4 p, f32x4 m, f32x4 v, float step_size, float inv_sqrt_bc2, float beta1,
+                                                  float beta2, float eps, float wd, float gscale, int zero_grads, int wt) {
+    const f32x4 zero4 = f32x4{0.f, 0.f, 0.f, 0.f};
+#pragma unroll
+    for (int e = 0; e < 4; ++e) {
+        float g = g0[e] * gscale;
+        if (wd != 0.0f) g += wd * p[e];
+        m[e] = beta1 * m[e] + (1.0f - beta1) * g;
+        v[e] = beta2 * v[e] + (1.0f - beta2) * g * g;
+        const float denom = sqrtf(v[e]) * inv_sqrt_bc2 + eps;
+        p[e] -= step_size * (m[e] / denom);
+    }
+    if (wt) {
+        store16_wt(P, buf_bytes, wo, p);
+        store16_wt(M, buf_bytes, wo, m);
+        store16_wt(V, buf_bytes, wo, v);
+        if (zero_grads) store16_wt(Gr, buf_bytes, wo, zero4);
+    } else {
+        *reinterpret_cast<f32x4*>(P + o) = p;
+        *reinterpret_cast<f32x4*>(M + o) = m;
+        *reinterpret_cast<f32x4*>(V + o) = v;
+        if (zero_grads) *reinterpret_cast<f32x4*>(Gr + o) = zero4;
+    }
+}
+
+__device__ __forceinline__ void adam_find_run(const int32_t* __restrict__ chunk_tensor, int n_chunks, int t, int b, int& first,
+                                              int& chunks) {
+    int lo = 0, hi = b;
+    while (lo < hi) {
+        const int mid = (lo + hi) >> 1;
+        if (chunk_tensor[mid] < t) lo = mid + 1; else hi = mid;
+    }
+    int lo2 = b, hi2 = n_chunks;
+    while (lo2 < hi2) {
+        const int mid = (lo2 + hi2) >> 1;
+        if (chunk_tensor[mid] <= t) lo2 = mid + 1; else hi2 = mid;
+    }
+    first = lo;
+    chunks = lo2 - lo;
+}
+
 __global__ __launch_bounds__(256) void adam_kernel(float* __restrict__ P, float* __restrict__ Gr, float* __restrict__ M,
                                                    float* __restrict__ V, const int32_t* __restrict__ chunk_tensor,
                                                    int n_chunks, const float* __restrict__ active,
                                                    int32_t* __restrict__ tensor_step, int32_t* __restrict__ scratch, float lr,
                                                    float beta1, float beta2, float eps, float wd, float gscale,
-                                                   int zero_grads, const int32_t* __restrict__ skip, int wt) {
+                                                   int zero_grads, const int32_t* __restrict__ skip, int wt,
+                                                   long long* __restrict__ trace) {
     __shared__ float s_corr[2];
+    long long* const tr = trace ? trace + 8 * (int64_t)blockIdx.x : nullptr;
+    ADAM_STAMP(0, 0);
     const uint32_t buf_bytes = (uint32_t)n_chunks * 4096u, wo = ((uint32_t)blockIdx.x * 1024u + threadIdx.x * 4u) * 4u;
     const f32x4 zero4 = f32x4{0.f, 0.f, 0.f, 0.f};
     const int b = blockIdx.x;
     const bool skipped = skip && skip[0] != 0;
     const int t = chunk_tensor[b];
+    if (tr) {
+        asm volatile("" ::"s"(t));
+        ADAM_STAMP(1, 0);
+    }
     if (t < 0 || !(active[t] > 0.0f)) return;
     if (skipped) {
         if (zero_grads) {
@@ -1064,6 +1131,7 @@
     } else if (!seen && threadIdx.x == 0) {
         __atomic_store_n(sc + ADAM_SEEN, 1, __ATOMIC_RELAXED);
     }
+    ADAM_STAMP_ARRIVED(2, 0);
     f32x4 p = f32x4{0.f, 0.f, 0.f, 0.f}, m = p, v = p;
     if (!idle) {
         p = *reinterpret_cast<f32x4*>(P + o);
@@ -1074,60 +1142,22 @@
     if (threadIdx.x == 0) {
         first = __atomic_load_n(sc + ADAM_FIRST, __ATOMIC_RELAXED) - 1;
         chunks = __atomic_load_n(sc + ADAM_CHUNKS, __ATOMIC_RELAXED);
-        if (first < 0) {
-            int lo = 0, hi = b;
-            while (lo < hi) {
-                const int mid = (lo + hi) >> 1;
-                if (chunk_tensor[mid] < t) lo = mid + 1; else hi = mid;
-            }
-            int lo2 = b, hi2 = n_chunks;
-            while (lo2 < hi2) {
-                const int mid = (lo2 + hi2) >> 1;
-                if (chunk_tensor[mid] <= t) lo2 = mid + 1; else hi2 = mid;
-            }
-            first = lo;
-            chunks = lo2 - lo;
-        }
+        if (first < 0) adam_find_run(chunk_tensor, n_chunks, t, b, first, chunks);
         step_old = __atomic_load_n(tensor_step + t, __ATOMIC_RELAXED);
-        const int step = step_old + 1;
-        double p1 = 1.0, p2 = 1.0, q1 = (double)beta1, q2 = (double)beta2;
-        for (int e = step; e > 0; e >>= 1) {
-            if (e & 1) { p1 *= q1; p2 *= q2; }
-            q1 *= q1;
-            q2 *= q2;
-        }
-        const double bc1 = 1.0 - p1, bc2 = 1.0 - p2;
-        s_corr[0] = (float)((double)lr / bc1);
-        s_corr[1] = (float)(1.0 / sqrt(bc2));
-    }
+        adam_corrections(step_old + 1, lr, beta1, beta2, s_corr);
+    }
+    ADAM_STAMP_ARRIVED(3, 64);
     __syncthreads();
+    ADAM_STAMP(4, 0);
     const float step_size = s_corr[0], inv_sqrt_bc2 = s_corr[1];
     const int k = (b - first) & 31;
     const int quota = (chunks - k + 31) >> 5;
     int ticket = -1;
     if (threadIdx.x == 0) ticket = atomicAdd(sc + 32 * k, 1);
-    if (!idle) {
-#pragma unroll
-        for (int e = 0; e < 4; ++e) {
-            float g = g0[e] * gscale;
-            if (wd != 0.0f) g += wd * p[e];
-            m[e] = beta1 * m[e] + (1.0f - beta1) * g;
-            v[e] = beta2 * v[e] + (1.0f - beta2) * g * g;
-            const float denom = sqrtf(v[e]) * inv_sqrt_bc2 + eps;
-            p[e] -= step_size * (m[e] / denom);
-        }
-        if (wt) {
-            store16_wt(P, buf_bytes, wo, p);
-            store16_wt(M, buf_bytes, wo, m);
-            store16_wt(V, buf_bytes, wo, v);
-            if (zero_grads) store16_wt(Gr, buf_bytes, wo, zero4);
-        } else {
-            *reinterpret_cast<f32x4*>(P + o) = p;
-            *reinterpret_cast<f32x4*>(M + o) = m;
-            *reinterpret_cast<f32x4*>(V + o) = v;
-            if (zero_grads) *reinterpret_cast<f32x4*>(Gr + o) = zero4;
-        }
-    }
+    if (!idle)
+        adam_update_store(P, Gr, M, V, o, buf_bytes, wo, g0, p, m, v, step_size, inv_sqrt_bc2, beta1, beta2, eps, wd, gscale,
+                          zero_grads, wt);
+    ADAM_STAMP(5, 0);
     if (threadIdx.x == 0 && ticket == quota - 1) {
         __atomic_store_n(sc + 32 * k, 0, __ATOMIC_RELAXED);
         if (atomicAdd(sc + ADAM_TOP, 1) == min(chunks, 32) - 1) {
@@ -1137,6 +1167,128 @@
             __atomic_store_n(tensor_step + t, step_old + 1, __ATOMIC_RELAXED);
         }
     }
+    if (tr && threadIdx.x == 0) {
+        tr[7] = t;
+        ADAM_STAMP(6, 0);
+    }
+}
+
+__global__ __launch_bounds__(256) void live_adam_kernel(float* __restrict__ P, float* __restrict__ Gr, float* __restrict__ M,
+                                                        float* __restrict__ V, const int32_t* __restrict__ chunk_tensor,
+                                                        int n_chunks, const float* __restrict__ active,
+                                                        int32_t* __restrict__ tensor_step, int32_t* __restrict__ scratch,
+                                                        float lr, float beta1, float beta2, float eps, float wd, float gscale,
+                                                        int zero_grads, const int32_t* __restrict__ skip, int wt,
+                                                        const AdamLiveTable tab, long long* __restrict__ trace) {
+    __shared__ float s_corr[2];
+    long long* const tr = trace ? trace + 8 * (int64_t)blockIdx.x : nullptr;
+    ADAM_STAMP(0, 0);
+    const int bid = blockIdx.x;
+    int b = tab.run_chunk[0] + bid;
+#pragma unroll
+    for (int r = 1; r < ADAM_LIVE_MAX_RUNS; ++r) {
+        const bool in = (r < tab.n_runs) & (bid >= tab.run_blk[r]);
+        b = in ? tab.run_chunk[r] + (bid - tab.run_blk[r]) : b;
+    }
+    if (bid >= tab.live_blocks) {
+        if (skip && skip[0] != 0) return;
+        for (int g = 0; g < tab.n_gaps; ++g) {
+            int t0 = tab.gap_t0[0], t1 = tab.gap_t1[0];
+#pragma unroll
+            for (int i = 1; i <= ADAM_LIVE_MAX_RUNS; ++i)
+                if (g == i) {
+                    t0 = tab.gap_t0[i];
+                    t1 = tab.gap_t1[i];
+                }
+            for (int t = t0 + (int)threadIdx.x; t < t1; t += 256) {
+                if (!(active[t] > 0.0f)) continue;
+                int32_t* const sc = scratch + (int64_t)t * PP_ADAM_SCRATCH;
+                int first = sc[ADAM_FIRST] - 1, chunks = sc[ADAM_CHUNKS];
+                if (first < 0) {
+                    int lo = 0, hi = n_chunks;
+                    while (lo < hi) {
+                        const int mid = (lo + hi) >> 1;
+                        if (chunk_tensor[mid] < t) lo = mid + 1; else hi = mid;
+                    }
+                    if (lo >= n_chunks || chunk_tensor[lo] != t) continue;
+                    adam_find_run(chunk_tensor, n_chunks, t, lo, first, chunks);
+                }
+                sc[ADAM_FIRST] = first + 1;
+                sc[ADAM_CHUNKS] = chunks;
+                tensor_step[t] = tensor_step[t] + 1;
+            }
+        }
+        return;
+    }
+    const uint32_t buf_bytes = (uint32_t)n_chunks * 4096u, wo = ((uint32_t)b * 1024u + threadIdx.x * 4u) * 4u;
+    const int64_t o = (int64_t)b * 1024 + threadIdx.x * 4;
+    int first = -1, chunks = 0;
+    const int t = chunk_tensor[b];
+    const f32x4 g0 = *reinterpret_cast<const f32x4*>(Gr + o);
+    const f32x4 p = *reinterpret_cast<const f32x4*>(P + o);
+    const f32x4 m = *reinterpret_cast<const f32x4*>(M + o);
+    const f32x4 v = *reinterpret_cast<const f32x4*>(V + o);
+    const int32_t skip_word = (skip ? skip : chunk_tensor)[0];
+    const bool skipped = skip && skip_word != 0;
+    if (tr) {
+        asm volatile("" ::"s"(t));
+        ADAM_STAMP(1, 0);
+    }
+    if (t < 0) return;
+    int32_t* const sc = scratch + (int64_t)t * PP_ADAM_SCRATCH;
+    const float act = active[t];
+    int step_old = 0;
+    if (threadIdx.x == 0) {
+        step_old = __atomic_load_n(tensor_step + t, __ATOMIC_RELAXED);
+        first = __atomic_load_n(sc + ADAM_FIRST, __ATOMIC_RELAXED) - 1;
+        chunks = __atomic_load_n(sc + ADAM_CHUNKS, __ATOMIC_RELAXED);
+    }
+    if (!(act > 0.0f)) return;
+    if (skipped) {
+        if (zero_grads) {
+            const f32x4 zero4 = f32x4{0.f, 0.f, 0.f, 0.f};
+            if (wt) store16_wt(Gr, buf_bytes, wo, zero4);
+            else *reinterpret_cast<f32x4*>(Gr + o) = zero4;
+        }
+        return;
+    }
+    if (threadIdx.x == 0) {
+        if (first < 0) adam_find_run(chunk_tensor, n_chunks, t, b, first, chunks);
+        adam_corrections(step_old + 1, lr, beta1, beta2, s_corr);
+    }
+    ADAM_STAMP_ARRIVED(2, 64);
+    ADAM_STAMP(3, 64);
+    __syncthreads();
+    ADAM_STAMP(4, 0);
+    const float step_size = s_corr[0], inv_sqrt_bc2 = s_corr[1];
+    const int k = (b - first) & 31;
+    const int quota = (chunks - k + 31) >> 5;
+    int ticket = -1;
+    if (threadIdx.x == 0) ticket = atomicAdd(sc + 32 * k, 1);
+    adam_update_store(P, Gr, M, V, o, buf_bytes, wo, g0, p, m, v, step_size, inv_sqrt_bc2, beta1, beta2, eps, wd, gscale,
+                      zero_grads, wt);
+    ADAM_STAMP(5, 0);
+    if (threadIdx.x == 0 && ticket == quota - 1) {
+        __atomic_store_n(sc + 32 * k, 0, __ATOMIC_RELAXED);
+        if (atomicAdd(sc + ADAM_TOP, 1) == min(chunks, 32) - 1) {
+            __atomic_store_n(sc + ADAM_TOP, 0, __ATOMIC_RELAXED);
+            __atomic_store_n(sc + ADAM_FIRST, first + 1, __ATOMIC_RELAXED);
+            __atomic_store_n(sc + ADAM_CHUNKS, chunks, __ATOMIC_RELAXED);
+            __atomic_store_n(sc + ADAM_SEEN, 1, __ATOMIC_RELAXED);
+            __atomic_store_n(tensor_step + t, step_old + 1, __ATOMIC_RELAXED);
+        }
+    }
+    if (tr && threadIdx.x == 0) {
+        tr[7] = t;
+        ADAM_STAMP(6, 0);
+    }
+}
+
+extern long long* g_wgtrace;
+extern int g_wgtrace_cap, g_wgtrace_mode;
+
+static long long* adam_trace(int blocks) {
+    return g_wgtrace && g_wgtrace_mode == 3 && blocks <= g_wgtrace_cap ? g_wgtrace : nullptr;
 }
 
 int adam_step(float* params, float* grads, float* m, float* v, int64_t n_params, const int32_t* chunk_tensor,
@@ -1148,9 +1300,123 @@
     const int n_chunks = (int)(n_params / 1024);
     const int wt = store_wt_mode() && n_params < ((int64_t)1 << 30) ? 1 : 0;
     hipLaunchKernelGGL(adam_kernel, dim3((unsigned)n_chunks), dim3(256), 0, st, params, grads, m, v, chunk_tensor, n_chunks,
-                       active, tensor_step, scratch, lr, beta1, beta2, eps, wd, gscale, (flags & PP_ADAM_ZERO_GRADS) ? 1 : 0, skip, wt);
+                       active, tensor_step, scratch, lr, beta1, beta2, eps, wd, gscale, (flags & PP_ADAM_ZERO_GRADS) ? 1 : 0, skip, wt,
+                       adam_trace(n_chunks));
     PP_LAUNCH_CHECK("pp_adam_step");
     return 0;
 }
 
-}
+static std::mutex g_track_mutex;
+static std::vector<GradTrack> g_tracks;
+
+static int adam_live_mode() {
+    const char* e = getenv("PP_ADAM_LIVE");
+    return e ? (atoi(e) != 0) : 1;
+}
+
+static GradTrack* track_of(const void* ptr) {
+    const float* f = static_cast<const float*>(ptr);
+    for (auto& tr : g_tracks)
+        if (f >= tr.grads && f < tr.grads + tr.n_params) return &tr;
+    return nullptr;
+}
+
+int adam_live_bind(const float* grads, const float* m, const float* v, int64_t n_params, const int32_t* first, int n_tensors,
+                   bool clean) {
+    PP_CHECK_ARG(grads && m && v && first && n_tensors > 0 && n_params > 0 && n_params % 1024 == 0, "pp_adam_live_bind: bad argument");
+    PP_CHECK_ARG(first[0] == 0 && first[n_tensors] == n_params / 1024, "pp_adam_live_bind: the boundaries do not span the buffer");
+    for (int t = 0; t < n_tensors; ++t) PP_CHECK_ARG(first[t] <= first[t + 1], "pp_adam_live_bind: the boundaries must ascend");
+    std::lock_guard<std::mutex> lock(g_track_mutex);
+    for (size_t i = 0; i < g_tracks.size();) {
+        const GradTrack& o = g_tracks[i];
+        if (grads < o.grads + o.n_params && o.grads < grads + n_params) g_tracks.erase(g_tracks.begin() + i); else ++i;
+    }
+    GradTrack tr;
+    tr.grads = grads; tr.m = m; tr.v = v; tr.n_params = n_params; tr.n_tensors = n_tensors;
+    tr.first.assign(first, first + n_tensors + 1);
+    tr.touched.assign(n_tensors, clean ? 0 : 1);
+    g_tracks.push_back(std::move(tr));
+    return 0;
+}
+
+void adam_live_unbind(const float* grads) {
+    std::lock_guard<std::mutex> lock(g_track_mutex);
+    for (size_t i = 0; i < g_tracks.size();)
+        if (g_tracks[i].grads == grads) g_tracks.erase(g_tracks.begin() + i); else ++i;
+}
+
+int adam_live_info(const float* grads, int64_t* out, uint8_t* touched_out) {
+    std::lock_guard<std::mutex> lock(g_track_mutex);
+    GradTrack* tr = track_of(grads);
+    out[0] = tr ? 1 : 0; out[1] = out[2] = out[3] = 0;
+    if (!tr) return 0;
+    out[1] = (int64_t)tr->version; out[2] = (int64_t)tr->builds;
+    for (int t = 0; t < tr->n_tensors; ++t) {
+        out[3] += tr->touched[t] ? 0 : 1;
+        if (touched_out) touched_out[t] = tr->touched[t];
+    }
+    return 0;
+}
+
+void grads_touch(const float* ptr) {
+    std::lock_guard<std::mutex> lock(g_track_mutex);
+    if (GradTrack* tr = track_of(ptr)) tr->touch_offset(ptr - tr->grads);
+}
+
+void grads_touch_all(const void* ptr) {
+    if (!ptr) return;
+    std::lock_guard<std::mutex> lock(g_track_mutex);
+    const float* f = static_cast<const float*>(ptr);
+    for (auto& tr : g_tracks)
+        if ((f >= tr.grads && f < tr.grads + tr.n_params) || (f >= tr.m && f < tr.m + tr.n_params) ||
+            (f >= tr.v && f < tr.v + tr.n_params))
+            tr.touch_all();
+}
+
+void grads_touch_range(const float* grads, int64_t off, int64_t cnt) {
+    if (cnt <= 0) return;
+    std::lock_guard<std::mutex> lock(g_track_mutex);
+    GradTrack* tr = track_of(grads);
+    if (!tr) return;
+    off += grads - tr->grads;
+    for (int64_t c = std::max<int64_t>(off, 0) >> 10; c <= (std::min(off + cnt, tr->n_params) - 1) >> 10; ++c)
+        tr->touch_tensor(tr->tensor_of_chunk(c));
+}
+
+bool adam_live_table(const float* grads, const float* m, const float* v, int64_t n_params, int n_tensors, bool wd_on,
+                     AdamLiveTable& tab) {
+    if (!grads) return false;
+    std::lock_guard<std::mutex> lock(g_track_mutex);
+    GradTrack* tr = track_of(grads);
+    if (!(tr && tr->grads == grads && tr->n_params == n_params && tr->n_tensors == n_tensors)) return false;
+    if (tr->m != m || tr->v != v) tr->touch_all();
+    if (wd_on) tr->touch_all();
+    const AdamLiveTable* t = nullptr;
+    if (!tr->table(wd_on, &t)) return false;
+    tab = *t;
+    return true;
+}
+
+int adam_step_live(float* params, float* grads, float* m, float* v, int64_t n_params, const int32_t* chunk_tensor,
+                   const float* active, int32_t* tensor_step, int32_t* scratch, int n_tensors, float lr, float beta1, float beta2,
+                   float eps, float wd, float gscale, int flags, const int32_t* skip, hipStream_t st) {
+    const int mode = adam_live_mode();
+    AdamLiveTable tab{};
+    const bool live = mode != 0 && n_params < ((int64_t)1 << 30) &&
+                      adam_live_table(grads, m, v, n_params, n_tensors, wd != 0.0f, tab);
+    if (!live)
+        return adam_step(params, grads, m, v, n_params, chunk_tensor, active, tensor_step, scratch, n_tensors, lr, beta1, beta2, eps,
+                         wd, gscale, flags, skip, st);
+    PP_CHECK_ARG(params && m && v && chunk_tensor && active && tensor_step && scratch, "pp_adam_step_live: null pointer");
+    const int n_chunks = (int)(n_params / 1024);
+    const int wt = store_wt_mode();
+    const int blocks = tab.live_blocks + (tab.n_gaps > 0 ? 1 : 0);
+    if (blocks == 0) return 0;
+    const int zg = (flags & PP_ADAM_ZERO_GRADS) ? 1 : 0;
+    hipLaunchKernelGGL(live_adam_kernel, dim3((unsigned)blocks), dim3(256), 0, st, params, grads, m, v, chunk_tensor, n_chunks,
+                       active, tensor_step, scratch, lr, beta1, beta2, eps, wd, gscale, zg, skip, wt, tab, adam_trace(blocks));
+    PP_LAUNCH_CHECK("pp_adam_step_live");
+    return 0;
+}
+
+}
diff --git a/pyprob_amd/csrc/optim.hip b/pyprob_amd/csrc/optim.hip
--- a/pyprob_amd/csrc/optim.hip
+++ b/pyprob_amd/csrc/optim.hip
@@ -170,6 +170,8 @@
 int pp_sgd_step(float* params, float* grads, float* momentum_buf, int64_t n_params, const int32_t* chunk_tensor,
                 const float* active, int32_t n_tensors, float lr, float momentum, int32_t nesterov, float weight_decay,
                 float grad_scale, int32_t flags, const int32_t* skip, void* stream) {
+    pp::grads_touch_all(grads);
+    pp::grads_touch_all(momentum_buf);
     pp::prof_begin(3, pp::as_stream(stream));
     const int rc = pp::sgd_step(params, grads, momentum_buf, n_params, chunk_tensor, active, n_tensors, lr, momentum, nesterov,
                                 weight_decay, grad_scale, flags, skip, pp::as_stream(stream));
@@ -181,6 +183,7 @@
 int pp_larc_scale(const float* params, float* grads, int64_t n_params, const int32_t* chunk_tensor, const float* active,
                   int32_t n_tensors, float lr, float weight_decay, float grad_scale, float trust_coefficient, float eps,
                   float epsilon, int32_t clip, float* scratch, const int32_t* skip, void* stream) {
+    pp::grads_touch_all(grads);
     return pp::larc_scale(params, grads, n_params, chunk_tensor, active, n_tensors, lr, weight_decay, grad_scale,
                           trust_coefficient, eps, epsilon, clip, scratch, skip, pp::as_stream(stream));
 }
diff --git a/pyprob_amd/csrc/train_loop.hip b/pyprob_amd/csrc/train_loop.hip
--- a/pyprob_amd/csrc/train_loop.hip
+++ b/pyprob_amd/csrc/train_loop.hip
@@ -10,6 +10,9 @@
 int adam_step(float* params, float* grads, float* m, float* v, int64_t n_params, const int32_t* chunk_tensor,
               const float* active, int32_t* tensor_step, int32_t* arrived, int n_tensors, float lr, float beta1, float beta2,
               float eps, float wd, float gscale, int flags, const int32_t* skip, hipStream_t st);
+int adam_step_live(float* params, float* grads, float* m, float* v, int64_t n_params, const int32_t* chunk_tensor,
+                   const float* active, int32_t* tensor_step, int32_t* arrived, int n_tensors, float lr, float beta1, float beta2,
+                   float eps, float wd, float gscale, int flags, const int32_t* skip, hipStream_t st);
 int dp_world();
 int dp_reduce_grads(float* grads_full, int64_t n_params, int n_tensors, const float* presence, const int32_t* status,
                     const int64_t* skip_off, const int64_t* skip_cnt, int n_skip, float* loss_out, int32_t* status_out,
@@ -129,10 +132,10 @@
                                          st);
                 if (rc != 0) break;
             }
-            rc = pp::adam_step(tb->params, tb->grads, tb->exp_avg, tb->exp_avg_sq, net->n_params, tb->chunk_tensor,
-                               dp ? dp_tail : dev + pk[k].words, tb->tensor_step, tb->adam_scratch, n_tensors, lr[i], beta1, beta2,
-                               eps, weight_decay, dp ? 1.0f / (float)tb->dp_world : 1.0f, PP_ADAM_ZERO_GRADS,
-                               tb->status_ring + i, st);
+            rc = pp::adam_step_live(tb->params, tb->grads, tb->exp_avg, tb->exp_avg_sq, net->n_params, tb->chunk_tensor,
+                                    dp ? dp_tail : dev + pk[k].words, tb->tensor_step, tb->adam_scratch, n_tensors, lr[i], beta1,
+                                    beta2, eps, weight_decay, dp ? 1.0f / (float)tb->dp_world : 1.0f, PP_ADAM_ZERO_GRADS,
+                                    tb->status_ring + i, st);
         }
     }
     return rc;
@@ -172,9 +175,9 @@
                                      tb->dp_skip_cnt, tb->dp_n_skip, tb->loss_ring + i, tb->status_ring + i, st);
             if (rc != 0) return rc;
         }
-        rc = pp::adam_step(tb->params, tb->grads, tb->exp_avg, tb->exp_avg_sq, net->n_params, tb->chunk_tensor,
-                           dp ? dp_tail : active[i], tb->tensor_step, tb->adam_scratch, n_tensors, lr[i], beta1, beta2, eps,
-                           weight_decay, dp ? 1.0f / (float)tb->dp_world : 1.0f, PP_ADAM_ZERO_GRADS, tb->status_ring + i, st);
+        rc = pp::adam_step_live(tb->params, tb->grads, tb->exp_avg, tb->exp_avg_sq, net->n_params, tb->chunk_tensor,
+                                dp ? dp_tail : active[i], tb->tensor_step, tb->adam_scratch, n_tensors, lr[i], beta1, beta2, eps,
+                                weight_decay, dp ? 1.0f / (float)tb->dp_world : 1.0f, PP_ADAM_ZERO_GRADS, tb->status_ring + i, st);
         if (rc != 0) return rc;
     }
     return 0;
diff --git a/pyprob_amd/engine.py b/pyprob_amd/engine.py
--- a/pyprob_amd/engine.py
+++ b/pyprob_amd/engine.py
@@ -59,7 +59,9 @@
         self.tensor_step = torch.zeros(spec.n_tensors, dtype=torch.int32, device=self.device)
         self.arrived = torch.zeros(L.PP_ADAM_SCRATCH * spec.n_tensors, dtype=torch.int32, device=self.device)
         self._grads_clean = False
-        self.chunk_tensor = torch.from_numpy(spec.chunk_tensor_map()).to(self.device)
+        chunk_map = spec.chunk_tensor_map()
+        self.chunk_tensor = torch.from_numpy(chunk_map).to(self.device)
+        self._bind_live(chunk_map)
         self.addr_table = torch.from_numpy(spec.address_table()).to(self.device)
         self.net = spec.c_struct(self.addr_table.data_ptr())
         from . import ops
@@ -68,6 +70,37 @@
         self._active_cache = {}
         self._active_key = None
         self.ws_shape = (0, 0)
+
+    def _bind_live(self, chunk_map):
+        old = getattr(self, '_live_bound', None)
+        if old is not None:
+            self.lib.pp_adam_live_unbind(old)
+        self._live_bound = None
+        cm = np.asarray(chunk_map, np.int64)
+        nt = self.spec.n_tensors
+        if nt <= 0 or cm.size == 0 or cm[0] < 0 or np.any(np.diff(cm) < 0) or cm[-1] >= nt or cm.size * 1024 != self.spec.n_params:
+            return
+        first = np.ascontiguousarray(np.searchsorted(cm, np.arange(nt + 1)), np.int32)
+        L.check(self.lib.pp_adam_live_bind(self.grads.data_ptr(), self.exp_avg.data_ptr(), self.exp_avg_sq.data_ptr(),
+                                           self.spec.n_params, first.ctypes.data, nt, 1), 'pp_adam_live_bind')
+        self._live_bound = self.grads.data_ptr()
+
+    def __del__(self):
+        bound, lib = getattr(self, '_live_bound', None), getattr(self, 'lib', None)
+        if bound is not None and lib is not None:
+            try:
+                lib.pp_adam_live_unbind(bound)
+            except Exception:
+                pass
+
+    def mark_touched(self):
+        self.lib.pp_adam_live_mark_touched(self.grads.data_ptr())
+
+    def live_info(self):
+        out = np.zeros(4, np.int64)
+        touched = np.zeros(max(self.spec.n_tensors, 1), np.uint8)
+        self.lib.pp_adam_live_info(self.grads.data_ptr(), out.ctypes.data, touched.ctypes.data)
+        return tuple(int(x) for x in out), touched[:self.spec.n_tensors].astype(bool)
 
     def add_addresses(self, items):
         created = []
@@ -158,7 +191,8 @@
     def presence(self):
         return self._presence if self._active_key is not None else self.active
 
-    def adam_step(self, lr, beta1=0.9, beta2=0.999, eps=1e-8, weight_decay=0.0, zero_grads=False, skip=None, grad_scale=None):
+    def adam_step(self, lr, beta1=0.9, beta2=0.999, eps=1e-8, weight_decay=0.0, zero_grads=False, skip=None, grad_scale=None,
+                  live=False):
         gs = 1.0 / self.world_size if grad_scale is None else grad_scale
         if getattr(self, '_use_ops', False):
             from .ops import ops
@@ -166,11 +200,12 @@
                           self.tensor_step, self.arrived, lr, beta1, beta2, eps, weight_decay, gs,
                           L.PP_ADAM_ZERO_GRADS if zero_grads else 0, skip)
         else:
-            rc = self.lib.pp_adam_step(self.params.data_ptr(), self.grads.data_ptr(), self.exp_avg.data_ptr(),
-                                       self.exp_avg_sq.data_ptr(), self.spec.n_params, self.chunk_tensor.data_ptr(),
-                                       self.presence().data_ptr(), self.tensor_step.data_ptr(), self.arrived.data_ptr(),
-                                       self.spec.n_tensors, lr, beta1, beta2, eps, weight_decay, gs,
-                                       L.PP_ADAM_ZERO_GRADS if zero_grads else 0, L.ptr(skip), L.stream_ptr())
+            step = self.lib.pp_adam_step_live if live else self.lib.pp_adam_step
+            rc = step(self.params.data_ptr(), self.grads.data_ptr(), self.exp_avg.data_ptr(),
+                      self.exp_avg_sq.data_ptr(), self.spec.n_params, self.chunk_tensor.data_ptr(),
+                      self.presence().data_ptr(), self.tensor_step.data_ptr(), self.arrived.data_ptr(),
+                      self.spec.n_tensors, lr, beta1, beta2, eps, weight_decay, gs,
+                      L.PP_ADAM_ZERO_GRADS if zero_grads else 0, L.ptr(skip), L.stream_ptr())
             L.check(rc, 'pp_adam_step')
         self._grads_clean = bool(zero_grads)
 
@@ -211,7 +246,7 @@
                                         self._larc_scratch.data_ptr(), L.ptr(skip), L.stream_ptr())
             L.check(rc, 'pp_larc_scale')
 
-    def optimizer_step(self, lr, weight_decay=0.0, zero_grads=False, skip=None):
+    def optimizer_step(self, lr, weight_decay=0.0, zero_grads=False, skip=None, live=False):
         opt = self.optimizer
         scale = None
         if opt['larc']:
@@ -220,9 +255,9 @@
         if opt['kind'] == 'sgd':
             self.sgd_step(lr, opt['momentum'], True, weight_decay, zero_grads, skip, grad_scale=scale)
         elif scale is None:
-            self.adam_step(lr, weight_decay=weight_decay, zero_grads=zero_grads, skip=skip)
-        else:
-            self.adam_step(lr, weight_decay=0.0, zero_grads=zero_grads, skip=skip, grad_scale=1.0)
+            self.adam_step(lr, weight_decay=weight_decay, zero_grads=zero_grads, skip=skip, live=live)
+        else:
+            self.adam_step(lr, weight_decay=0.0, zero_grads=zero_grads, skip=skip, grad_scale=1.0, live=live)
 
     def _adam_only(self, what):
         if self.optimizer['kind'] != 'adam' or self.optimizer['larc']:
@@ -232,9 +267,9 @@
         loss = self.loss(batch, backward=True)
         if self.world_size > 1 or self.force_allreduce:
             self.allreduce_grads()
-            self.optimizer_step(lr, weight_decay=weight_decay, zero_grads=_ADAM_CLEARS, skip=self.reduced_status())
-        else:
-            self.optimizer_step(lr, weight_decay=weight_decay, zero_grads=_ADAM_CLEARS, skip=self.status_buf)
+            self.optimizer_step(lr, weight_decay=weight_decay, zero_grads=_ADAM_CLEARS, skip=self.reduced_status(), live=True)
+        else:
+            self.optimizer_step(lr, weight_decay=weight_decay, zero_grads=_ADAM_CLEARS, skip=self.status_buf, live=True)
         return loss
 
     def train_run(self, dataset, id_lists, lrs, weight_decay=0.0, beta1=0.9, beta2=0.999, eps=1e-8):
@@ -410,6 +445,7 @@
                     'pp_dp_reduce_grads')
             return
         from .parallel import allreduce_flat_
+        self.mark_touched()
         self.status_tail.copy_(self.status_buf[:1])
         if self.dp_overlap:
             import torch.distributed as dist
@@ -495,3 +531,4 @@
 
     def moments_written(self):
         self.arrived.view(-1, L.PP_ADAM_SCRATCH)[:, L.PP_ADAM_SEEN] = 1
+        self.mark_touched()
diff --git a/pyprob_amd/lib.py b/pyprob_amd/lib.py
--- a/pyprob_amd/lib.py
+++ b/pyprob_amd/lib.py
@@ -153,6 +153,15 @@
     'pp_ic_loss': (C.c_int, [C.POINTER(pp_net), C.POINTER(pp_batch), vp, vp, vp, C.c_size_t, vp, vp, vp, i32, vp]),
     'pp_adam_step': (C.c_int, [vp, vp, vp, vp, i64, vp, vp, vp, vp, i32, C.c_float, C.c_float, C.c_float, C.c_float,
                                C.c_float, C.c_float, i32, vp, vp]),
+    'pp_adam_step_live': (C.c_int, [vp, vp, vp, vp, i64, vp, vp, vp, vp, i32, C.c_float, C.c_float, C.c_float, C.c_float,
+                                    C.c_float, C.c_float, i32, vp, vp]),
+    'pp_adam_live_bind': (C.c_int, [vp, vp, vp, i64, vp, i32, i32]),
+    'pp_adam_live_unbind': (C.c_int, [vp]),
+    'pp_adam_live_mark_touched': (C.c_int, [vp]),
+    'pp_adam_live_mark_range': (C.c_int, [vp, i64, i64]),
+    'pp_adam_live_info': (C.c_int, [vp, vp, vp]),
+    'pp_adam_live_plan': (C.c_int, [vp, i32, vp, vp]),
+    'pp_adam_live_table': (C.c_int, [vp, vp, vp, i64, i32, C.c_float, vp]),
     'pp_sgd_step': (C.c_int, [vp, vp, vp, i64, vp, vp, i32, C.c_float, C.c_float, i32, C.c_float, C.c_float, i32, vp, vp]),
     'pp_larc_scale': (C.c_int, [vp, vp, i64, vp, vp, i32, C.c_float, C.c_float, C.c_float, C.c_float, C.c_float, C.c_float,
                                 i32, vp, vp, vp]),
```
